# ucla-mobility/QuantV2X

Hardware: AMD Instinct MI355X
Metric: frames/sec/node (N-agent int8 BEV fusion) (higher is better)
Workload: dtype i8

## Files before the change

### include/qv2x.h

```cpp
#ifndef QV2X_H
#define QV2X_H

#include <stdint.h>

#ifdef __cplusplus
extern "C" {
#endif
#if defined(__GNUC__) || defined(__clang__)
#pragma GCC visibility push(default)
#endif

#define QV2X_OK 0
#define QV2X_EINVAL (-1)
#define QV2X_EALIGN (-2)
#define QV2X_MAX_GROUPS 4

const char* qv2x_last_error(void);
#define QV2X_ABI_VERSION 9
int qv2x_version(void);

int qv2x_fill_i8(int8_t* buf, int64_t bytes, int value, void* stream);

int64_t qv2x_voxelize_workspace_bytes(int n_points);
int qv2x_voxelize_f32(const float* points, int n_points, const float* lidar_range, const float* voxel_size, int agent,
                      int max_points, int max_voxels, void* workspace, int64_t workspace_bytes,
                      float* voxel_features, int32_t* voxel_coords, int32_t* voxel_num_points, int32_t* n_voxels, void* stream);

int64_t qv2x_voxelize_batch_workspace_bytes(int n_sweeps, const int32_t* n_points );
int qv2x_voxelize_batch_f32(const float* const* points , const int32_t* n_points , int n_sweeps,
                            const float* lidar_range, const float* voxel_size, int first_agent, int max_points, int capacity,
                            void* workspace, int64_t workspace_bytes, float* voxel_features, int32_t* voxel_coords,
                            int32_t* voxel_num_points, int32_t* voxel_counts, void* stream);

typedef struct {
    float w[64 * 10];
    float b[64];
    float d1, z1, d2, z2;
    float vox[3], off[3];
} qv2x_pfn_params;
int qv2x_pfn_scatter_i8(const float* voxel_features, const int32_t* voxel_coords, const int32_t* voxel_num_points,
                        int M, int max_points, const qv2x_pfn_params* params ,
                        int8_t* canvas, int N, int ny, int nx, void* stream);
int qv2x_pfn_unscatter_i8(const int32_t* voxel_coords, int M, int value, int8_t* canvas, int N, int ny, int nx, void* stream);

typedef struct {
    int32_t n, h, w, cin_total, stride, cout;
    int32_t ngroups;
    int32_t group_c0[QV2X_MAX_GROUPS], group_c[QV2X_MAX_GROUPS], group_zx[QV2X_MAX_GROUPS];
    int32_t out_ctotal, out_c0;
    int32_t relu;
    float out_delta, out_zp;
} qv2x_conv_desc;
int qv2x_conv3x3_i8(const qv2x_conv_desc* desc , const int8_t* in, const int8_t* w,
                    const float* scale, const int32_t* corr, const int32_t* aw, const float* bias,
                    int8_t* out, void* stream);

int qv2x_conv3x3_i8_wide_ok(const qv2x_conv_desc* desc );
int qv2x_conv3x3_i8_pack_wide(const qv2x_conv_desc* desc , const int8_t* w, int8_t* w_wide, void* stream);
int qv2x_conv3x3_i8_wide(const qv2x_conv_desc* desc , const int8_t* in, const int8_t* w_wide,
                         const float* scale, const int32_t* corr, const int32_t* aw, const float* bias,
                         int8_t* out, void* stream);

typedef struct {
    int32_t n, h, w;
    int32_t in_h, in_w;
    int32_t depth, stride0, relu;
    float out_delta[4], out_zp[4];
} qv2x_chain_desc;
int qv2x_conv3x3_i8_chain64(const qv2x_chain_desc* desc , const int8_t* in, const int8_t* w_chain,
                            const float* scale, const int32_t* corr, const int32_t* aw, const float* bias,
                            int8_t* out, void* stream);

typedef struct {
    int32_t n, h, w, cin, cout, s;
    int32_t in_zx;
    float in_delta;
    int32_t out_ctotal, out_c0, relu;
    float out_delta, out_zp;
    int32_t out_h, out_w;
} qv2x_deconv_desc;
int qv2x_deconv_i8(const qv2x_deconv_desc* desc , const int8_t* in, const float* w, const float* bias,
                   int8_t* out, void* stream);

int qv2x_deconv_i8_batch(const qv2x_deconv_desc* descs , int n, const int8_t* const* ins ,
                         const float* const* ws, const float* const* biases, int8_t* const* outs, void* stream);

typedef struct {
    int32_t n, h, w;
    int32_t levels, kc;
    int32_t in_zx;
    float in_delta;
    int32_t segs;
} qv2x_encode_desc;
int64_t qv2x_codebook_level_floats(int kc);
int qv2x_codebook_c2_f32(const float* codebook, int kc, float* c2, void* stream);
int qv2x_codebook_encode_f32(const qv2x_encode_desc* desc , const int8_t* in,
                             const float* const* level_weights ,
                             uint8_t* codes, void* stream);
int qv2x_codebook_encode_wave_f32(const qv2x_encode_desc* desc , const int8_t* in, const float* in_f32,
                                  const float* const* level_weights , uint8_t* codes, void* stream);

int qv2x_codebook_encode_collapsed_f32(const qv2x_encode_desc* desc , const int8_t* in, const float* g_packed, const float* bias,
                                       const float* tables, uint8_t* codes, void* stream);

int qv2x_codebook_encode_candidates_i8(const qv2x_encode_desc* desc , const int8_t* in, const int8_t* g_limbs, const double* bias_packed,
                                       const int32_t* tables, const float* tau , uint8_t* codes, uint32_t* list, uint32_t* counters,
                                       void* stream);
int qv2x_codebook_encode_listed_f32(const qv2x_encode_desc* desc , const int8_t* in, const float* const* level_weights ,
                                    const uint32_t* list, const uint32_t* list_count, uint8_t* codes, void* stream);

int qv2x_codebook_encode_candidates_seg_i8(const qv2x_encode_desc* desc , const int8_t* in, const int8_t* g_limbs, const double* bias_packed,
                                           const int32_t* tables, const float* tau , uint8_t* codes, uint32_t* list, uint32_t* counters,
                                           void* stream);

typedef struct {
    int32_t agents, h, w, levels, kc;
    int32_t max_cav, ego;
    int64_t code_agent_stride, code_level_stride;
    double h_metres, w_metres, discrete_ratio;
    int32_t fusion;
} qv2x_fuse_desc;
int qv2x_fuse_att_f32(const qv2x_fuse_desc* desc , const uint8_t* codes, const float* lut, const float* lut_bias,
                      const float* feats, const double* pairwise, float* fused, void* stream);

int qv2x_fuse_att_batch_f32(const qv2x_fuse_desc* desc , int n_scenes, const int64_t* scene_offset ,
                            const int32_t* scene_agents , const uint8_t* codes, const float* lut, const float* lut_bias,
                            const float* feats, const double* pairwise, float* fused, void* stream);

int qv2x_decode_lut_f32(const uint8_t* codes, int R, int levels, int kc, const float* lut, const float* lut_bias,
                        float* out, void* stream);

int qv2x_dequant_i8_f32(const int8_t* in, int n, int h, int w, int c, int zp, float delta, float* out, void* stream);

int qv2x_heads_f32(const float* x, int R, int hw, int cout, int cout_pad, const float* w, const float* bias,
                   const float* da, const float* za, float* out, void* stream);

int qv2x_fuse_heads_batch_f32(const qv2x_fuse_desc* desc , int n_scenes, const int64_t* scene_offset ,
                              const int32_t* scene_agents , const uint8_t* codes, const float* lut, const float* lut_bias,
                              const float* feats, const double* pairwise, int cout, int cout_pad, const float* w, const float* bias,
                              const float* da, const float* za, float* out, float* fused_tap, void* stream);

int qv2x_table_heads_f32(const uint8_t* codes, int R, int hw, int levels, int kc, int c0, int c1, const float* tables,
                         const float* bias, const float* da, const float* za, float* out0, float* out1, void* stream);

int qv2x_decode_heads_f32(const uint8_t* codes, int R, int hw, int levels, int kc, const float* lut, const float* lut_bias,
                          int cout, int cout_pad, const float* w, const float* bias, const float* da, const float* za,
                          float* out, void* stream);

int qv2x_single_heads_lut_f32(const uint8_t* codes, int R, int hw, int levels, int kc, int cout, const float* tables,
                              const float* bias, const float* da, const float* za, float* out, void* stream);

int qv2x_heads_pair_f32(const float* x, int R, int hw, int cout, int cout_pad, const float* w, const float* bias,
                        const float* da, const float* za, float* out,
                        const uint8_t* codes, int R1, int levels, int kc, const float* lut, const float* lut_bias,
                        int cout1, int cout_pad1, const float* w1, const float* bias1, const float* da1,
                        const float* za1, float* out1, void* stream);

typedef struct {
    int32_t h, w, anchors_per_cell, num_bins;
    float score_threshold, nms_threshold, dir_offset;
    float range[6];
    float transform[16];
    int32_t max_boxes;
    int32_t num_classes;
    int32_t range_xy_only;
    float max_extent, z_min, z_max;
} qv2x_postprocess_desc;
int64_t qv2x_postprocess_workspace_bytes(const qv2x_postprocess_desc* desc );
int qv2x_postprocess_f32(const qv2x_postprocess_desc* desc , const float* cls, const float* reg, const float* dir,
                         const float* anchors, void* workspace, int64_t workspace_bytes, float* out_corners,
                         float* out_scores, int32_t* out_labels, int32_t* out_count, void* stream);

int64_t qv2x_postprocess_batch_workspace_bytes(const qv2x_postprocess_desc* desc , int frames);
int qv2x_postprocess_batch_f32(const qv2x_postprocess_desc* desc , int frames, const float* cls, int64_t cls_frame_stride,
                               const float* reg, int64_t reg_frame_stride, const float* dir, int64_t dir_frame_stride,
                               const float* anchors, const float* transforms , void* workspace, int64_t workspace_bytes,
                               float* out_corners, float* out_scores, int32_t* out_labels, int32_t* out_count, void* stream);

int64_t qv2x_postprocess_late_workspace_bytes(const qv2x_postprocess_desc* desc , int ncav);
int qv2x_postprocess_late_f32(const qv2x_postprocess_desc* desc , int ncav, const float* const* cls, const float* const* reg,
                              const float* const* dir, const float* const* anchors, const float* transforms , void* workspace,
                              int64_t workspace_bytes, float* out_corners, float* out_scores, int32_t* out_labels, int32_t* out_count,
                              void* stream);

typedef struct {
    int32_t n, h, w;
    int32_t cin_total, cin0, cin;
    int32_t stride;
    int32_t cout;
    int32_t out_ctotal, out_c0, relu;
} qv2x_f32conv_desc;
int qv2x_conv3x3_f32(const qv2x_f32conv_desc* desc , const float* in, const float* w, const float* bias, float* out, void* stream);
int qv2x_deconv_f32(const qv2x_f32conv_desc* desc , const float* in, const float* w, const float* bias, float* out, void* stream);
int qv2x_pfn_scatter_f32(const float* voxel_features, const int32_t* voxel_coords, const int32_t* voxel_num_points, int M, int max_points,
                         const float* w, const float* b, const float* vox, const float* off, float* canvas, int N, int ny, int nx, void* stream);
int qv2x_codebook_encode_f32in(const qv2x_encode_desc* desc , const float* in, const float* const* level_weights ,
                               uint8_t* codes, void* stream);

int qv2x_pyramid_weighted_fuse_f32(const qv2x_fuse_desc* desc , int channels, const float* feats, const float* score,
                                   const double* pairwise, float* out, void* stream);


typedef struct {
    int32_t n, h, w, cin, cout, stride;
    int32_t mode, relu;
    int32_t out_ctotal, out_c0;
    float out_delta, out_zp;
    int32_t res_zx;
    float res_delta;
} qv2x_conv1x1_desc;
int qv2x_conv1x1_i8(const qv2x_conv1x1_desc* desc , const int8_t* in, const int8_t* w_frag, const float* scale,
                    const int32_t* corr, const int32_t* aw, const float* bias, const void* res, void* out, void* stream);

typedef struct {
    int32_t n, h, w, c, cg, stride, relu;
    float out_delta, out_zp;
} qv2x_gconv_desc;
int qv2x_gconv3x3_i8(const qv2x_gconv_desc* desc , const int8_t* in, const int8_t* w_frag, const float* scale,
                     const int32_t* corr, const int32_t* aw, const float* bias, int8_t* out, void* stream);

typedef struct {
    int32_t n, h, w, planes, width, cg;
    int32_t in_zx;
    float in_delta;
    float delta1, zp1, delta2, zp2, out_delta, out_zp;
} qv2x_bottleneck_desc;
int qv2x_bottleneck_i8(const qv2x_bottleneck_desc* desc , const int8_t* x, const int8_t* const* w, const float* const* scale,
                       const int32_t* const* corr, const int32_t* const* aw, const float* const* bias, int8_t* out, void* stream);

int qv2x_conv3x3_i8_res(const qv2x_conv_desc* desc , const int8_t* in, const int8_t* w, const float* scale, const int32_t* corr,
                        const int32_t* aw, const float* bias, int res_mode, const void* res, int res_zx, float res_delta,
                        int8_t* out, void* stream);

int qv2x_deconv_f32in(const qv2x_deconv_desc* desc , const float* in, const float* w, const float* bias, int8_t* out, void* stream);

int qv2x_codebook_decode_f32(const uint8_t* codes, int64_t agent_stride, int64_t level_stride, int agents, int hw, int levels,
                             int kc, int d, const float* lut, const float* bias, float* out, void* stream);

int64_t qv2x_codebook64_level_floats(int kc);
int qv2x_codebook64_c2_f32(const float* codebook, int kc, float* c2, void* stream);
int qv2x_codebook_encode64_f32(const qv2x_encode_desc* desc , int cin_total, const int8_t* in,
                               const float* const* level_weights , uint8_t* codes, void* stream);

int qv2x_codebook_encode64_f32in(const qv2x_encode_desc* desc , int cin_total, const float* in,
                                 const float* const* level_weights , uint8_t* codes, void* stream);

int qv2x_add_relu_f32(const float* a, const float* b, float* out, int64_t count, void* stream);
int qv2x_occ_sigmoid_f32(const float* in, int n, int h, int w, int c_total, float* occ, float* score, void* stream);
int qv2x_pyramid_weighted_fuse_f32p(const qv2x_fuse_desc* desc , int channels, const float* feats, const float* score,
                                    const double* pairwise, float* out, void* stream);

typedef struct {
    int32_t n, h, w, c;
    int32_t aw, corr;
    float scale, bias, out_delta, out_zp;
} qv2x_occ_desc;
int qv2x_occ_score_i8(const qv2x_occ_desc* desc , const int8_t* in, const int8_t* w, const float* score_lut, float* score,
                      uint8_t* occ_code, void* stream);

int qv2x_pyramid_weighted_fuse_i8(const qv2x_fuse_desc* desc , int channels, const int8_t* feats, int in_zx, float in_delta,
                                  const float* score, const double* pairwise, float* out, void* stream);

typedef struct {
    int32_t subm;
    int32_t k[3], s[3], p[3];
    int32_t in_shape[3], out_shape[3];
    int32_t agents, cin, cout;
    int32_t cap_in, cap_out;
    float out_delta, out_zp;
} qv2x_spconv_desc;
int qv2x_mean_vfe_f32(const float* voxel_features, const int32_t* voxel_num_points, const int32_t* n_voxels , int cap,
                      int max_points, float* out, void* stream);
int qv2x_sp_index_scatter(const int32_t* coords, const int32_t* n_rows , int cap, int agents, int D, int H, int W,
                          int32_t* volume, int set, void* stream);
int64_t qv2x_sp_out_sites_workspace_bytes(const qv2x_spconv_desc* desc );
int qv2x_sp_out_sites(const qv2x_spconv_desc* desc , const int32_t* in_coords, const int32_t* n_in, int32_t* out_volume,
                      int32_t* out_coords, int32_t* n_out, void* workspace, int64_t workspace_bytes, void* stream);
int qv2x_sp_rulebook(const qv2x_spconv_desc* desc , const int32_t* out_coords, const int32_t* n_out, const int32_t* in_volume,
                     int32_t* nbr, void* stream);
int qv2x_sp_conv_f32in(const qv2x_spconv_desc* desc , const float* feat, const int32_t* nbr, const int32_t* n_out, const float* w,
                       const float* bn_g, const float* bn_h, int8_t* out, void* stream);
int qv2x_sp_conv_i8(const qv2x_spconv_desc* desc , const int8_t* in, const int32_t* nbr, const int32_t* n_out, const int8_t* w_frag,
                    const float* scale, const int32_t* corr, const int32_t* aw, const float* bn_g, const float* bn_h, int8_t* out, void* stream);
int qv2x_sp_to_bev_i8(const int8_t* feat, const int32_t* coords, const int32_t* n_rows , int cap, int c, int c_padded, int agents,
                      int D, int H, int W, int fill, int8_t* bev, void* stream);

#define QV2X_COMM_ID_BYTES 128
int qv2x_comm_unique_id(void* id );
int qv2x_comm_init(const void* id , int world, int rank, void** comm);
int qv2x_comm_destroy(void* comm);
int qv2x_allgather_codes(void* comm, const uint8_t* send, uint8_t* recv, int64_t bytes_per_rank, void* stream);

int qv2x_pairwise_from_poses_f64(const uint8_t* gathered, int world, int64_t agent_stride_bytes, int64_t pose_offset_bytes,
                                 int max_cav, double* pairwise, void* stream);
int qv2x_pairwise_from_poses_batch_f64(const uint8_t* gathered, int world, int64_t agent_stride_bytes, int64_t pose_offset_bytes,
                                       int frames, int64_t frame_stride_bytes, int max_cav, double* pairwise, void* stream);

#define QV2X_WIRE_F32 0
#define QV2X_WIRE_U8 1
int qv2x_fuse_att_band_f32(const qv2x_fuse_desc* desc , int n_scenes, const int64_t* scene_offset ,
                           const int32_t* scene_agents , const uint8_t* codes, const float* lut, const float* lut_bias,
                           const float* feats, const double* pairwise, int64_t cell0, int64_t n_cells, float* fused, void* stream);
int qv2x_heads_band(const float* x, int n_scenes, int64_t n_cells, int cout, int cout_pad, const float* w, const float* bias,
                    const float* da, const float* za, int wire, const float* da_host , void* out, void* stream);
int qv2x_fuse_heads_band(const qv2x_fuse_desc* desc , int n_scenes, const int64_t* scene_offset ,
                         const int32_t* scene_agents , const uint8_t* codes, const float* lut, const float* lut_bias,
                         const float* feats, const double* pairwise, int64_t cell0, int64_t n_cells, int cout, int cout_pad,
                         const float* w, const float* bias, const float* da, const float* za, int wire, const float* da_host ,
                         void* out, float* fused_tap, void* stream);
int qv2x_assemble_bands(const uint8_t* slabs, int world, int64_t slab_bytes, int frames, int cout, int h, int w, int wire,
                        const float* da, const float* za, float* out, void* stream);

typedef struct {
    int32_t frames;
    int32_t det_cap;
    int32_t gt_cap;
    int32_t n_classes;
    int32_t n_ranges;
    int32_t n_thresholds;
    float ranges[4][2];
    float thresholds[4];
} qv2x_eval_desc;
int64_t qv2x_eval_workspace_bytes(const qv2x_eval_desc* desc );
int qv2x_eval_tp_fp_f32(const qv2x_eval_desc* desc , const float* det_corners, const float* det_scores, const int32_t* det_labels,
                        const int32_t* det_count, const float* gt_corners, const int32_t* gt_labels, const int32_t* gt_count,
                        void* workspace, int64_t workspace_bytes, int32_t* out_order, float* out_scores, uint8_t* out_flags,
                        int32_t* out_match, int32_t* out_gt, void* stream);

typedef struct {
    int32_t frames;
    int32_t agents;
    int32_t obj_cap;
    int32_t gt_cap;
    int32_t row_floats;
    int32_t order;
    int32_t mode;
    int32_t range_xy_only;
    float range[6];
    float iou_threshold;
} qv2x_gt_desc;
int qv2x_gt_boxes_f32(const qv2x_gt_desc* desc , const float* boxes, const uint8_t* mask, const int32_t* ids, const float* transforms,
                      const int32_t* agent_counts, float* gt_corners, int32_t* gt_labels, int32_t* gt_ids, int32_t* gt_counts,
                      int32_t* gt_totals, void* stream);

typedef struct {
    int32_t channels;
    int32_t candidates;
    int32_t n_levels;
    int32_t reserved;
    int64_t per_channel;
} qv2x_range_search_desc;
int64_t qv2x_range_search_workspace_bytes(const qv2x_range_search_desc* desc );
int qv2x_range_search_f32(const qv2x_range_search_desc* desc , const float* x, const float* delta, const float* zp, double* loss,
                          int32_t* best, void* workspace, void* stream);

#define QV2X_LSS_LOGITS 0
#define QV2X_LSS_PROBS 1
typedef struct {
    int32_t samples;
    int32_t views;
    int32_t depth_bins;
    int32_t fh, fw;
    int32_t features;
    int32_t nx[3];
    float dx[3], bx[3];
} qv2x_lss_desc;
int64_t qv2x_lss_workspace_bytes(const qv2x_lss_desc* desc );
int qv2x_lss_plan_f32(const qv2x_lss_desc* desc , const float* frustum, const float* rots, const float* trans, const float* intrins,
                      const float* post_rots, const float* post_trans, int32_t* cells_out, void* workspace, void* stream);
int qv2x_lss_splat_f32(const qv2x_lss_desc* desc , const float* depth, const float* feats, int mode, void* workspace, float* out,
                       void* stream);

#if defined(__GNUC__) || defined(__clang__)
#pragma GCC visibility pop
#endif
#ifdef __cplusplus
}
#endif
#endif
```

### quantv2x_amd/csrc/codebook_encode.h

```cpp
#pragma once
#include "common.h"

namespace qv2x {

constexpr int ENC_D = 256;
constexpr int ENC_WAVE_PAD = 16 * 256;

struct EncArgs {
    const int8_t* in; const float* in_f32; uint8_t* codes;
    const float* lvl[4];
    int n, h, w, levels, kc, ax, M;
    int segs, ke;
    float dx;
    int m_lo, m_hi;
    int list_slots = 1, list_tail_max = 0;
    const unsigned* list = nullptr; const unsigned* list_count = nullptr;
};

__device__ __host__ __forceinline__ int64_t level_floats_wg(int kc) { return 3LL * (ENC_D * ENC_D + ENC_D) + (int64_t)ENC_D * kc + (int64_t)kc * ENC_D + kc; }
__device__ __host__ __forceinline__ int64_t level_floats(int kc) { return level_floats_wg(kc) + 3LL * ENC_D * ENC_D + (int64_t)((kc + 63) / 64 * 64) * ENC_D + ENC_WAVE_PAD; }

struct ListPlan { int n[3], first[3], total, full; };
__device__ __forceinline__ ListPlan list_plan(const EncArgs& a) {
    ListPlan p;
    int t = 0;
#pragma unroll
    for (int c = 0; c < 3; ++c) { p.n[c] = (int)a.list_count[1 + c]; p.first[c] = t; t += (p.n[c] + 31) >> 5; }
    p.total = t;
    const int full = t / a.list_slots * a.list_slots;
    p.full = t - full > a.list_tail_max ? t : full;
    return p;
}
__device__ __forceinline__ void list_tile(const ListPlan& p, int tile, int& cls, int& i0) {
    cls = tile >= p.first[2] ? 2 : (tile >= p.first[1] ? 1 : 0);
    i0 = (tile - p.first[cls]) * 32;
}

int encode_wave_launch(const EncArgs& a, hipStream_t st);
int encode_wave_list_launch(const EncArgs& a, int waves, hipStream_t st);

}
```

### quantv2x_amd/csrc/codebook_encode.hip

```cpp
#include <cstdlib>

#include <atomic>

#include "codebook_encode.h"

namespace qv2x {

#ifdef QV2X_ENC_TRACE
__device__ unsigned long long g_enc_blk[4096][4];
#endif
#ifdef QV2X_ENC_FINE
__device__ long long g_enc_fine[2048][40];
#define EFINE(k) do { if (threadIdx.x == 0 && blockIdx.x < 2048) g_enc_fine[blockIdx.x][12 * l + (k)] = __builtin_amdgcn_s_memtime(); } while (0)
#else
#define EFINE(k) do { } while (0)
#endif

constexpr int LDF = 258;
__device__ __forceinline__ int kpos(int c) { return (c & ~3) | ((c & 1) << 1) | ((c >> 1) & 1); }
constexpr int D = 256;
#ifndef QV2X_ENC_LDS_PAD
#define QV2X_ENC_LDS_PAD 0
#endif

__device__ __forceinline__ void lds_barrier() {
    asm volatile("s_waitcnt lgkmcnt(0)" ::: "memory");
    __builtin_amdgcn_s_barrier();
}


struct GemmHead { float2 s0[4]; float b; };
__device__ __forceinline__ GemmHead gemm_head(const float2* __restrict__ wp, const float* __restrict__ bias, int wave, int lane) {
    const int par = lane >> 5, col = wave * 32 + (lane & 31);
    GemmHead h;
    h.b = bias[col];
    const float2* wl = wp + (size_t)col * 2 + par;
#pragma unroll
    for (int t = 0; t < 4; ++t) h.s0[t] = wl[(size_t)t * D * 2];
    return h;
}

template <int ERT>
__device__ __forceinline__ void gemm_rows_x32(const float* __restrict__ src, const float2* __restrict__ wp, const GemmHead& head,
                                              int wave, int lane, v16f (&acc)[ERT]) {
    const int par = lane >> 5, col = wave * 32 + (lane & 31);
    const float b = head.b;
#pragma unroll
    for (int i = 0; i < ERT; ++i)
#pragma unroll
        for (int r = 0; r < 16; ++r) acc[i][r] = b;
    const float2* wl = wp + (size_t)col * 2 + par;
    const float* al = src + (lane & 31) * LDF + 2 * par;
    auto loadB = [&](float2 (&dst)[4], int q0) {
#pragma unroll
        for (int t = 0; t < 4; ++t) dst[t] = wl[(size_t)(q0 + t) * D * 2];
    };
    auto compute4 = [&](const float2 (&bset)[4], int q0) {
        float2 av[4][ERT];
#pragma unroll
        for (int t = 0; t < 4; ++t)
#pragma unroll
            for (int i = 0; i < ERT; ++i) av[t][i] = *(const float2*)(al + i * 32 * LDF + (q0 + t) * 4);
#pragma unroll
        for (int t = 0; t < 4; ++t) {
#pragma unroll
            for (int i = 0; i < ERT; ++i) acc[i] = __builtin_amdgcn_mfma_f32_32x32x2f32(av[t][i].x, bset[t].x, acc[i], 0, 0, 0);
#pragma unroll
            for (int i = 0; i < ERT; ++i) acc[i] = __builtin_amdgcn_mfma_f32_32x32x2f32(av[t][i].y, bset[t].y, acc[i], 0, 0, 0);
        }
    };
    float2 s0[4], s1[4];
#pragma unroll
    for (int t = 0; t < 4; ++t) s0[t] = head.s0[t];
    for (int q0 = 0; q0 < 64; q0 += 8) {
        loadB(s1, q0 + 4);
        __builtin_amdgcn_sched_barrier(0);
        compute4(s0, q0);
        __builtin_amdgcn_sched_barrier(0);
        loadB(s0, q0 + 8);
        __builtin_amdgcn_sched_barrier(0);
        compute4(s1, q0 + 4);
        __builtin_amdgcn_sched_barrier(0);
    }
}

__device__ __forceinline__ unsigned long long dist_key(float d, int code) {
    unsigned b = __builtin_bit_cast(unsigned, d);
    b ^= (unsigned)((int)b >> 31) | 0x80000000u;
    return ((unsigned long long)b << 32) | (unsigned)code;
}

template <int ERT>
__device__ __forceinline__ void store_tile(float* __restrict__ dst, int wave, int lane, const v16f (&acc)[ERT]) {
#pragma unroll
    for (int i = 0; i < ERT; ++i)
#pragma unroll
        for (int r = 0; r < 16; ++r)
            dst[(i * 32 + mfma32_row(r, lane)) * LDF + kpos(wave * 32 + (lane & 31))] = acc[i][r];
}

constexpr int ENC_MAX_TILES = 16;
template <int ER> constexpr int enc_smem_floats() { return 2 * ER * LDF + 4 * ER + 4 * ER + 2 * ENC_MAX_TILES * ER + 4 * ER + QV2X_ENC_LDS_PAD; }

template <int ER, bool EXT, bool LIST = false>
__device__ __forceinline__ void encode_rows(const EncArgs& a, const int m0, float* __restrict__ smem, const unsigned* __restrict__ lst = nullptr,
                                            const int n_listed = 0, const int start = 0) {
    constexpr int ERT = ER / 32;
    const int segs = EXT ? a.segs : 1;
    float* bufA = smem;
    float* bufB = smem + ER * LDF;
    float* x2 = smem + 2 * ER * LDF;
    float* pval = x2 + 4 * ER;
    unsigned long long* pkey = (unsigned long long*)(pval + 4 * ER);
    int* code_s = (int*)(pkey + ENC_MAX_TILES * ER);

    const int tid = threadIdx.x, lane = tid & 63, wave = tid >> 6;
#ifdef QV2X_ENC_TRACE
    const unsigned long long t_start = __builtin_readcyclecounter();
    unsigned hwid, xcc;
    asm volatile("s_getreg_b32 %0, hwreg(HW_REG_HW_ID)" : "=s"(hwid));
    asm volatile("s_getreg_b32 %0, hwreg(HW_REG_XCC_ID)" : "=s"(xcc));
#endif
    {
        constexpr int TPR = 512 / ER;
        constexpr int CPT = D / TPR;
        const int row = tid / TPR, part = tid % TPR;
        int m = m0 + row;
        if (LIST) m = (int)lst[m < n_listed ? m : n_listed - 1];
        m = m < a.M ? m : a.M - 1;
        const int img = m / (a.h * a.w), rem = m - img * (a.h * a.w);
        const int y = rem / a.w, x = rem - y * a.w;
        const size_t pixel = (size_t)(img * (a.h + 2) + y + 1) * (a.w + 2) + x + 1;
        const int8_t* src = a.in + pixel * D + part * CPT;
        if (a.in_f32) {
            const float* sf = a.in_f32 + pixel * D + part * CPT;
#pragma unroll
            for (int c = 0; c < CPT / 4; ++c) {
                const v4f v = *(const v4f*)(sf + c * 4);
#pragma unroll
                for (int e = 0; e < 4; ++e) bufA[row * LDF + kpos(part * CPT + c * 4 + e)] = v[e];
            }
        } else
#pragma unroll
        for (int c = 0; c < CPT / 16; ++c) {
            const v4i raw = *(const v4i*)(src + c * 16);
#pragma unroll
            for (int e = 0; e < 16; ++e) {
                const int xs = (raw[e >> 2] << (24 - (e & 3) * 8)) >> 24;
                bufA[row * LDF + kpos(part * CPT + c * 16 + e)] = (float)(xs + a.ax) * a.dx;
            }
        }
    }
    GemmHead head = gemm_head((const float2*)a.lvl[0], a.lvl[0] + D * D, wave, lane);
    lds_barrier();

    v16f acc[ERT];
    for (int l = 0; l < a.levels; ++l) {
        const float* W = a.lvl[l];
        const float* stage_w = W;
        const float* stage_b = stage_w + D * D;
        const float* qhead_w = stage_b + D;
        const float* qhead_b = qhead_w + D * D;
        const float* lhead_w = qhead_b + D;
        const float* lhead_b = lhead_w + D * D;
        const float* cbp = lhead_b + D;
        const float* cb = cbp + (size_t)D * a.ke;
        const float* c2 = cb + (size_t)a.ke * D;

        EFINE(0);
        gemm_rows_x32(bufA, (const float2*)stage_w, head, wave, lane, acc);
        EFINE(1);
        const bool proven = LIST && l < start;
        if (proven) {
            head = gemm_head((const float2*)lhead_w, lhead_b, wave, lane);
            store_tile(bufB, wave, lane, acc);
            if (tid < ER * segs) {
                const int sg = tid / ER, r = tid - sg * ER;
                code_s[tid] = sg * a.kc + (int)a.codes[((size_t)l * segs + sg) * a.M + lst[m0 + r < n_listed ? m0 + r : n_listed - 1]];
            }
            lds_barrier();
        } else {
        head = gemm_head((const float2*)qhead_w, qhead_b, wave, lane);
        store_tile(bufB, wave, lane, acc);
        lds_barrier();
        EFINE(2);
        gemm_rows_x32(bufB, (const float2*)qhead_w, head, wave, lane, acc);
        EFINE(3);
        if (l + 1 < a.levels) head = gemm_head((const float2*)lhead_w, lhead_b, wave, lane);
        store_tile(bufA, wave, lane, acc);
        lds_barrier();
        EFINE(4);

        if (tid < ER * 4) {
            const int row = tid % ER, part = tid / ER;
            const float2* qr = (const float2*)(bufA + row * LDF + part * 64);
            float s = 0.0f;
#pragma unroll 4
            for (int j = 0; j < 16; ++j) {
                const float2 e = qr[2 * j], o = qr[2 * j + 1];
                s = fmaf(e.x, e.x, s); s = fmaf(o.x, o.x, s); s = fmaf(e.y, e.y, s); s = fmaf(o.y, o.y, s);
            }
            pval[part * ER + row] = s;
        }
        constexpr int TPR = 8 / ERT;
        const int ct0 = wave % TPR, rt = wave / TPR;
        const int ntile = (a.ke + 31) >> 5;
        float2 dhead[4];
        float c2v = 0.0f;
        if (ct0 < ntile) {
            const int code = ct0 * 32 + (lane & 31);
            const float2* cl = (const float2*)cbp + (size_t)code * 2 + (lane >> 5);
#pragma unroll
            for (int t = 0; t < 4; ++t) dhead[t] = cl[(size_t)t * a.ke * 2];
            c2v = c2[code];
        }
        lds_barrier();
        EFINE(5);
        if (tid < ER) {
            const float p0 = pval[tid], p1 = pval[ER + tid], p2 = pval[2 * ER + tid], p3 = pval[3 * ER + tid];
            if (segs == 1) x2[tid] = (p0 + p1) + (p2 + p3);
            else if (segs == 2) { x2[tid] = p0 + p1; x2[ER + tid] = p2 + p3; }
            else { x2[tid] = p0; x2[ER + tid] = p1; x2[2 * ER + tid] = p2; x2[3 * ER + tid] = p3; }
        }
        lds_barrier();
        EFINE(6);

#pragma unroll 1
        for (int ct = ct0; ct < ntile; ct += EXT ? TPR : ENC_MAX_TILES) {
            const int par = lane >> 5, code = ct * 32 + (lane & 31);
            v16f dacc;
#pragma unroll
            for (int r = 0; r < 16; ++r) dacc[r] = 0.0f;
            const float2* cl = (const float2*)cbp + (size_t)code * 2 + par;
            const float* al = bufA + (rt * 32 + (lane & 31)) * LDF + 2 * par;
            auto loadC = [&](float2 (&dst)[4], int q0) {
#pragma unroll
                for (int t = 0; t < 4; ++t) dst[t] = cl[(size_t)(q0 + t) * a.ke * 2];
            };
            auto dist4 = [&](const float2 (&bset)[4], int q0) {
                float2 av[4];
#pragma unroll
                for (int t = 0; t < 4; ++t) av[t] = *(const float2*)(al + (q0 + t) * 4);
#pragma unroll
                for (int t = 0; t < 4; ++t) {
                    dacc = __builtin_amdgcn_mfma_f32_32x32x2f32(av[t].x, bset[t].x, dacc, 0, 0, 0);
                    dacc = __builtin_amdgcn_mfma_f32_32x32x2f32(av[t].y, bset[t].y, dacc, 0, 0, 0);
                }
            };
            float2 s0[4], s1[4];
            if (ct == ct0) {
#pragma unroll
                for (int t = 0; t < 4; ++t) s0[t] = dhead[t];
            } else {
                loadC(s0, 0);
                c2v = c2[code];
            }
            for (int q0 = 0; q0 < 64; q0 += 8) {
                loadC(s1, q0 + 4);
                __builtin_amdgcn_sched_barrier(0);
                dist4(s0, q0);
                __builtin_amdgcn_sched_barrier(0);
                loadC(s0, q0 + 8);
                __builtin_amdgcn_sched_barrier(0);
                dist4(s1, q0 + 4);
                __builtin_amdgcn_sched_barrier(0);
            }
            EFINE(7);
            unsigned resk = 0xffffffffu;
            int resc = 0;
            const int l31 = lane & 31, hi = lane >> 5;
            const float* x2r = x2 + (segs == 1 ? 0 : (ct * 32) / a.kc) * ER;
#pragma unroll
            for (int r = 0; r < 16; ++r) {
                const int row = rt * 32 + mfma32_row(r, lane);
                const float d = (x2r[row] + c2v) - 2.0f * dacc[r];
                unsigned b = __builtin_bit_cast(unsigned, d);
                b ^= (unsigned)((int)b >> 31) | 0x80000000u;
                unsigned m = b, o;
                o = (unsigned)__builtin_amdgcn_update_dpp((int)m, (int)m, 0xB1, 0xf, 0xf, false); m = o < m ? o : m;
                o = (unsigned)__builtin_amdgcn_update_dpp((int)m, (int)m, 0x4E, 0xf, 0xf, false); m = o < m ? o : m;
                o = (unsigned)__builtin_amdgcn_update_dpp((int)m, (int)m, 0x141, 0xf, 0xf, false); m = o < m ? o : m;
                o = (unsigned)__builtin_amdgcn_update_dpp((int)m, (int)m, 0x140, 0xf, 0xf, false); m = o < m ? o : m;
                const auto sw = __builtin_amdgcn_permlane16_swap(m, m, false, false);
                m = sw[0] < sw[1] ? sw[0] : sw[1];
                const unsigned long long eq = __builtin_amdgcn_ballot_w64(b == m);
                const int c_lo = __builtin_ctz((unsigned)eq), c_hi = __builtin_ctz((unsigned)(eq >> 32));
                const int c = hi ? c_hi : c_lo;
                const bool mine = l31 == r;
                resk = mine ? m : resk;
                resc = mine ? c : resc;
            }
            if (l31 < 16) pkey[ct * ER + rt * 32 + mfma32_row(l31, lane)] = ((unsigned long long)resk << 32) | (unsigned)(ct * 32 + resc);
        }
        lds_barrier();
        EFINE(8);
        if (tid < ER) {
            const int tps = segs == 1 ? ntile : a.kc >> 5;
            for (int sg = 0; sg < segs; ++sg) {
                unsigned long long bk = pkey[(sg * tps) * ER + tid];
                for (int wv = 1; wv < tps; ++wv) {
                    const unsigned long long ok = pkey[(sg * tps + wv) * ER + tid];
                    bk = ok < bk ? ok : bk;
                }
                const int bi = (int)(unsigned)bk;
                code_s[sg * ER + tid] = bi;
                if (LIST) {
                    if (m0 + tid < n_listed) a.codes[((size_t)l * segs + sg) * a.M + lst[m0 + tid]] = (uint8_t)(bi - sg * a.kc);
                } else if (m0 + tid < a.m_hi) a.codes[((size_t)l * segs + sg) * a.M + m0 + tid] = (uint8_t)(bi - sg * a.kc);
            }
        }
        lds_barrier();
        EFINE(9);
        }

        if (l + 1 < a.levels) {
            const int col = wave * 32 + (lane & 31);
            const int* cs = code_s + ((wave * segs) >> 3) * ER;
            float cv[ERT][16];
#pragma unroll
            for (int i = 0; i < ERT; ++i)
#pragma unroll
                for (int r = 0; r < 16; ++r) cv[i][r] = cb[(size_t)cs[i * 32 + mfma32_row(r, lane)] * D + col];
            gemm_rows_x32(bufB, (const float2*)lhead_w, head, wave, lane, acc);
            EFINE(10);
            head = gemm_head((const float2*)a.lvl[l + 1], a.lvl[l + 1] + D * D, wave, lane);
#pragma unroll
            for (int i = 0; i < ERT; ++i)
#pragma unroll
                for (int r = 0; r < 16; ++r) bufA[(i * 32 + mfma32_row(r, lane)) * LDF + kpos(col)] = acc[i][r] - cv[i][r];
            lds_barrier();
            EFINE(11);
        }
    }
#ifdef QV2X_ENC_TRACE
    if (tid == 0 && blockIdx.x < 4096) {
        g_enc_blk[blockIdx.x][0] = t_start; g_enc_blk[blockIdx.x][1] = __builtin_readcyclecounter();
        g_enc_blk[blockIdx.x][2] = hwid; g_enc_blk[blockIdx.x][3] = xcc;
    }
#endif
}

template <int ER, bool EXT = false>
__global__ __launch_bounds__(512, ER == 32 ? 4 : 2) void codebook_encode_kernel(const EncArgs a) {
    __shared__ __attribute__((aligned(16))) float smem[enc_smem_floats<ER>()];
    encode_rows<ER, EXT>(a, a.m_lo + blockIdx.x * ER, smem);
}

template <bool EXT>
__global__ __launch_bounds__(512, 2) void codebook_encode_list_tail_kernel(const EncArgs a) {
    __shared__ __attribute__((aligned(16))) float smem[enc_smem_floats<32>()];
    const ListPlan plan = list_plan(a);
    for (int t = plan.full + (int)blockIdx.x; t < plan.total; t += (int)gridDim.x) {
        int cls, i0;
        list_tile(plan, t, cls, i0);
        encode_rows<32, EXT, true>(a, i0, smem, a.list + (size_t)cls * a.M, plan.n[cls], cls);
        __syncthreads();
    }
}

template <bool EXT>
__global__ __launch_bounds__(512, 2) void codebook_encode_mixed_kernel(const EncArgs a, const int n64) {
    __shared__ __attribute__((aligned(16))) float smem[enc_smem_floats<64>()];
    if ((int)blockIdx.x < n64) encode_rows<64, EXT>(a, a.m_lo + blockIdx.x * 64, smem);
    else encode_rows<32, EXT>(a, a.m_lo + n64 * 64 + ((int)blockIdx.x - n64) * 32, smem);
}

__global__ void codebook_c2_kernel(const float* __restrict__ cb, int kc, float* __restrict__ c2) {
    const int k = blockIdx.x * blockDim.x + threadIdx.x;
    if (k >= kc) return;
    float s[4];
    for (int q = 0; q < 4; ++q) {
        float acc = 0.0f;
        for (int i = 0; i < 64; ++i) { const float v = cb[(size_t)k * D + q * 64 + i]; acc = fmaf(v, v, acc); }
        s[q] = acc;
    }
    c2[k] = (s[0] + s[1]) + (s[2] + s[3]);
}

}

extern "C" int qv2x_codebook_c2_f32(const float* codebook, int kc, float* c2, void* stream) {
    using namespace qv2x;
    if (!codebook || !c2 || kc <= 0) return fail(QV2X_EINVAL, "qv2x_codebook_c2_f32: bad arguments");
    codebook_c2_kernel<<<(kc + 63) / 64, 64, 0, (hipStream_t)stream>>>(codebook, kc, c2);
    return hip_check(hipGetLastError(), "qv2x_codebook_c2_f32 launch");
}

extern "C" int64_t qv2x_codebook_level_floats(int kc) { return qv2x::level_floats(kc); }

static int encode_launch(const qv2x_encode_desc* d, const int8_t* in, const float* in_f32, const float* const* level_weights, uint8_t* codes, void* stream,
                         int form = 0);

extern "C" int qv2x_codebook_encode_wave_f32(const qv2x_encode_desc* d, const int8_t* in, const float* in_f32, const float* const* level_weights,
                                             uint8_t* codes, void* stream) {
    if (!in && !in_f32) return qv2x::fail(QV2X_EINVAL, "qv2x_codebook_encode_wave_f32: null pointer");
    return encode_launch(d, in_f32 ? (const int8_t*)in_f32 : in, in_f32, level_weights, codes, stream, 1);
}

extern "C" int qv2x_codebook_encode_f32(const qv2x_encode_desc* d, const int8_t* in, const float* const* level_weights,
                                        uint8_t* codes, void* stream) {
    return encode_launch(d, in, nullptr, level_weights, codes, stream);
}

extern "C" int qv2x_codebook_encode_f32in(const qv2x_encode_desc* d, const float* in, const float* const* level_weights,
                                          uint8_t* codes, void* stream) {
    if (!in) return qv2x::fail(QV2X_EINVAL, "qv2x_codebook_encode_f32in: null pointer");
    return encode_launch(d, (const int8_t*)in, in, level_weights, codes, stream);
}

extern "C" int qv2x_codebook_encode_listed_f32(const qv2x_encode_desc* d, const int8_t* in, const float* const* level_weights,
                                               const uint32_t* list, const uint32_t* list_count, uint8_t* codes, void* stream) {
    using namespace qv2x;
    if (!d || !in || !level_weights || !codes || !list || !list_count) return fail(QV2X_EINVAL, "qv2x_codebook_encode_listed_f32: null pointer");
    if (d->n <= 0 || d->h <= 0 || d->w <= 0 || d->levels < 1 || d->levels > 4) return fail(QV2X_EINVAL, "qv2x_codebook_encode_listed_f32: bad shape");
    const int segs = d->segs ? d->segs : 1;
    if (segs != 1 && segs != 2) return fail(QV2X_EINVAL, "qv2x_codebook_encode_listed_f32: seg_num 1 or 2 (got %d)", d->segs);
    if (d->kc < 32 || d->kc > 256 || d->kc % 32 || (segs > 1 && d->kc % 64) || segs * d->kc > 32 * ENC_MAX_TILES)
        return fail(QV2X_EINVAL, "qv2x_codebook_encode_listed_f32: dict_size must be a multiple of 32 up to 256 (of 64 with two segments): got %d x %d", segs, d->kc);
    if ((uintptr_t)in & 15) return fail(QV2X_EALIGN, "qv2x_codebook_encode_listed_f32: in must be 16-byte aligned");
    EncArgs a;
    a.in = in; a.in_f32 = nullptr; a.codes = codes; a.n = d->n; a.h = d->h; a.w = d->w; a.levels = d->levels; a.kc = d->kc;
    a.segs = segs; a.ke = segs * d->kc;
    const bool ext = segs > 1 || a.ke > 128;
    a.ax = 128 - d->in_zx; a.dx = d->in_delta; a.M = d->n * d->h * d->w; a.m_lo = 0; a.m_hi = a.M;
    a.list = list; a.list_count = list_count;
    for (int l = 0; l < 4; ++l) {
        a.lvl[l] = l < d->levels ? level_weights[l] : nullptr;
        if (l < d->levels && (!a.lvl[l] || ((uintptr_t)a.lvl[l] & 15))) return fail(QV2X_EALIGN, "qv2x_codebook_encode_listed_f32: level %d weights null or unaligned", l);
    }
    int cus = 256, dev = 0, v = 0;
    if (hipGetDevice(&dev) == hipSuccess && hipDeviceGetAttribute(&v, hipDeviceAttributeMultiprocessorCount, dev) == hipSuccess && v > 0) cus = v;
    const int tiles = (a.M + 31) / 32;
    int tail_knob = 0;
#ifdef QV2X_DEV_KNOBS
    static const int tail_env = getenv("QV2X_LIST_TAIL") ? atoi(getenv("QV2X_LIST_TAIL")) : 0;
    tail_knob = tail_env;
#endif
    a.list_slots = 4 * cus; a.list_tail_max = tail_knob > 0 ? tail_knob : 2 * cus;
    const int grid_tail = 2 * cus;
    if (tiles + 3 >= 2 * a.list_slots) {
        if (int rc = encode_wave_list_launch(a, a.list_slots, (hipStream_t)stream)) return rc;
    } else {
        a.list_slots = 1 << 30; a.list_tail_max = 1 << 30;
    }
    if (ext) codebook_encode_list_tail_kernel<true><<<tiles < grid_tail ? tiles : grid_tail, 512, 0, (hipStream_t)stream>>>(a);
    else codebook_encode_list_tail_kernel<false><<<tiles < grid_tail ? tiles : grid_tail, 512, 0, (hipStream_t)stream>>>(a);
    return hip_check(hipGetLastError(), "qv2x_codebook_encode_listed_f32 launch");
}

static int encode_launch(const qv2x_encode_desc* d, const int8_t* in, const float* in_f32, const float* const* level_weights, uint8_t* codes, void* stream,
                         int form) {
    using namespace qv2x;
    if (!d || !in || !level_weights || !codes) return fail(QV2X_EINVAL, "qv2x_codebook_encode_f32: null pointer");
    if (d->n <= 0 || d->h <= 0 || d->w <= 0 || d->levels < 1 || d->levels > 4) return fail(QV2X_EINVAL, "qv2x_codebook_encode_f32: bad shape");
    const int segs = d->segs ? d->segs : 1;
    if (segs != 1 && segs != 2 && segs != 4) return fail(QV2X_EINVAL, "qv2x_codebook_encode_f32: seg_num must be 1, 2 or 4 (got %d)", d->segs);
    if (d->kc < 32 || d->kc > 256 || d->kc % 32 || (segs > 1 && d->kc % 64) || segs * d->kc > 32 * ENC_MAX_TILES)
        return fail(QV2X_EINVAL, "qv2x_codebook_encode_f32: dict_size must be a multiple of 32 up to 256 (of 64 with seg_num > 1; seg_num * dict_size <= %d): "
                                 "got dict_size %d, seg_num %d", 32 * ENC_MAX_TILES, d->kc, segs);
    if ((uintptr_t)in & 15) return fail(QV2X_EALIGN, "qv2x_codebook_encode_f32: in must be 16-byte aligned");
    EncArgs a;
    a.in = in; a.in_f32 = in_f32; a.codes = codes; a.n = d->n; a.h = d->h; a.w = d->w; a.levels = d->levels; a.kc = d->kc;
    a.segs = segs; a.ke = segs * d->kc;
    const bool ext = segs > 1 || a.ke > 128;
    a.ax = 128 - d->in_zx; a.dx = d->in_delta; a.M = d->n * d->h * d->w; a.m_lo = 0; a.m_hi = a.M;
    for (int l = 0; l < 4; ++l) {
        a.lvl[l] = l < d->levels ? level_weights[l] : nullptr;
        if (l < d->levels && (!a.lvl[l] || ((uintptr_t)a.lvl[l] & 15))) return fail(QV2X_EALIGN, "qv2x_codebook_encode_f32: level %d weights null or unaligned", l);
    }
    int er_env = 0;
#ifdef QV2X_DEV_KNOBS
    static const int er_knob = [] { const char* e = getenv("QV2X_ENC_ROWS"); return e ? atoi(e) : 0; }();
    if (er_knob != 0 && er_knob != 32 && er_knob != 64 && er_knob != 96) return fail(QV2X_EINVAL, "QV2X_ENC_ROWS=%d: 32, 64 or 96", er_knob);
    er_env = er_knob;
#endif
    static std::atomic<int> cus_of[64];
    int cus = 256, dev = 0, v = 0;
    if (hipGetDevice(&dev) == hipSuccess && dev >= 0 && dev < 64) {
        cus = cus_of[dev].load(std::memory_order_relaxed);
        if (cus == 0) {
            cus = (hipDeviceGetAttribute(&v, hipDeviceAttributeMultiprocessorCount, dev) == hipSuccess && v > 0) ? v : 256;
            cus_of[dev].store(cus, std::memory_order_relaxed);
        }
    }
    hipStream_t st = (hipStream_t)stream;
    if (form == 1) return encode_wave_launch(a, st);
    const int slots = 4 * cus, waves = (a.M + 31) / 32;
    const int rounds = waves / slots, rest = waves - rounds * slots;
    int tail_max = 2 * cus;
#ifdef QV2X_DEV_KNOBS
    static const int tail_knob = [] { const char* e = getenv("QV2X_ENC_TAIL"); return e ? atoi(e) : -1; }();
    if (tail_knob >= 0) tail_max = tail_knob;
#endif
    if (er_env == 0 && rounds >= 1) {
        if (rest == 0 || rest > tail_max) return encode_wave_launch(a, st);
        EncArgs main = a, tail = a;
        main.m_hi = rounds * slots * 32;
        tail.m_lo = main.m_hi;
        if (int rc = encode_wave_launch(main, st)) return rc;
        if (ext) codebook_encode_kernel<32, true><<<rest, 512, 0, st>>>(tail);
        else codebook_encode_kernel<32><<<rest, 512, 0, st>>>(tail);
        return hip_check(hipGetLastError(), "qv2x_codebook_encode_f32 launch");
    }
    const int n64 = (a.M / 64) / cus * cus;
    const int er = er_env ? er_env : (n64 > 0 ? 96 : 32);
    if (er == 64) {
        if (ext) codebook_encode_kernel<64, true><<<(a.M + 63) / 64, 512, 0, st>>>(a);
        else codebook_encode_kernel<64><<<(a.M + 63) / 64, 512, 0, st>>>(a);
    } else if (er == 96 && n64 > 0) {
        if (ext) codebook_encode_mixed_kernel<true><<<n64 + (a.M - n64 * 64 + 31) / 32, 512, 0, st>>>(a, n64);
        else codebook_encode_mixed_kernel<false><<<n64 + (a.M - n64 * 64 + 31) / 32, 512, 0, st>>>(a, n64);
    } else if (ext) {
        codebook_encode_kernel<32, true><<<(a.M + 31) / 32, 512, 0, st>>>(a);
    } else {
        codebook_encode_kernel<32><<<(a.M + 31) / 32, 512, 0, st>>>(a);
    }
    return hip_check(hipGetLastError(), "qv2x_codebook_encode_f32 launch");
}

#ifdef QV2X_ENC_FINE
extern "C" __attribute__((visibility("default"))) int qv2x_debug_encode_fine(long long* host, int n) {
    return hipMemcpyFromSymbol(host, HIP_SYMBOL(qv2x::g_enc_fine), (size_t)n * 40 * sizeof(long long)) == hipSuccess ? 0 : -1;
}
#endif
#ifdef QV2X_ENC_TRACE
extern "C" __attribute__((visibility("default"))) int qv2x_debug_encode_blocks(unsigned long long* host, int n) {
    return (int)hipMemcpyFromSymbol(host, HIP_SYMBOL(qv2x::g_enc_blk), (size_t)n * 4 * sizeof(unsigned long long));
}
#endif
```

### quantv2x_amd/csrc/codebook_encode_cand.hip

```cpp
#include "common.h"

namespace qv2x {
namespace {

struct CandArgs {
    const int8_t* in; const int8_t* gpack; const double* bias; const int* tables;
    uint8_t* codes; unsigned* list; unsigned* counters;
    float tau[3][3];
    int n, h, w, hw, M, levels, kc, ke, zx, gbytes, tbytes;
    float delta;
};

constexpr int NPF = 8;
constexpr int LIMBS = 3;
template <int V> struct IC { static constexpr int value = V; };

__device__ __forceinline__ double shfl_xor_f64(double v, int m) {
    const long long b = __builtin_bit_cast(long long, v);
    const int lo = __shfl_xor((int)b, m), hi = __shfl_xor((int)(b >> 32), m);
    return __builtin_bit_cast(double, ((long long)hi << 32) | (unsigned)lo);
}

template <int CT, int SEGS, int PACK>
__global__ __launch_bounds__(256) __attribute__((amdgpu_waves_per_eu(1, 1))) void encode_candidates_kernel(const CandArgs a) {
    const int lane = threadIdx.x & 63, wave = __builtin_amdgcn_readfirstlane(threadIdx.x >> 6), j = lane & 31, hf = lane >> 5;
    const int m0 = ((int)blockIdx.x * 4 + wave) * (32 * CT);

    v4i xb[CT][8];
    int m[CT];
    float n0[CT], n1[CT];
#pragma unroll
    for (int ct = 0; ct < CT; ++ct) {
        m[ct] = m0 + 32 * ct + j;
        const int mc = m[ct] < a.M ? m[ct] : a.M - 1;
        const int img = mc / a.hw, rem = mc - img * a.hw, y = rem / a.w, x = rem - y * a.w;
        const int8_t* px = a.in + ((size_t)(img * (a.h + 2) + y + 1) * (a.w + 2) + x + 1) * 256 + 16 * hf;
#pragma unroll
        for (int s = 0; s < 8; ++s) xb[ct][s] = *(const v4i*)(px + 32 * s);
        unsigned s1 = 0, s2 = 0, sad = 0;
        const unsigned zx4 = (unsigned)a.zx * 0x01010101u;
#pragma unroll
        for (int s = 0; s < 8; ++s)
#pragma unroll
            for (int d = 0; d < 4; ++d) {
                const unsigned u = (unsigned)xb[ct][s][d] ^ 0x80808080u;
                s1 = __builtin_amdgcn_udot4(u, 0x01010101u, s1, false);
                s2 = __builtin_amdgcn_udot4(u, u, s2, false);
                sad = __builtin_amdgcn_sad_u8(u, zx4, sad);
            }
        s1 += __shfl_xor(s1, 32); s2 += __shfl_xor(s2, 32); sad += __shfl_xor(sad, 32);
        const int n2 = (int)s2 - 2 * a.zx * (int)s1 + 256 * a.zx * a.zx;
        n0[ct] = a.delta * sqrtf((float)n2);
        n1[ct] = (float)sad;
    }

    const __amdgpu_buffer_rsrc_t grs = __builtin_amdgcn_make_buffer_rsrc((void*)a.gpack, 0, a.gbytes, 0x00020000);
    int wo = 0;
    const int loff = lane * 16;
    auto gload = [&](int f) __attribute__((always_inline)) { return (v4i)__builtin_amdgcn_raw_buffer_load_b128(grs, loff, wo + f * 1024, 0); };
    v4i ring[NPF];
#pragma unroll
    for (int i = 0; i < NPF; ++i) ring[i] = gload(i);

    const __amdgpu_buffer_rsrc_t brs = __builtin_amdgcn_make_buffer_rsrc((void*)a.bias, 0, a.levels * a.ke * 8, 0x00020000);
    const __amdgpu_buffer_rsrc_t trs = __builtin_amdgcn_make_buffer_rsrc((void*)a.tables, 0, a.tbytes, 0x00020000);
    int o[2][SEGS][CT] = {};
    int first[CT];
#pragma unroll
    for (int ct = 0; ct < CT; ++ct) first[ct] = 3;
    const int ntile = a.kc >> 5;
    const int tsz = a.ke * a.ke;
    auto level = [&](auto lc) __attribute__((always_inline)) {
        constexpr int l = decltype(lc)::value;
        bool weak_l[CT];
#pragma unroll
        for (int ct = 0; ct < CT; ++ct) weak_l[ct] = false;
        auto segment = [&](auto sc) __attribute__((always_inline)) {
        constexpr int sg = decltype(sc)::value;
        double best[CT], second[CT];
#pragma unroll
        for (int ct = 0; ct < CT; ++ct) best[ct] = second[ct] = 1.0e300;
        v4i qb[2][2], qt[2][l > 0 ? l * SEGS : 1][CT];
        auto issue = [&](int T, int g, int slot) __attribute__((always_inline)) {
            const int col = sg * a.kc + 32 * T + 8 * g;
            const int kofs = l * a.ke + col;
            qb[slot][0] = (v4i)__builtin_amdgcn_raw_buffer_load_b128(brs, 32 * hf, kofs * 8, 0);
            qb[slot][1] = (v4i)__builtin_amdgcn_raw_buffer_load_b128(brs, 32 * hf + 16, kofs * 8, 0);
#pragma unroll
            for (int ct = 0; ct < CT; ++ct) {
#pragma unroll
                for (int jj = 0; jj < l; ++jj)
#pragma unroll
                    for (int sp = 0; sp < SEGS; ++sp)
                        qt[slot][jj * SEGS + sp][ct] = (v4i)__builtin_amdgcn_raw_buffer_load_b128(trs, o[jj][sp][ct], ((l * (l - 1) / 2 + jj) * tsz + col) * 4, 0);
            }
        };
#pragma unroll 1
        for (int T = 0; T < ntile; ++T) {
            v16i acc[LIMBS][CT];
#pragma unroll
            for (int lb = 0; lb < LIMBS; ++lb)
#pragma unroll
                for (int ct = 0; ct < CT; ++ct)
#pragma unroll
                    for (int r = 0; r < 16; ++r) acc[lb][ct][r] = 0;
#pragma unroll
            for (int f = 0; f < LIMBS * 8; ++f) {
                const v4i A = ring[f % NPF];
#pragma unroll
                for (int ct = 0; ct < CT; ++ct) acc[f >> 3][ct] = __builtin_amdgcn_mfma_i32_32x32x32_i8(A, xb[ct][f & 7], acc[f >> 3][ct], 0, 0, 0);
                ring[f % NPF] = gload(f + NPF);
                if (f == LIMBS * 8 - 6) issue(T, 0, 0);
                __builtin_amdgcn_sched_barrier(0);
            }
            wo += LIMBS * 8 * 1024;
#pragma unroll
            for (int g = 0; g < 4; ++g) {
                if (g < 3) issue(T, g + 1, (g + 1) & 1);
                __builtin_amdgcn_sched_barrier(0);
                const int sl = g & 1;
                double b[4];
                b[0] = __builtin_bit_cast(double, ((unsigned long long)(unsigned)qb[sl][0][1] << 32) | (unsigned)qb[sl][0][0]);
                b[1] = __builtin_bit_cast(double, ((unsigned long long)(unsigned)qb[sl][0][3] << 32) | (unsigned)qb[sl][0][2]);
                b[2] = __builtin_bit_cast(double, ((unsigned long long)(unsigned)qb[sl][1][1] << 32) | (unsigned)qb[sl][1][0]);
                b[3] = __builtin_bit_cast(double, ((unsigned long long)(unsigned)qb[sl][1][3] << 32) | (unsigned)qb[sl][1][2]);
#pragma unroll
                for (int ct = 0; ct < CT; ++ct) {
#pragma unroll
                    for (int e = 0; e < 4; ++e) {
                        const int r = 4 * g + e;
                        int lo = (acc[1][ct][r] << 8) + acc[0][ct][r];
#pragma unroll
                        for (int q = 0; q < l * SEGS; ++q) lo += qt[sl][q][ct][e];
                        double c = __builtin_fma((double)lo, (double)PACK, b[e]);
                        c = __builtin_fma((double)acc[2][ct][r], 65536.0 * PACK, c);
                        second[ct] = fmin(second[ct], fmax(best[ct], c));
                        best[ct] = fmin(best[ct], c);
                    }
                }
                __builtin_amdgcn_sched_barrier(0);
            }
        }
#pragma unroll
        for (int ct = 0; ct < CT; ++ct) {
            const double ob = shfl_xor_f64(best[ct], 32), os = shfl_xor_f64(second[ct], 32);
            const double nb = fmin(best[ct], ob), ns = fmin(fmax(best[ct], ob), fmin(second[ct], os));
            const int c = (int)((long long)nb & (PACK - 1));
            if (l < 2) o[l < 2 ? l : 0][sg][ct] = ((sg * a.kc + c) * a.ke + 4 * hf) * 4;
            const float t = ((a.tau[l][0] + a.tau[l][1] * n0[ct]) + (a.tau[l][2] * n0[ct]) * n0[ct]) + n1[ct];
            weak_l[ct] |= !(ns - nb > (double)PACK * (double)ceilf(t) + (double)(PACK - 1));
            if (hf == 0 && m[ct] < a.M) a.codes[(size_t)(l * SEGS + sg) * a.M + m[ct]] = (uint8_t)c;
        }
        };
        segment(IC<0>{});
        if constexpr (SEGS > 1) segment(IC<1>{});
#pragma unroll
        for (int ct = 0; ct < CT; ++ct)
            if (weak_l[ct] && first[ct] == 3) first[ct] = l;
    };
    level(IC<0>{});
    if (a.levels > 1) level(IC<1>{});
    if (a.levels > 2) level(IC<2>{});
    unsigned long long mask[3][CT];
    unsigned cnt[3] = {0, 0, 0};
#pragma unroll
    for (int c = 0; c < 3; ++c)
#pragma unroll
        for (int ct = 0; ct < CT; ++ct) {
            mask[c][ct] = __builtin_amdgcn_ballot_w64(first[ct] == c && hf == 0 && m[ct] < a.M);
            cnt[c] += (unsigned)__builtin_popcountll(mask[c][ct]);
        }
    __shared__ unsigned wcnt[4][3], wbase[3];
    if (lane == 0) { wcnt[wave][0] = cnt[0]; wcnt[wave][1] = cnt[1]; wcnt[wave][2] = cnt[2]; }
    __syncthreads();
    if (threadIdx.x < 3) {
        const unsigned tot = wcnt[0][threadIdx.x] + wcnt[1][threadIdx.x] + wcnt[2][threadIdx.x] + wcnt[3][threadIdx.x];
        wbase[threadIdx.x] = tot ? atomicAdd(a.counters + 1 + threadIdx.x, tot) : 0u;
        if (tot) atomicAdd(a.counters, tot);
    }
    __syncthreads();
    unsigned base[3];
#pragma unroll
    for (int c = 0; c < 3; ++c) {
        base[c] = wbase[c];
        for (int w2 = 0; w2 < wave; ++w2) base[c] += wcnt[w2][c];
    }
#pragma unroll
    for (int c = 0; c < 3; ++c) {
        unsigned at = __builtin_amdgcn_readfirstlane(base[c]);
#pragma unroll
        for (int ct = 0; ct < CT; ++ct) {
            if (first[ct] == c && hf == 0 && m[ct] < a.M)
                a.list[(size_t)c * a.M + at + (unsigned)__builtin_popcountll(mask[c][ct] & ((1ull << lane) - 1ull))] = (unsigned)m[ct];
            at += (unsigned)__builtin_popcountll(mask[c][ct]);
        }
    }
}

__global__ void zero_counters_kernel(unsigned* c) { if (threadIdx.x < 4) c[threadIdx.x] = 0; }

template <int CT, int SEGS, int PACK>
void launch(const CandArgs& a, hipStream_t st) {
    encode_candidates_kernel<CT, SEGS, PACK><<<(a.M + 128 * CT - 1) / (128 * CT), 256, 0, st>>>(a);
}

template <int PACK, int MAX_SEGS>
int candidates(const char* me, const qv2x_encode_desc* d, const int8_t* in, const int8_t* g_limbs, const double* bias_packed, const int32_t* tables,
               const float* tau, uint8_t* codes, uint32_t* list, uint32_t* counters, void* stream) {
    if (!d || !in || !g_limbs || !bias_packed || !tau || !codes || !list || !counters) return fail(QV2X_EINVAL, "%s: null pointer", me);
    if (d->n <= 0 || d->h <= 0 || d->w <= 0 || d->levels < 1 || d->levels > 3) return fail(QV2X_EINVAL, "%s: 1..3 levels", me);
    const int segs = d->segs ? d->segs : 1;
    if (segs < 1 || segs > MAX_SEGS) return fail(QV2X_EINVAL, "%s: seg_num 1 .. %d (got %d; the exact entry takes seg_num 1 | 2 | 4)", me, MAX_SEGS, d->segs);
    if (d->kc < 32 || d->kc > PACK || d->kc % 32 || (segs > 1 && d->kc % 64))
        return fail(QV2X_EINVAL, "%s: dict_size a multiple of 32 up to %d (of 64 with two segments; got %d x %d)", me, PACK, segs, d->kc);
    if (d->levels > 1 && !tables) return fail(QV2X_EINVAL, "%s: the residual levels need their tables", me);
    if (d->in_zx < 0 || d->in_zx > 255) return fail(QV2X_EINVAL, "%s: in_zx outside 0..255", me);
    if (((uintptr_t)in & 15) || ((uintptr_t)g_limbs & 15) || ((uintptr_t)tables & 15) || ((uintptr_t)bias_packed & 7))
        return fail(QV2X_EALIGN, "%s: 16-byte aligned maps, limbs and tables", me);
    CandArgs a;
    a.in = in; a.gpack = g_limbs; a.bias = bias_packed; a.tables = tables; a.codes = codes; a.list = list; a.counters = counters;
    for (int l = 0; l < 3; ++l)
        for (int i = 0; i < 3; ++i) a.tau[l][i] = l < d->levels ? tau[l * 3 + i] : 0.0f;
    a.n = d->n; a.h = d->h; a.w = d->w; a.hw = d->h * d->w; a.M = d->n * a.hw; a.levels = d->levels; a.kc = d->kc; a.ke = segs * d->kc; a.zx = d->in_zx;
    a.gbytes = d->levels * (a.ke / 32) * LIMBS * 8 * 1024;
    a.tbytes = (d->levels > 1 ? d->levels * (d->levels - 1) / 2 : 1) * a.ke * a.ke * 4;
    a.delta = d->in_delta;
    hipStream_t st = (hipStream_t)stream;
    zero_counters_kernel<<<1, 64, 0, st>>>(counters);
    int dev = 0, cus = 256, v = 0;
    if (hipGetDevice(&dev) == hipSuccess && hipDeviceGetAttribute(&v, hipDeviceAttributeMultiprocessorCount, dev) == hipSuccess && v > 0) cus = v;
    const bool large = a.M >= 4 * cus * 32 * (segs == 2 ? 3 : 4) * 2;
    if (segs == 1) large ? launch<4, 1, PACK>(a, st) : launch<2, 1, PACK>(a, st);
    else if constexpr (MAX_SEGS > 1) large ? launch<3, 2, PACK>(a, st) : launch<2, 2, PACK>(a, st);
    return hip_check(hipGetLastError(), me);
}

}
}

extern "C" int qv2x_codebook_encode_candidates_i8(const qv2x_encode_desc* d, const int8_t* in, const int8_t* g_limbs, const double* bias_packed,
                                                  const int32_t* tables, const float* tau, uint8_t* codes, uint32_t* list, uint32_t* counters,
                                                  void* stream) {
    return qv2x::candidates<128, 1>("qv2x_codebook_encode_candidates_i8", d, in, g_limbs, bias_packed, tables, tau, codes, list, counters, stream);
}

extern "C" int qv2x_codebook_encode_candidates_seg_i8(const qv2x_encode_desc* d, const int8_t* in, const int8_t* g_limbs, const double* bias_packed,
                                                      const int32_t* tables, const float* tau, uint8_t* codes, uint32_t* list, uint32_t* counters,
                                                      void* stream) {
    return qv2x::candidates<256, 2>("qv2x_codebook_encode_candidates_seg_i8", d, in, g_limbs, bias_packed, tables, tau, codes, list, counters, stream);
}
```

### quantv2x_amd/csrc/codebook_encode_wave.hip

```cpp
#include "codebook_encode.h"

namespace qv2x {

namespace {

constexpr int D = ENC_D;
constexpr int RS = 260;
constexpr int NPF = 4;

__device__ __forceinline__ v16f mfma(float a, float b, v16f c) { return __builtin_amdgcn_mfma_f32_32x32x2f32(a, b, c, 0, 0, 0); }


__device__ __forceinline__ void tile_to_lds(float* __restrict__ row, int h, int T, const v16f& acc) {
#pragma unroll
    for (int rq = 0; rq < 4; ++rq) {
        float* g = row + (4 * T + rq) * 8 + 2 * h;
        *(float2*)g = make_float2(acc[4 * rq], acc[4 * rq + 2]);
        *(float2*)(g + 4) = make_float2(acc[4 * rq + 1], acc[4 * rq + 3]);
    }
}

__device__ __forceinline__ void lds_to_operand(const float* __restrict__ row, int h, float (&m)[128]) {
#pragma unroll
    for (int g = 0; g < 32; ++g) {
        const v4f v = *(const v4f*)(row + g * 8 + 4 * h);
        m[4 * g] = v.x; m[4 * g + 1] = v.y; m[4 * g + 2] = v.z; m[4 * g + 3] = v.w;
    }
}

__device__ __forceinline__ void tile_vec(const float* __restrict__ p, int h, int T, v4f (&o)[4]) {
#pragma unroll
    for (int rq = 0; rq < 4; ++rq) o[rq] = *(const v4f*)(p + 32 * T + 8 * rq + 4 * h);
}

#ifdef QV2X_ENCW_FINE
__device__ long long g_encw_fine[4096][32];
#define WFINE(k) do { if (threadIdx.x == 0 && blockIdx.x < 4096) g_encw_fine[blockIdx.x][8 * l + (k)] = __builtin_readcyclecounter(); } while (0)
#define WFINE2(k) do { if (fine2 && threadIdx.x == 0 && blockIdx.x < 4096) g_encw_fine[blockIdx.x][24 + (k)] = __builtin_readcyclecounter(); } while (0)
#define WFINE2_ARM(v) fine2 = (v)
#else
#define WFINE(k) do { } while (0)
#define WFINE2(k) do { } while (0)
#define WFINE2_ARM(v) do { } while (0)
#endif

}

template <int V> struct IC { static constexpr int value = V; };

template <bool F32IN, int SEGS, bool LIST = false>
__global__ __attribute__((amdgpu_flat_work_group_size(64, 64), amdgpu_waves_per_eu(1, 1))) void codebook_encode_wave_kernel(const EncArgs a) {
    __shared__ __attribute__((aligned(16))) float smem[32 * RS];
    const int lane = threadIdx.x, j = lane & 31, h = lane >> 5;
    float* const row = smem + j * RS;
    ListPlan plan{};
    if (LIST) plan = list_plan(a);
#pragma unroll 1
    for (int round = 0; LIST ? round * (int)gridDim.x < plan.full : round == 0; ++round) {
    const int tile = LIST ? round * (int)gridDim.x + ((round & 1) ? (int)gridDim.x - 1 - (int)blockIdx.x : (int)blockIdx.x) : (int)blockIdx.x;
    if (LIST && tile >= plan.full) continue;
    int mrow;
    bool owned;
    int start = 0;
    if (LIST) {
        int cls, i0;
        list_tile(plan, tile, cls, i0);
        owned = i0 + j < plan.n[cls];
        mrow = (int)a.list[(size_t)cls * a.M + (owned ? i0 + j : plan.n[cls] - 1)];
        start = cls;
    } else {
        mrow = a.m_lo + tile * 32 + j;
        owned = mrow < a.m_hi;
    }

    float xq[128], z[128];
    {
        int m = mrow;
        m = m < a.M ? m : a.M - 1;
        const int img = m / (a.h * a.w), rem = m - img * (a.h * a.w);
        const int y = rem / a.w, x = rem - y * a.w;
        const size_t pixel = (size_t)(img * (a.h + 2) + y + 1) * (a.w + 2) + x + 1;
        if (F32IN) {
            const v4f* sf = (const v4f*)(a.in_f32 + pixel * D);
#pragma unroll
            for (int q = 0; q < 64; ++q) {
                const v4f v = sf[q];
                xq[2 * q] = h ? v.y : v.x;
                xq[2 * q + 1] = h ? v.w : v.z;
            }
        } else {
            const v4i* src = (const v4i*)(a.in + pixel * D);
            const float fax = (float)(a.ax - 128);
#pragma unroll
            for (int c = 0; c < 16; ++c) {
                const v4i raw = src[c];
#pragma unroll
                for (int d = 0; d < 4; ++d) {
                    const unsigned u = ((unsigned)raw[d] ^ 0x80808080u) >> (8 * h);
                    xq[8 * c + 2 * d] = ((float)(u & 0xffu) + fax) * a.dx;
                    xq[8 * c + 2 * d + 1] = ((float)((u >> 16) & 0xffu) + fax) * a.dx;
                }
            }
        }
    }

    for (int l = 0; l < a.levels; ++l) {
        const float* W = a.lvl[l];
        const float* stage_b = W + D * D;
        const float* qhead_b = stage_b + D + D * D;
        const float* lhead_b = qhead_b + D + D * D;
        const float* cb = lhead_b + D + (size_t)D * a.ke;
        const float* c2 = cb + (size_t)a.ke * D;
        const __amdgpu_buffer_rsrc_t wrs = __builtin_amdgcn_make_buffer_rsrc((void*)(W + level_floats_wg(a.ke)), 0, 0x7fffffff, 0x00020000);
        int wo = 0;
        const int loff = lane * 16;
        auto wload = [&](int grp) __attribute__((always_inline)) {
            return __builtin_bit_cast(v4f, __builtin_amdgcn_raw_buffer_load_b128(wrs, loff, wo + grp * 1024, 0));
        };
        const bool last = l + 1 == a.levels;
        const int npair = (a.ke + 63) >> 6;

        v4f bn[2][4];
        auto next_vec = [&](const float* p, int P) __attribute__((always_inline)) {
            tile_vec(p, h, 2 * P, bn[0]);
            tile_vec(p, h, 2 * P + 1, bn[1]);
        };
        auto next_c2 = [&](int P) __attribute__((always_inline)) {
            tile_vec(c2, h, 2 * P, bn[0]);
            if (64 * P + 32 < a.ke) tile_vec(c2, h, 2 * P + 1, bn[1]);
            else
#pragma unroll
                for (int i = 0; i < 4; ++i) bn[1][i] = v4f{INFINITY, INFINITY, INFINITY, INFINITY};
        };
        auto next_c2s = [&](int s0, int s1, int P) __attribute__((always_inline)) {
            tile_vec(c2 + s0 * a.kc, h, P, bn[0]);
            tile_vec(c2 + s1 * a.kc, h, P, bn[1]);
        };
        next_vec(stage_b, 0);
        __builtin_amdgcn_sched_barrier(0);
        v4f ring[2 * NPF];
#pragma unroll
        for (int i = 0; i < 2 * NPF; ++i) ring[i] = wload(i);
        __builtin_amdgcn_sched_barrier(0);

        v16f acc[2];
#ifdef QV2X_ENCW_FINE
        bool fine2 = false;
#endif
        auto tile2g = [&](const float (&m)[128], const bool biased, auto&& hook, auto ng_c, auto off0_c, auto off1_c) __attribute__((always_inline)) {
            constexpr int NG = decltype(ng_c)::value, OFF0 = decltype(off0_c)::value, OFF1 = decltype(off1_c)::value;
            WFINE2(0);
#pragma unroll
            for (int t = 0; t < 2; ++t)
#pragma unroll
                for (int r = 0; r < 16; ++r) acc[t][r] = biased ? bn[t][r >> 2][r & 3] : 0.0f;
            WFINE2(1);
#pragma unroll
            for (int g = 0; g < NG; ++g) {
                const v4f A0 = ring[(2 * g) % (2 * NPF)], A1 = ring[(2 * g + 1) % (2 * NPF)];
                acc[0] = mfma(A0.x, m[OFF0 + 4 * g], acc[0]);
                acc[1] = mfma(A1.x, m[OFF1 + 4 * g], acc[1]);
                __builtin_amdgcn_sched_barrier(0);
                acc[0] = mfma(A0.y, m[OFF0 + 4 * g + 1], acc[0]);
                acc[1] = mfma(A1.y, m[OFF1 + 4 * g + 1], acc[1]);
                __builtin_amdgcn_sched_barrier(0);
                acc[0] = mfma(A0.z, m[OFF0 + 4 * g + 2], acc[0]);
                acc[1] = mfma(A1.z, m[OFF1 + 4 * g + 2], acc[1]);
                __builtin_amdgcn_sched_barrier(0);
                acc[0] = mfma(A0.w, m[OFF0 + 4 * g + 3], acc[0]);
                acc[1] = mfma(A1.w, m[OFF1 + 4 * g + 3], acc[1]);
                if (g == NG - NPF - 1) hook();
                if (NG == 32 && g == 7) WFINE2(2);
                if (NG == 32 && g == 15) WFINE2(3);
                if (NG == 32 && g == 23) WFINE2(4);
#ifndef QV2X_ENCW_ABL_NOLOAD
                ring[(2 * g) % (2 * NPF)] = wload(2 * (g + NPF));
                ring[(2 * g + 1) % (2 * NPF)] = wload(2 * (g + NPF) + 1);
#endif
                __builtin_amdgcn_sched_barrier(0);
            }
#ifndef QV2X_ENCW_ABL_SAMEW
            wo += NG * 2048;
#endif
            WFINE2(5);
        };
        auto tile2 = [&](const float (&m)[128], const bool biased, auto&& hook) __attribute__((always_inline)) {
            tile2g(m, biased, hook, IC<32>{}, IC<0>{}, IC<0>{});
        };

        WFINE(0);
#pragma unroll 1
        for (int P = 0; P < 4; ++P) {
            WFINE2_ARM(l == 1 && P == 1);
            tile2(xq, true, [&]() __attribute__((always_inline)) { next_vec(P < 3 ? stage_b : qhead_b, P < 3 ? P + 1 : 0); });
            tile_to_lds(row, h, 2 * P, acc[0]);
            tile_to_lds(row, h, 2 * P + 1, acc[1]);
            WFINE2(6);
            WFINE2_ARM(false);
        }
        WFINE(1);
        lds_to_operand(row, h, z);
        WFINE(2);
        unsigned bcs = 0;
        if (LIST && l < start) {
            wo = SEGS == 1 ? (8 + npair) * 65536 : 8 * 65536 + (SEGS / 2) * (a.kc >> 5) * (32 / SEGS) * 2048;
            next_vec(lhead_b, 0);
#pragma unroll
            for (int i = 0; i < 2 * NPF; ++i) ring[i] = wload(i);
#pragma unroll
            for (int sg = 0; sg < SEGS; ++sg) bcs |= (unsigned)a.codes[((size_t)l * SEGS + sg) * a.M + mrow] << (8 * sg);
        } else {
#pragma unroll 1
        for (int P = 0; P < 4; ++P) {
            tile2(z, true, [&]() __attribute__((always_inline)) { if (P < 3) next_vec(qhead_b, P + 1); else if (SEGS == 1) next_c2(0); else next_c2s(0, 1, 0); });
            tile_to_lds(row, h, 2 * P, acc[0]);
            tile_to_lds(row, h, 2 * P + 1, acc[1]);
        }
        WFINE(3);
        lds_to_operand(row, h, xq);
        float x2s[4];
        {
            const float* qh = row + 128 * h;
            float p[2];
#pragma unroll
            for (int c = 0; c < 2; ++c) {
                float s = 0.0f;
#pragma unroll
                for (int g = 0; g < 8; ++g) {
                    const v4f e = *(const v4f*)(qh + (8 * c + g) * 8), o = *(const v4f*)(qh + (8 * c + g) * 8 + 4);
                    s = fmaf(e.x, e.x, s); s = fmaf(o.x, o.x, s); s = fmaf(e.y, e.y, s); s = fmaf(o.y, o.y, s);
                    s = fmaf(e.z, e.z, s); s = fmaf(o.z, o.z, s); s = fmaf(e.w, e.w, s); s = fmaf(o.w, o.w, s);
                }
                p[c] = s;
            }
            const float mine = p[0] + p[1];
            const float other = __shfl_xor(mine, 32);
            if (a.segs == 1) {
                x2s[0] = x2s[1] = x2s[2] = x2s[3] = mine + other;
            } else if (a.segs == 2) {
                x2s[0] = h ? other : mine; x2s[1] = h ? mine : other; x2s[2] = x2s[3] = 0.0f;
            } else {
                const float o0 = __shfl_xor(p[0], 32), o1 = __shfl_xor(p[1], 32);
                x2s[0] = h ? o0 : p[0]; x2s[1] = h ? o1 : p[1]; x2s[2] = h ? p[0] : o0; x2s[3] = h ? p[1] : o1;
            }
        }
        WFINE(4);
        if constexpr (SEGS == 1) {
        float best = INFINITY;
        int bc = 0;
        const int ppseg = npair / a.segs;
#pragma unroll 1
        for (int P = 0; P < npair; ++P) {
            const int seg = a.segs == 1 ? 0 : P / ppseg, cbase = seg * a.kc;
            const float x2 = seg == 0 ? x2s[0] : (seg == 1 ? x2s[1] : (seg == 2 ? x2s[2] : x2s[3]));
            v4f c2t[2][4];
#pragma unroll
            for (int t = 0; t < 2; ++t)
#pragma unroll
                for (int i = 0; i < 4; ++i) c2t[t][i] = bn[t][i];
            tile2(xq, false, [&]() __attribute__((always_inline)) { if (P + 1 < npair) next_c2(P + 1); else if (!last) next_vec(lhead_b, 0); });
#pragma unroll
            for (int t = 0; t < 2; ++t)
#pragma unroll
                for (int r = 0; r < 16; ++r) {
                    const float s = x2 + c2t[t][r >> 2][r & 3];
                    const float d = s - 2.0f * acc[t][r];
                    const int code = 64 * P + 32 * t + 8 * (r >> 2) + 4 * h + (r & 3) - cbase;
                    const bool lt = d < best;
                    best = lt ? d : best;
                    bc = lt ? code : bc;
                }
            if (a.segs == 1 ? P + 1 == npair : (P + 1) % ppseg == 0) {
                const float od = __shfl_xor(best, 32);
                const int oc = __shfl_xor(bc, 32);
                if (od < best || (od == best && oc < bc)) bc = oc;
                if (h == 0 && owned) a.codes[((size_t)l * a.segs + seg) * a.M + mrow] = (uint8_t)bc;
                bcs |= (unsigned)bc << (8 * seg);
                best = INFINITY; bc = 0;
            }
        }
        } else {
            const int ntile = a.kc >> 5;
            auto seg_pairs = [&](auto sa_c, auto sb_c, const bool more_after) __attribute__((always_inline)) {
                constexpr int SA = decltype(sa_c)::value, SB = decltype(sb_c)::value, NG = 32 / SEGS;
                float best[2] = {INFINITY, INFINITY};
                int bc[2] = {0, 0};
#pragma unroll 1
                for (int P = 0; P < ntile; ++P) {
                    v4f c2t[2][4];
#pragma unroll
                    for (int t = 0; t < 2; ++t)
#pragma unroll
                        for (int i = 0; i < 4; ++i) c2t[t][i] = bn[t][i];
                    tile2g(xq, false, [&]() __attribute__((always_inline)) {
                        if (P + 1 < ntile) next_c2s(SA, SB, P + 1);
                        else if (more_after) next_c2s(SA + 2, SB + 2, 0);
                        else if (!last) next_vec(lhead_b, 0);
                    }, IC<NG>{}, IC<4 * NG * SA>{}, IC<4 * NG * SB>{});
#pragma unroll
                    for (int t = 0; t < 2; ++t) {
                        const float x2 = x2s[t ? SB : SA];
#pragma unroll
                        for (int r = 0; r < 16; ++r) {
                            const float sv = x2 + c2t[t][r >> 2][r & 3];
                            const float d = sv - 2.0f * acc[t][r];
                            const int code = 32 * P + 8 * (r >> 2) + 4 * h + (r & 3);
                            const bool lt = d < best[t];
                            best[t] = lt ? d : best[t];
                            bc[t] = lt ? code : bc[t];
                        }
                    }
                }
#pragma unroll
                for (int t = 0; t < 2; ++t) {
                    const int seg = t ? SB : SA;
                    const float od = __shfl_xor(best[t], 32);
                    const int oc = __shfl_xor(bc[t], 32);
                    if (od < best[t] || (od == best[t] && oc < bc[t])) bc[t] = oc;
                    if (h == 0 && owned) a.codes[((size_t)l * SEGS + seg) * a.M + mrow] = (uint8_t)bc[t];
                    bcs |= (unsigned)bc[t] << (8 * seg);
                }
            };
            if constexpr (SEGS == 2) seg_pairs(IC<0>{}, IC<1>{}, false);
            else { seg_pairs(IC<0>{}, IC<1>{}, true); seg_pairs(IC<2>{}, IC<3>{}, false); }
        }
        }
        WFINE(5);
        if (last) break;
#pragma unroll 1
        for (int P = 0; P < 4; ++P) {
            const int seg = (P * a.segs) >> 2;
            const float* cw = cb + (size_t)(seg * a.kc + (int)((bcs >> (8 * seg)) & 0xffu)) * D;
            v4f cv[2][4];
            tile_vec(cw, h, 2 * P, cv[0]);
            tile_vec(cw, h, 2 * P + 1, cv[1]);
            __builtin_amdgcn_sched_barrier(0);
            tile2(z, true, [&]() __attribute__((always_inline)) { if (P < 3) next_vec(lhead_b, P + 1); });
#pragma unroll
            for (int t = 0; t < 2; ++t) {
#pragma unroll
                for (int r = 0; r < 16; ++r) acc[t][r] = acc[t][r] - cv[t][r >> 2][r & 3];
                tile_to_lds(row, h, 2 * P + t, acc[t]);
            }
        }
        WFINE(6);
        lds_to_operand(row, h, xq);
        WFINE(7);
    }
    }
}

int encode_wave_launch(const EncArgs& a, hipStream_t st) {
    const unsigned grid = (unsigned)((a.m_hi - a.m_lo + 31) / 32);
    if (a.segs == 2) {
        if (a.in_f32) codebook_encode_wave_kernel<true, 2><<<grid, 64, 0, st>>>(a);
        else codebook_encode_wave_kernel<false, 2><<<grid, 64, 0, st>>>(a);
    } else if (a.segs == 4) {
        if (a.in_f32) codebook_encode_wave_kernel<true, 4><<<grid, 64, 0, st>>>(a);
        else codebook_encode_wave_kernel<false, 4><<<grid, 64, 0, st>>>(a);
    } else if (a.in_f32) codebook_encode_wave_kernel<true, 1><<<grid, 64, 0, st>>>(a);
    else codebook_encode_wave_kernel<false, 1><<<grid, 64, 0, st>>>(a);
    return hip_check(hipGetLastError(), "qv2x_codebook_encode_f32 (wave form) launch");
}


int encode_wave_list_launch(const EncArgs& a, int waves, hipStream_t st) {
    if ((a.segs != 1 && a.segs != 2) || a.in_f32) return fail(QV2X_EINVAL, "qv2x_codebook_encode_listed_f32: seg_num 1 | 2, i8 rows");
    if (a.segs == 2) codebook_encode_wave_kernel<false, 2, true><<<(unsigned)waves, 64, 0, st>>>(a);
    else codebook_encode_wave_kernel<false, 1, true><<<(unsigned)waves, 64, 0, st>>>(a);
    return hip_check(hipGetLastError(), "qv2x_codebook_encode_listed_f32 launch");
}

}

#ifdef QV2X_ENCW_FINE
extern "C" __attribute__((visibility("default"))) int qv2x_debug_encw_fine(long long* host, int n) {
    return hipMemcpyFromSymbol(host, HIP_SYMBOL(qv2x::g_encw_fine), (size_t)n * 32 * sizeof(long long)) == hipSuccess ? 0 : -1;
}
#endif
```

### quantv2x_amd/encode_two_stage.py

```python
from typing import Dict

import numpy as np

U = 2.0 ** -24
LIMBS = 3
G_MAX_INT = 2 ** 23 - 2 ** 15 - 2 ** 7 - 1


def _sn(m):
    return float(np.linalg.norm(m, 2)) if m.size else 0.0


def _kappa(w, block=8):
    k = w.shape[1]
    return float(sum(min(block, k - i0) * _sn(w[:, :min(k, i0 + block)]) for i0 in range(0, k, block)))


class _Aff:

    def __init__(self, p=0.0, r=0.0):
        self.p, self.r = float(p), float(r)

    def __add__(self, o):
        return _Aff(self.p + o.p, self.r + o.r)

    def scale(self, c):
        return _Aff(self.p * c, self.r * c)


def encode_error_bound(state: Dict[str, np.ndarray], levels: int, delta: float, segs: int = 1):
    g = lambda l, n: state[f"codebook/{l}/{n}"].astype(np.float64)
    u1 = U / (1.0 - U)
    ub = u1 / (1.0 - 256.0 * u1)
    eye = np.eye(256)
    A, shift, back = eye.copy(), np.zeros(256), []
    srcs = [(eye.copy(), _Aff(U, 0.0), "x0 = fl(n * delta)")]
    ea, eb, ec, report = [], [], [], []

    def offset(shift, back):
        return float(np.linalg.norm(shift) + sum(sum(float(n.max()) for n in np.split(np.linalg.norm(g(j, "codebook") @ B.T, axis=1), segs))
                                                 for j, B in enumerate(back)))

    def norm_bound(A, shift, back, srcs):
        d = _Aff()
        for M, e, _ in srcs:
            d = d + e.scale(_sn(M))
        return _Aff(_sn(A), offset(shift, back)) + d

    def layer(W, b, vin: _Aff):
        return _Aff(ub * _kappa(W) * vin.p, ub * (256.0 * float(np.linalg.norm(b)) + _kappa(W) * vin.r) + 1e-30)

    for l in range(levels):
        S, bs, Q, bq, Cb = g(l, "stage_w"), g(l, "stage_b"), g(l, "qhead_w"), g(l, "qhead_b"), g(l, "codebook")
        vx = norm_bound(A, shift, back, srcs)
        srcs = [(S @ M, e, n) for M, e, n in srcs] + [(eye.copy(), layer(S, bs, vx), f"stage{l}")]
        A, shift, back = S @ A, S @ shift + bs, [S @ B for B in back]
        vz = norm_bound(A, shift, back, srcs)
        sq = [(Q @ M, e, n) for M, e, n in srcs] + [(eye.copy(), layer(Q, bq, vz), f"qhead{l}")]
        vq = norm_bound(Q @ A, Q @ shift + bq, [Q @ B for B in back], sq)
        cn = np.linalg.norm(Cb, axis=1)
        cmax, c2max = float(cn.max()), float((cn ** 2).max())
        e = _Aff()
        for M, eps, name in sq:
            wpair = 0.0
            for K in np.split(Cb @ M, segs):
                gram = K @ K.T
                dg = np.diag(gram)
                wpair = max(wpair, float(np.sqrt(max(0.0, (dg[:, None] + dg[None, :] - 2.0 * gram).max()))))
            e = e + eps.scale(2.0 * wpair)
            report.append((l, name, wpair, eps.p, eps.r))
        e = e + vq.scale(2.0 * 2.0 * 256.0 * ub * cmax)
        e = e + vq.scale(2.0 * 2.0 * U * cmax * (1.0 + 256.0 * ub))
        fin = 2.0 * U * (2.0 + U)
        x2 = fin * (1.0 + 2.0 ** -17)
        ea.append(e.r + (fin * (1.0 + 1e-5) + 2.0 * 67.0 * U) * c2max + x2 * vq.r * vq.r)
        eb.append(e.p + x2 * 2.0 * vq.p * vq.r)
        ec.append(x2 * vq.p * vq.p)
        if l < levels - 1:
            Lh, bl = g(l, "lhead_w"), g(l, "lhead_b")
            srcs = [(Lh @ M, e_, n) for M, e_, n in srcs] + [(eye.copy(), layer(Lh, bl, vz), f"lhead{l}")]
            A, shift, back = Lh @ A, Lh @ shift + bl, [Lh @ B for B in back] + [eye.copy()]
            vn = norm_bound(A, shift, back, srcs)
            srcs = srcs + [(eye.copy(), vn.scale(U / (1.0 - U)), f"sub{l}")]
    host = 1.0 + 1e-6
    return np.array(ea) * host, np.array(eb) * host, np.array(ec) * host, report


def pack_factor(segs: int, kc: int) -> int:
    return 128 if segs == 1 and kc <= 128 else 256


CANDIDATE_ENTRY = {128: "qv2x_codebook_encode_candidates_i8", 256: "qv2x_codebook_encode_candidates_seg_i8"}


def candidate_tables(state: Dict[str, np.ndarray], levels: int, in_delta: float, in_zx: int, segs: int = 1) -> Dict[str, np.ndarray]:
    from .engine import collapse_encoder_f64
    G, gb, tabs = collapse_encoder_f64(state, levels)
    ke = G.shape[0] // levels
    kc = ke // segs
    if any(state[f"codebook/{l}/codebook"].shape[0] != ke for l in range(levels)):
        raise ValueError("two-stage encode: every level needs the same dict_size")
    if segs == 1:
        if kc % 32 or kc > 256 or levels > 3:
            raise ValueError("two-stage encode: dict_size 32 | 64 | 96 | 128 | ... | 256, up to three levels")
    elif segs != 2 or kc * segs != ke or kc % 64 or kc > 256 or levels > 3:
        raise ValueError("two-stage encode: seg_num 1 | 2, dict_size a multiple of 64 up to 256 with two segments, up to three levels")
    n_t = segs * max(levels - 1, 0)
    tlim = 2.0 ** 29 / max(2, n_t)
    blim = 2.0 ** 44 if pack_factor(segs, kc) == 128 else 2.0 ** 43
    gs = float(in_delta) * G
    tmax = max([float(np.abs(t).max()) for t in tabs.values()] + [0.0])
    h = max(float(np.abs(gs).max()) / G_MAX_INT, tmax / (tlim - 2.0), float(np.abs(gb).max()) / (blim - 2.0 ** 32))
    gi = np.rint(gs / h).astype(np.int64)
    limbs, rest = [], gi.copy()
    for _ in range(LIMBS):
        d = ((rest + 128) % 256) - 128
        limbs.append(d.astype(np.int8))
        rest = (rest - d) // 256
    if rest.any():
        raise ValueError("two-stage encode: G on the grid does not fit the candidate stage's int8 limbs")
    bias = np.rint(gb / h).astype(np.int64) + (128 - int(in_zx)) * gi.sum(1)
    tables = np.stack([np.rint(tabs[(l, j)] / h) for l in range(levels) for j in range(l)]) if levels > 1 else np.zeros((1, ke, ke))
    if np.abs(tables).max() >= tlim or np.abs(bias).max() >= blim:
        raise ValueError("two-stage encode: table / bias entries leave the fixed-point range of the candidate stage")
    lane = np.arange(64)
    score = (np.arange(levels * ke // 32)[:, None, None, None] * 32 + (lane & 31)[None, None, :, None])
    chan = (32 * np.arange(8)[None, :, None, None] + 16 * (lane >> 5)[None, None, :, None] + np.arange(16)[None, None, None, :])
    packed = np.stack([lb[score, chan] for lb in limbs], axis=1)
    packed = packed.reshape(levels, ke // 32, LIMBS, 8, 64, 16)
    ea, eb, ec, report = encode_error_bound(state, levels, in_delta, segs)
    fp = 1.0 + 1e-4
    tau = np.zeros((levels, 3))
    for l in range(levels):
        own = 1.0 + segs * l + 2.0
        tau[l] = [(ea[l] / h + own) * fp, eb[l] / h * fp, ec[l] / h * fp]
    return {"gpack": np.ascontiguousarray(packed, dtype=np.int8), "bias": np.ascontiguousarray(bias, dtype=np.int64),
            "tables": np.ascontiguousarray(tables, dtype=np.int32), "tau": np.ascontiguousarray(tau, dtype=np.float32), "h": h,
            "g_int": gi, "bound": (ea, eb, ec), "report": report, "segs": segs, "kc": kc, "pack": pack_factor(segs, kc)}


def candidate_emulate(codes_u8: np.ndarray, tabs: Dict[str, np.ndarray], in_delta: float, in_zx: int):
    gi, bias, tables, tau, h = tabs["g_int"], tabs["bias"], tabs["tables"], tabs["tau"], tabs["h"]
    levels = tau.shape[0]
    segs = int(tabs.get("segs", 1))
    ke = gi.shape[0] // levels
    kc = ke // segs
    P = float(tabs.get("pack", 128))
    b = codes_u8.astype(np.float64) - 128.0
    s = b @ gi.astype(np.float64).T + bias.astype(np.float64)[None]
    n = codes_u8.astype(np.int64) - int(in_zx)
    n1, n2 = np.abs(n).sum(1), (n * n).sum(1)
    n0 = (np.float32(in_delta) * np.sqrt(n2.astype(np.float32))).astype(np.float32)
    out = np.zeros((levels * segs, codes_u8.shape[0]), np.uint8)
    flags = np.zeros((levels * segs, codes_u8.shape[0]), bool)
    gaps = np.zeros((levels * segs, codes_u8.shape[0]))
    for l in range(levels):
        sc = s[:, l * ke:(l + 1) * ke].copy()
        for j in range(l):
            for sp in range(segs):
                sc += tables[l * (l - 1) // 2 + j][sp * kc + out[j * segs + sp].astype(np.int64)].astype(np.float64)
        t = (((tau[l, 0] + tau[l, 1] * n0) + (tau[l, 2] * n0) * n0) + n1.astype(np.float32)).astype(np.float32)
        assert t.dtype == np.float32 and n0.dtype == np.float32
        t = t.astype(np.float64)
        for sg in range(segs):
            v = sc[:, sg * kc:(sg + 1) * kc]
            order = np.argsort(v, axis=1, kind="stable")
            best, second = np.take_along_axis(v, order[:, :1], 1)[:, 0], np.take_along_axis(v, order[:, 1:2], 1)[:, 0]
            p = l * segs + sg
            out[p] = order[:, 0]
            k2 = order[:, 1]
            flags[p] = (P * second + k2) - (P * best + out[p]) <= P * np.ceil(t) + (P - 1.0)
            gaps[p] = (second - best) * h
    return out, flags.any(0), flags, gaps
```

### quantv2x_amd/engine.py

```python
from __future__ import annotations

import ctypes as C
from typing import Dict, List, NamedTuple, Optional

import numpy as np
import torch
import torch.nn as nn

from . import lib as L
from .ptq_state import export_ptq_state, load_ptq_state

_HEADS = ("cls_head", "reg_head", "dir_head")


def _dev(a: np.ndarray, dev) -> torch.Tensor:
    return torch.from_numpy(np.ascontiguousarray(a)).to(dev).contiguous()


def _pack_k4(w: np.ndarray) -> np.ndarray:
    j, k = w.shape
    assert k % 4 == 0
    return np.ascontiguousarray(w.T.reshape(k // 4, 4, j).transpose(0, 2, 1), dtype=np.float32)


def decode_tables(state: Dict[str, np.ndarray], levels: int, width: int = 256):
    g = lambda l, n: state[f"codebook/{l}/{n}"].astype(np.float64)
    tables, const, chain = [], np.zeros(width), np.eye(width)
    for l in range(levels):
        front = chain @ g(l, "restore_w")
        tables.append((front @ g(l, "dqhead_w") @ g(l, "codebook").T).T)
        const = const + front @ g(l, "dqhead_b") + chain @ g(l, "restore_b")
        if l < levels - 1:
            const = const + front @ g(l, "side_b")
            chain = front @ g(l, "side_w")
    return np.ascontiguousarray(np.stack(tables), dtype=np.float32), np.ascontiguousarray(const, dtype=np.float32)


def collapse_encoder_f64(state: Dict[str, np.ndarray], levels: int):
    g = lambda l, n: state[f"codebook/{l}/{n}"].astype(np.float64)
    kc = int(state["codebook/0/codebook"].shape[0])
    front, shift = np.eye(256), np.zeros(256)
    back = []
    G, gb, tables = [], [], {}
    for l in range(levels):
        Ws, bs, Wq, bq, Cb = g(l, "stage_w"), g(l, "stage_b"), g(l, "qhead_w"), g(l, "qhead_b"), g(l, "codebook")
        Gp = -2.0 * Cb @ Wq @ Ws
        gp = (Cb * Cb).sum(1) - 2.0 * Cb @ (Wq @ bs + bq)
        G.append(Gp @ front)
        gb.append(Gp @ shift + gp)
        for j, Bj in enumerate(back):
            tables[(l, j)] = -(Gp @ Bj @ g(j, "codebook").T).T
        if l < levels - 1:
            A = g(l, "lhead_w") @ Ws
            d = g(l, "lhead_w") @ bs + g(l, "lhead_b")
            front, shift = A @ front, A @ shift + d
            back = [A @ Bj for Bj in back] + [np.eye(256)]
    return np.concatenate(G), np.concatenate(gb), tables


def collapse_encoder(state: Dict[str, np.ndarray], levels: int, in_delta: float, in_zx: int):
    Gall, gall, tables = collapse_encoder_f64(state, levels)
    kc = Gall.shape[0] // levels
    bias = gall + in_delta * (0.0 - in_zx) * Gall.sum(1)
    Gs = in_delta * Gall
    nct = levels * kc // 32
    lane = np.arange(64)
    col = (np.arange(nct)[:, None, None] * 32 + (lane & 31)[None, None, :])
    k = (2 * np.arange(128)[None, :, None] + (lane >> 5)[None, None, :])
    packed = Gs[col, k]
    tab = np.stack([tables[(l, j)] for l in range(levels) for j in range(l)]) if levels > 1 else np.zeros((1, kc, kc))
    return (np.ascontiguousarray(packed, dtype=np.float32), np.ascontiguousarray(bias, dtype=np.float32), np.ascontiguousarray(tab, dtype=np.float32))


def _pack_k4p(w: np.ndarray) -> np.ndarray:
    return np.ascontiguousarray(_pack_k4(w)[:, :, [0, 2, 1, 3]])


def _pack_wave(w: np.ndarray) -> np.ndarray:
    j, k = w.shape
    assert k == 256
    if j % 64:
        w = np.concatenate([w, np.zeros((64 - j % 64, k), w.dtype)])
    return np.ascontiguousarray(w.reshape(-1, 2, 32, 32, 4, 2).transpose(0, 3, 1, 5, 2, 4), dtype=np.float32)


ENC_WAVE_PAD = 16 * 256


def _pack_wave_seg(cb: np.ndarray, segs: int) -> np.ndarray:
    ke, k = cb.shape
    kc, d = ke // segs, 256 // segs
    assert k == 256 and segs in (2, 4) and kc % 32 == 0
    blocks = np.stack([cb[sg * kc:(sg + 1) * kc, sg * d:(sg + 1) * d] for sg in range(segs)])
    b = blocks.reshape(segs // 2, 2, kc // 32, 32, d // 8, 4, 2)
    return np.ascontiguousarray(b.transpose(0, 2, 4, 1, 6, 3, 5), dtype=np.float32)


def wave_section(stage_w, qhead_w, lhead_w, cb, segs: int = 1) -> np.ndarray:
    cbs = _pack_wave(cb) if segs == 1 else _pack_wave_seg(cb, segs)
    sec = np.concatenate([_pack_wave(stage_w).reshape(-1), _pack_wave(qhead_w).reshape(-1), cbs.reshape(-1), _pack_wave(lhead_w).reshape(-1)])
    full = 3 * 65536 + (cb.shape[0] + 63) // 64 * 64 * 256
    return np.concatenate([sec, np.zeros(full - sec.size + ENC_WAVE_PAD, np.float32)])


class _ConvLayer:

    def __init__(self, state, name, in_groups, stride, dev, pad_cin=0, pad_cout=0):
        code = state[name + "/w_code"]
        dw = state[name + "/w_delta"].astype(np.float32)
        zw = state[name + "/w_zp"].astype(np.int64)
        bias_np = state[name + "/bias"].astype(np.float32)
        if pad_cin > code.shape[1]:
            fill = np.broadcast_to(np.clip(zw, 0, 255).astype(np.uint8)[:, None, None, None], (code.shape[0], pad_cin - code.shape[1], 3, 3))
            code = np.concatenate([code, fill], axis=1)
        if pad_cout > code.shape[0]:
            extra = pad_cout - code.shape[0]
            code = np.concatenate([code, np.full((extra,) + code.shape[1:], 128, np.uint8)])
            dw, zw = np.concatenate([dw, np.ones(extra, np.float32)]), np.concatenate([zw, np.full(extra, 128, np.int64)])
            bias_np = np.concatenate([bias_np, np.zeros(extra, np.float32)])
        cout = code.shape[0]
        ws = code.astype(np.int64) - 128
        aw = 128 - zw
        parts, corr, scale = [], [], []
        for (c0, c, dx, zx) in in_groups:
            blk = ws[:, c0:c0 + c].transpose(0, 2, 3, 1).reshape(cout, -1)
            parts.append(blk)
            ax = 128 - int(zx)
            corr.append(ax * blk.sum(axis=1) + blk.shape[1] * ax * aw)
            scale.append(np.float32(dx) * dw)
        self.name, self.stride, self.cout = name, stride, cout
        self.groups = [(int(c0), int(c), int(zx)) for (c0, c, _, zx) in in_groups]
        self.w = _dev(np.concatenate(parts, axis=1).astype(np.int8), dev)
        self.w_wide = None
        self.scale = _dev(np.stack(scale).astype(np.float32), dev)
        self.corr = _dev(np.stack(corr).astype(np.int32), dev)
        self.aw = _dev(aw.astype(np.int32), dev)
        self.bias = _dev(bias_np, dev)
        self.out_q = (float(np.float32(state[name + "/a_delta"])), int(state[name + "/a_zp"]))
        assert np.abs(np.stack(corr)).max() < 2 ** 31


class _ChainLayers:
    MAX_DEPTH = 4

    @staticmethod
    def eligible(convs) -> bool:
        return (1 <= len(convs) <= _ChainLayers.MAX_DEPTH and all(c.cout == 64 and len(c.groups) == 1 and c.groups[0][1] == 64 for c in convs)
                and all(c.stride == 1 for c in convs[1:]))

    def __init__(self, convs, dev):
        self.convs = convs
        self.name = convs[-1].name
        packed = []
        for c in convs:
            w = c.w.cpu().numpy().reshape(2, 32, 9, 2, 2, 16)
            packed.append(w.transpose(0, 2, 3, 4, 1, 5))
        self.w = _dev(np.stack(packed).astype(np.int8), dev)
        cat = lambda ts: torch.cat([t.reshape(-1) for t in ts]).contiguous()
        self.scale, self.corr = cat([c.scale for c in convs]), cat([c.corr for c in convs])
        self.aw, self.bias = cat([c.aw for c in convs]), cat([c.bias for c in convs])
        self.stride0 = convs[0].stride
        self.out_q = convs[-1].out_q


class _DeconvLayer:
    def __init__(self, state, name, in_q, dev):
        code = state[name + "/w_code"].astype(np.float32)
        dw = state[name + "/w_delta"].astype(np.float32).reshape(-1, 1, 1, 1)
        zw = state[name + "/w_zp"].astype(np.float32).reshape(-1, 1, 1, 1)
        wdeq = ((code - zw) * dw).astype(np.float32)
        cin, cout, s, _ = wdeq.shape
        cols = wdeq.transpose(0, 2, 3, 1).reshape(cin, s * s * cout)
        self.w = _dev(_pack_k4p(cols.T), dev)
        self.bias = _dev(state[name + "/bias"].astype(np.float32), dev)
        self.name, self.cin, self.cout, self.s, self.in_q = name, cin, cout, s, in_q
        self.out_q = (float(np.float32(state[name + "/a_delta"])), int(state[name + "/a_zp"]))


class _Heads:

    def __init__(self, state, suffix, dev):
        ws, bs, das, zas = [], [], [], []
        for h in _HEADS:
            n = h + suffix
            code = state[n + "/w_code"].astype(np.float32).reshape(state[n + "/w_code"].shape[0], -1)
            w = ((code - state[n + "/w_zp"].astype(np.float32)[:, None]) * state[n + "/w_delta"].astype(np.float32)[:, None])
            ws.append(w.astype(np.float32))
            bs.append(state[n + "/bias"].astype(np.float32))
            off = bool(state[n + "/a_off"])
            das.append(np.full(w.shape[0], -1.0 if off else float(np.float32(state[n + "/a_delta"])), np.float32))
            zas.append(np.full(w.shape[0], 0.0 if off else float(state[n + "/a_zp"]), np.float32))
        self._stack(ws, bs, das, zas, dev)

    @classmethod
    def folded_fp32(cls, state, suffix, dev):
        hd = cls.__new__(cls)
        ws = [state[h + suffix + "/w"] for h in _HEADS]
        hd._stack(ws, [state[h + suffix + "/bias"] for h in _HEADS], [np.full(w.shape[0], -1.0, np.float32) for w in ws],
                  [np.zeros(w.shape[0], np.float32) for w in ws], dev)
        return hd

    def _stack(self, ws, bs, das, zas, dev):
        self.splits = [w.shape[0] for w in ws]
        self.cout = sum(self.splits)
        self.cout_pad = (self.cout + 31) // 32 * 32
        if self.cout_pad > 96:
            raise NotImplementedError("heads: at most 96 stacked output channels")
        pad = self.cout_pad - self.cout
        w = np.concatenate(ws + [np.zeros((pad, 256), np.float32)])
        self.w = _dev(_pack_k4p(w), dev)
        self.bias = _dev(np.concatenate(bs + [np.zeros(pad, np.float32)]), dev)
        self.da = _dev(np.concatenate(das + [np.full(pad, -1.0, np.float32)]), dev)
        self.za = _dev(np.concatenate(zas + [np.zeros(pad, np.float32)]), dev)
        self._w_np, self._b_np = np.concatenate(ws).astype(np.float64), np.concatenate(bs).astype(np.float64)
        self.da_np = np.ascontiguousarray(np.concatenate(das))
        self.lut_tables = None

    def collapse_over_decode(self, lut: np.ndarray, lut_bias: np.ndarray, dev):
        t = np.einsum("lkd,cd->lkc", lut.astype(np.float64), self._w_np)
        b = lut_bias.astype(np.float64) @ self._w_np.T + self._b_np
        self.lut_tables = (_dev(t.astype(np.float32), dev), _dev(b.astype(np.float32), dev))


def scene_layout(data_dict: dict, n_total: int):
    pairwise = data_dict["pairwise_t_matrix"]
    if pairwise.dtype != torch.float64 or not pairwise.is_contiguous():
        pairwise = pairwise.to(torch.float64).contiguous()
    if pairwise.shape[0] == 1:
        return pairwise, [n_total]
    rl = data_dict["record_len"]
    if isinstance(rl, torch.Tensor) and rl.is_cuda and torch.cuda.is_current_stream_capturing():
        raise ValueError("record_len on the GPU cannot be read during HIP-graph capture: pass a CPU tensor")
    return pairwise, [int(v) for v in (rl.tolist() if isinstance(rl, torch.Tensor) else rl)]


def split_heads(preds: torch.Tensor, splits, suffix: str = "") -> dict:
    c, r, _ = splits
    out = {"cls_preds" + suffix: preds[:, :c], "reg_preds" + suffix: preds[:, c:c + r], "dir_preds" + suffix: preds[:, c + r:]}
    if not suffix:
        out["preds_tensor"] = preds
    return out


def capture_call(call):
    side = torch.cuda.Stream()
    side.wait_stream(torch.cuda.current_stream())
    with torch.cuda.stream(side):
        for _ in range(2):
            call()
    torch.cuda.current_stream().wait_stream(side)
    graph = torch.cuda.CUDAGraph()
    with torch.cuda.graph(graph):
        out = call()

    def replay():
        graph.replay()
        return out
    replay.graph = graph
    return replay


def capture_forward(module: nn.Module, data_dict: dict):
    rl = data_dict.get("record_len")
    if data_dict["pairwise_t_matrix"].shape[0] > 1 and isinstance(rl, torch.Tensor) and rl.is_cuda:
        data_dict = dict(data_dict, record_len=rl.cpu())
    return capture_call(lambda: module.forward(data_dict))


def assemble_heter_codes(owner: str, engines: dict, slot_cache: dict, agents: list, data_dict: dict, encode, taps: Optional[dict]) -> torch.Tensor:
    unknown = sorted(set(agents) - set(engines))
    if unknown:
        raise NotImplementedError(f"{owner}: no engine for modality {unknown}")
    slots = slot_cache.get(tuple(agents))
    if slots is None:
        if torch.cuda.is_current_stream_capturing():
            raise L.Qv2xError(f"{owner}: agent layout {agents} is new and the stream is capturing -- its slot indices are an H2D copy; "
                              "run one eager forward of this layout first (capture does)")
        slots = {m: torch.as_tensor([i for i, a in enumerate(agents) if a == m], dtype=torch.int64, device=e.dev) for m, e in engines.items()}
        slot_cache[tuple(agents)] = slots
    e = next(iter(engines.values()))
    n_total, hw, lv = len(agents), e.fh * e.fw, e.levels
    enc = torch.empty((lv, n_total * hw), dtype=torch.uint8, device=e.dev)
    for m, eng in engines.items():
        k = int(slots[m].numel())
        if not k:
            continue
        mt = {} if taps is not None else None
        codes = encode(eng, data_dict["inputs_" + m], k, mt).view(lv, k, hw)
        enc.view(lv, n_total, hw).index_copy_(1, slots[m], codes)
        if taps is not None:
            taps["modality/" + m] = mt
    return enc


def pillar_inputs(inputs: dict, pfn: bool = True):
    vf = inputs["voxel_features"].contiguous()
    co = inputs["voxel_coords"].to(torch.int32).contiguous()
    npnt = inputs["voxel_num_points"].to(torch.int32).contiguous()
    if pfn and (vf.dtype != torch.float32 or vf.dim() != 3 or tuple(vf.shape[1:]) != (32, 4)):
        raise ValueError("voxel_features must be float32 [M, 32, 4]")
    return vf, co, npnt


def pfn_params(state: Dict[str, np.ndarray]):
    s, n = state, "encoder_m1.pillar_vfe.pfn_layers.0.linear"
    wq = ((s[n + "/w_code"].astype(np.float32) - s[n + "/w_zp"].astype(np.float32)[:, None])
          * s[n + "/w_delta"].astype(np.float32)[:, None]).astype(np.float32)
    if wq.shape != (64, 10):
        raise NotImplementedError("deployed PFN expects Linear(10 -> 64)")
    p = L.PfnParams()
    p.w[:] = wq.reshape(-1).tolist()
    p.b[:] = s[n + "/bias"].astype(np.float32).tolist()
    p.d1, p.z1 = float(np.float32(s[n + "/a_delta"])), float(s[n + "/a_zp"])
    p.d2, p.z2 = float(np.float32(s["pfn/a2_delta"])), float(s["pfn/a2_zp"])
    p.vox[:] = [float(np.float32(v)) for v in s["meta/voxel"]]
    p.off[:] = [float(np.float32(v)) for v in s["meta/offset"]]
    return p, (p.d2, int(p.z2))


def level_blob_host(state: Dict[str, np.ndarray], l: int, ke: int, D: int, segs: int):
    W = 64 if D == 64 else 256
    last = f"codebook/{l}/lhead_w" not in state

    def padded(n, *shape):
        out = np.zeros(shape, np.float32)
        if not (last and n.startswith("lhead")):
            a = state[f"codebook/{l}/{n}"]
            out[tuple(slice(0, k) for k in a.shape)] = a
        return out
    stage, qhead, lhead, cb = padded("stage_w", W, W), padded("qhead_w", W, W), padded("lhead_w", W, W), padded("codebook", ke, W)
    parts = [_pack_k4p(stage), padded("stage_b", W), _pack_k4p(qhead), padded("qhead_b", W), _pack_k4p(lhead), padded("lhead_b", W),
             _pack_k4p(cb), cb, np.zeros(ke, np.float32)]
    flat = np.concatenate([p.reshape(-1) for p in parts])
    c2_off = flat.size - ke
    if W == 256:
        flat = np.concatenate([flat, wave_section(stage, qhead, lhead, cb, segs)])
    return flat, c2_off - ke * W, c2_off


def level_blob(lib, state: Dict[str, np.ndarray], l: int, ke: int, D: int, segs: int, dev) -> torch.Tensor:
    flat, cb_off, c2_off = level_blob_host(state, l, ke, D, segs)
    floats, c2fn, name = ((lib.qv2x_codebook64_level_floats, lib.qv2x_codebook64_c2_f32, "qv2x_codebook64_c2_f32") if D == 64
                          else (lib.qv2x_codebook_level_floats, lib.qv2x_codebook_c2_f32, "qv2x_codebook_c2_f32"))
    assert flat.size == floats(ke)
    blob = _dev(flat, dev)
    L.check(c2fn(C.c_void_p(blob.data_ptr() + 4 * cb_off), ke, C.c_void_p(blob.data_ptr() + 4 * c2_off), L.current_stream()), name)
    return blob


class CodebookConstants(NamedTuple):
    enc_levels: int
    segs: int
    levels: int
    ke: int
    kc: int
    D: int
    lut_host: np.ndarray
    lut_bias_host: np.ndarray
    lut: torch.Tensor
    lut_bias: torch.Tensor
    level_blobs: List[torch.Tensor]
    level_ptrs: object


def codebook_constants(lib, state: Dict[str, np.ndarray], dev, refuse) -> CodebookConstants:
    s = state
    enc_levels, segs = int(s["meta/codebook_levels"]), int(s.get("meta/codebook_segs", 1))
    ke, D = (int(v) for v in s["codebook/0/codebook"].shape)
    kc, levels = ke // segs, enc_levels * segs
    refuse(ke, kc, D, segs)
    lut, lut_bias = decode_tables(s, enc_levels, D)
    lut = lut.reshape(levels, kc, D)
    blobs = [level_blob(lib, s, l, ke, D, segs, dev) for l in range(enc_levels)]
    return CodebookConstants(enc_levels, segs, levels, ke, kc, D, lut, lut_bias, _dev(lut, dev), _dev(lut_bias, dev), blobs,
                             (C.c_void_p * enc_levels)(*[b.data_ptr() for b in blobs]))


def _pairwise_from_poses(self, gathered: torch.Tensor, world: int, agent_stride: int, pose_offset: int, max_cav: int, out: torch.Tensor):
    L.check(self.lib.qv2x_pairwise_from_poses_f64(L.ptr(gathered), world, agent_stride, pose_offset, max_cav, L.ptr(out),
                                                  L.current_stream()), "qv2x_pairwise_from_poses_f64")


class DeployedPostStage(nn.Module):
    fuse_heads_min_tiles = 4 * 1280
    fuse_heads_max_agents = 4
    single_agent_tables = True
    band_one_launch = None
    _band_rows = None

    def __init__(self, state: Dict[str, np.ndarray], device, emit_single_preds: Optional[bool]):
        super().__init__()
        self.lib = L.load()
        if not torch.cuda.is_available():
            raise L.Qv2xError(f"{type(self).__name__} needs an MI355X (torch.cuda.is_available() is False)")
        self.state, self.dev = state, torch.device(device)
        s, dev = state, self.dev
        if str(s.get("meta/fusion_method", "att")) not in ("att", "max"):
            raise NotImplementedError(f"deployed path: fusion_method {s['meta/fusion_method']!r} ('att' = AttFusion and 'max' = MaxFusion are built here)")
        self.fusion = 1 if str(s.get("meta/fusion_method", "att")) == "max" else 0
        self.nx, self.ny, _ = (int(v) for v in s["meta/grid"])
        self.hm, self.wm = (float(v) for v in s["meta/HW_metres"])
        self.ratio = float(s["meta/discrete_ratio"])
        self.layer_nums = [int(v) for v in s["meta/layer_nums"]]
        self.strides = [int(v) for v in s["meta/layer_strides"]]
        self.ups = [int(v) for v in s["meta/upsample_strides"]]
        self.has_codebook = bool(s["meta/has_codebook"])
        self.emit_single = bool(s["meta/supervise_single"]) if emit_single_preds is None else bool(emit_single_preds)
        self._lut_host = (None, None)
        if self.has_codebook:
            c = codebook_constants(self.lib, s, dev, self._refuse_codebook)
            self.enc_levels, self.segs, self.levels, self.ke, self.kc = c.enc_levels, c.segs, c.levels, c.ke, c.kc
            self.lut, self.lut_bias, self.level_blobs, self.level_ptrs = c.lut, c.lut_bias, c.level_blobs, c.level_ptrs
            self._lut_host = (c.lut_host, c.lut_bias_host)

    @staticmethod
    def _refuse_codebook(ke, kc, D, segs):
        if ke > 512 or kc > 256:
            raise NotImplementedError(f"deployed codebook path: seg_num * dict_size <= 512, dict_size <= 256 (got {segs} x {kc}): "
                                      "the encode kernels' tile budget (qv2x_codebook_encode_f32)")
        if D != 256:
            raise NotImplementedError(f"deployed codebook path: a codebook as wide as the 256-channel shared feature (got {D})")

    def _set_heads(self, heads: _Heads, heads_single: Optional[_Heads], tables: bool):
        self.heads, self.heads_single = heads, heads_single
        self.table_heads, self.single_by_tables, self.single_by_global_tables = None, False, False
        if not (tables and self.has_codebook):
            return
        (lut, lut_bias), dev = self._lut_host, self.dev
        self.single_by_tables = (self.heads_single is not None and self.levels <= 4
                                 and self.levels * self.kc * self.heads_single.cout * 4 <= 60 * 1024)
        self.single_by_global_tables = (not self.single_by_tables and self.heads_single is not None and self.levels <= 16
                                        and self.heads_single.cout % 4 == 0 and self.heads_single.cout <= 128)
        if self.single_by_tables or self.single_by_global_tables:
            self.heads_single.collapse_over_decode(lut, lut_bias, dev)
        sets = [self.heads] + ([self.heads_single] if self.heads_single is not None else [])
        ct = sum(h.cout for h in sets)
        ct4 = (ct + 3) // 4 * 4
        st = ct4 if (ct4 // 4) % 2 else ct4 + 4
        in_lds = self.levels <= 4 and (self.levels * self.kc * st + 4 * ct4) * 4 <= 160 * 1024
        if in_lds or (self.levels <= 16 and ct % 4 == 0 and ct <= 128):
            t = np.concatenate([np.einsum("lkd,cd->lkc", lut.astype(np.float64), h._w_np) for h in sets], axis=2)
            b = np.concatenate([lut_bias.astype(np.float64) @ h._w_np.T + h._b_np for h in sets])
            cat = lambda name: torch.cat([getattr(h, name)[:h.cout] for h in sets]).contiguous()
            self.table_heads = (_dev(t.astype(np.float32), dev), _dev(b.astype(np.float32), dev), cat("da"), cat("za"),
                                self.heads.cout, self.heads_single.cout if self.heads_single is not None else 0)

    def _run_heads(self, hd: _Heads, rows, nb, hw):
        out = torch.empty((nb, hd.cout, self.fh, self.fw), dtype=torch.float32, device=self.dev)
        L.check(self.lib.qv2x_heads_f32(L.ptr(rows), nb * hw, hw, hd.cout, hd.cout_pad, L.ptr(hd.w), L.ptr(hd.bias),
                                        L.ptr(hd.da), L.ptr(hd.za), L.ptr(out), L.current_stream()), "qv2x_heads_f32")
        return out

    def wire_shape(self):
        self._workspace(1)
        return self.levels, self.fh * self.fw

    pairwise_from_poses = _pairwise_from_poses

    def pairwise_frames_from_poses(self, gathered: torch.Tensor, world: int, agent_stride: int, pose_offset: int, frames: int, frame_stride: int,
                                   max_cav: int, out: torch.Tensor):
        L.check(self.lib.qv2x_pairwise_from_poses_batch_f64(L.ptr(gathered), world, agent_stride, pose_offset, frames, frame_stride, max_cav,
                                                            L.ptr(out), L.current_stream()), "qv2x_pairwise_from_poses_batch_f64")

    def fuse_frames_and_heads(self, gathered: torch.Tensor, agent_stride: int, level_stride: int, frame_stride: int, pairwise: torch.Tensor,
                              n_agents: int, ego: int, own_codes: Optional[torch.Tensor], frames: int) -> dict:
        lens = [n_agents] * frames
        form = self._post_form(lens, None, own_codes is not None and frame_stride == self.fh * self.fw)
        return self._post(form, L.ptr(gathered), agent_stride, level_stride, None, pairwise, [f * frame_stride for f in range(frames)], lens, ego,
                          own_codes, frames)

    def band_shape(self):
        self._workspace(1)
        return self.heads.cout, self.fh, self.fw

    def head_wire_supported(self, wire: str) -> bool:
        if wire not in L.WIRES:
            raise ValueError(f"wire: one of {sorted(L.WIRES)}, got {wire!r}")
        return wire == "f32" or bool((self.heads.da_np > 0).all())

    def fuse_frames_and_heads_band(self, gathered: torch.Tensor, agent_stride: int, level_stride: int, frame_stride: int, pairwise: torch.Tensor,
                                   n_agents: int, ego: int, frames: int, y0: int, y1: int, out_slab: torch.Tensor, wire: str = "f32"):
        if not self.head_wire_supported(wire):
            raise L.Qv2xError("band wire 'u8': a head without an output quantizer has no codes to send")
        hd, n_cells, esz = self.heads, (y1 - y0) * self.fw, (1 if wire == "u8" else 4)
        if not 0 <= y0 <= y1 <= self.fh:
            raise ValueError(f"band rows [{y0}, {y1}) outside the map's {self.fh} rows")
        if out_slab.dtype != torch.uint8 or out_slab.numel() < frames * hd.cout * n_cells * esz:
            raise ValueError("out_slab: u8, at least frames * cout * band cells * element size bytes")
        if n_cells == 0:
            return
        one_launch = self.band_one_launch
        if one_launch is None:
            one_launch = frames * n_cells // 32 >= self.fuse_heads_min_tiles and n_agents <= self._one_launch_agents()
        rows = None
        if not one_launch:
            key = (frames, n_cells)
            if self._band_rows is None or self._band_rows[0] != key:
                self._band_rows = (key, torch.empty((frames, n_cells, 256), dtype=torch.float32, device=self.dev))
            rows = self._band_rows[1]
        base, st = out_slab.data_ptr(), L.current_stream()
        for s0, n, d, offs, cnts, lut, lb in self._scene_chunks(agent_stride, level_stride, pairwise, [f * frame_stride for f in range(frames)],
                                                                [n_agents] * frames, ego):
            out = C.c_void_p(base + s0 * hd.cout * n_cells * esz)
            if one_launch:
                L.check(self.lib.qv2x_fuse_heads_band(C.byref(d), n, offs, cnts, L.ptr(gathered), lut, lb, None, L.ptr(pairwise[s0]),
                                                      y0 * self.fw, n_cells, hd.cout, hd.cout_pad, L.ptr(hd.w), L.ptr(hd.bias), L.ptr(hd.da),
                                                      L.ptr(hd.za), L.WIRES[wire], L.ptr(hd.da_np), out, None, st), "qv2x_fuse_heads_band")
            else:
                L.check(self.lib.qv2x_fuse_att_band_f32(C.byref(d), n, offs, cnts, L.ptr(gathered), lut, lb, None, L.ptr(pairwise[s0]),
                                                        y0 * self.fw, n_cells, L.ptr(rows[s0]), st), "qv2x_fuse_att_band_f32")
                L.check(self.lib.qv2x_heads_band(L.ptr(rows[s0]), n, n_cells, hd.cout, hd.cout_pad, L.ptr(hd.w), L.ptr(hd.bias),
                                                 L.ptr(hd.da), L.ptr(hd.za), L.WIRES[wire], L.ptr(hd.da_np), out, st), "qv2x_heads_band")

    def assemble_bands(self, gathered_slabs: torch.Tensor, world: int, frames: int, wire: str, out: torch.Tensor):
        hd = self.heads
        L.check(self.lib.qv2x_assemble_bands(L.ptr(gathered_slabs), world, gathered_slabs.shape[1], frames, hd.cout, self.fh, self.fw, L.WIRES[wire],
                                             L.ptr(hd.da), L.ptr(hd.za), L.ptr(out), L.current_stream()), "qv2x_assemble_bands")

    def band_output(self, preds: torch.Tensor, own_codes: Optional[torch.Tensor], frames: int) -> dict:
        out = split_heads(preds, self.heads.splits)
        if own_codes is not None:
            out.update(self.single_preds(own_codes, frames))
        return out

    def decode_rows(self, codes, n_rows_total):
        out = torch.empty((n_rows_total, 256), dtype=torch.float32, device=self.dev)
        L.check(self.lib.qv2x_decode_lut_f32(L.ptr(codes), n_rows_total, self.levels, self.kc, L.ptr(self.lut),
                                             L.ptr(self.lut_bias), L.ptr(out), L.current_stream()), "qv2x_decode_lut_f32")
        return out

    def _fuse_desc(self, agent_stride, level_stride, pairwise_b, n, ego):
        d = L.FuseDesc()
        d.agents, d.h, d.w = n, self.fh, self.fw
        d.levels, d.kc = (self.levels, self.kc) if self.has_codebook else (1, 1)
        d.max_cav, d.ego = pairwise_b.shape[0], ego
        d.code_agent_stride, d.code_level_stride = agent_stride, level_stride
        d.h_metres, d.w_metres, d.discrete_ratio = self.hm, self.wm, self.ratio
        d.fusion = self.fusion
        return d

    def fuse(self, codes_ptr, agent_stride, level_stride, feats, pairwise_b, n, out, ego=0):
        d = self._fuse_desc(agent_stride, level_stride, pairwise_b, n, ego)
        lut, lb = self._lut_ptrs()
        L.check(self.lib.qv2x_fuse_att_f32(C.byref(d), codes_ptr, lut, lb, L.ptr(feats) if feats is not None else None,
                                           L.ptr(pairwise_b), L.ptr(out), L.current_stream()), "qv2x_fuse_att_f32")

    def _lut_ptrs(self):
        return (L.ptr(self.lut), L.ptr(self.lut_bias)) if self.has_codebook else (None, None)

    def _scene_chunks(self, agent_stride, level_stride, pairwise, offsets, counts, ego):
        lut, lb = self._lut_ptrs()
        for s0 in range(0, len(counts), 64):
            s1 = min(len(counts), s0 + 64)
            d = self._fuse_desc(agent_stride, level_stride, pairwise[s0], max(counts[s0:s1]), ego)
            yield s0, s1 - s0, d, (C.c_int64 * (s1 - s0))(*offsets[s0:s1]), (C.c_int32 * (s1 - s0))(*counts[s0:s1]), lut, lb

    def fuse_scenes(self, codes_ptr, agent_stride, level_stride, feats, pairwise, offsets, counts, out, ego=0):
        for s0, n, d, offs, cnts, lut, lb in self._scene_chunks(agent_stride, level_stride, pairwise, offsets, counts, ego):
            L.check(self.lib.qv2x_fuse_att_batch_f32(C.byref(d), n, offs, cnts, codes_ptr, lut, lb,
                                                     L.ptr(feats) if feats is not None else None, L.ptr(pairwise[s0]), L.ptr(out[s0]),
                                                     L.current_stream()), "qv2x_fuse_att_batch_f32")

    def _self_transforms_are_identity(self, pairwise: torch.Tensor) -> bool:
        if pairwise.is_cuda:
            if torch.cuda.is_current_stream_capturing():
                return True
            ref = getattr(self, "_ident_ref", None)
            if ref is not None and ref[0]() is pairwise and ref[1] == pairwise._version:
                return ref[2]
            t00 = pairwise[:, 0, 0].cpu()
        else:
            t00 = pairwise[:, 0, 0]
        ok = bool((t00 == torch.eye(4, dtype=t00.dtype)).all())
        if pairwise.is_cuda:
            import weakref
            self._ident_ref = (weakref.ref(pairwise), pairwise._version, ok)
        return ok

    def _one_launch_agents(self) -> int:
        batched = self.has_codebook and self.levels == 3
        return self.fuse_heads_max_agents if batched else min(self.fuse_heads_max_agents, 1)

    def _table_heads_out(self, codes, n: int) -> dict:
        tab, tb, da, za, c0, c1 = self.table_heads
        hw = self.fh * self.fw
        preds = torch.empty((n, c0, self.fh, self.fw), dtype=torch.float32, device=self.dev)
        sp = torch.empty((n, c1, self.fh, self.fw), dtype=torch.float32, device=self.dev) if c1 else None
        L.check(self.lib.qv2x_table_heads_f32(L.ptr(codes), n * hw, hw, self.levels, self.kc, c0, c1, L.ptr(tab), L.ptr(tb), L.ptr(da), L.ptr(za),
                                              L.ptr(preds), L.ptr(sp) if sp is not None else None, L.current_stream()), "qv2x_table_heads_f32")
        out = split_heads(preds, self.heads.splits)
        if sp is not None:
            out.update(split_heads(sp, self.heads_single.splits, "_single"))
        return out

    def fuse_heads_scenes(self, codes_ptr, agent_stride, level_stride, feats, pairwise, offsets, counts, ego=0, fused_tap=None):
        hd, hw = self.heads, self.fh * self.fw
        out = torch.empty((len(counts), hd.cout, self.fh, self.fw), dtype=torch.float32, device=self.dev)
        for s0, n, d, offs, cnts, lut, lb in self._scene_chunks(agent_stride, level_stride, pairwise, offsets, counts, ego):
            L.check(self.lib.qv2x_fuse_heads_batch_f32(C.byref(d), n, offs, cnts, codes_ptr, lut, lb,
                                                       L.ptr(feats) if feats is not None else None, L.ptr(pairwise[s0]),
                                                       hd.cout, hd.cout_pad, L.ptr(hd.w), L.ptr(hd.bias), L.ptr(hd.da), L.ptr(hd.za), L.ptr(out[s0]),
                                                       L.ptr(fused_tap[s0]) if fused_tap is not None else None, L.current_stream()),
                    "qv2x_fuse_heads_batch_f32")
        return out

    def _post_form(self, lens: List[int], taps: Optional[dict], identity) -> str:
        if (taps is None and self.table_heads is not None and self.single_agent_tables and all(n == 1 for n in lens)
                and (identity() if callable(identity) else identity)):
            return "tables"
        if taps is None and len(lens) * self.fh * self.fw // 32 >= self.fuse_heads_min_tiles and max(lens) <= self._one_launch_agents():
            return "one_launch"
        return "fused"

    def _post(self, form: str, codes_ptr, agent_stride, level_stride, feats, pairwise, offsets, lens: List[int], ego: int,
              own: Optional[torch.Tensor], n_own: int, taps: Optional[dict] = None) -> dict:
        if form == "tables":
            return self._table_heads_out(own, len(lens))
        hw, nb = self.fh * self.fw, len(lens)
        single = self.heads_single is not None and own is not None
        sp = None
        if form == "one_launch":
            preds = self.fuse_heads_scenes(codes_ptr, agent_stride, level_stride, feats, pairwise, offsets, lens, ego)
            if single:
                sp = self._decode_heads_single(own, n_own)
        else:
            fused = torch.empty((nb, hw, 256), dtype=torch.float32, device=self.dev)
            self.fuse_scenes(codes_ptr, agent_stride, level_stride, feats, pairwise, offsets, lens, fused, ego)
            if single:
                preds, sp = self._heads_pair(fused, nb, own, n_own)
            else:
                preds = self._run_heads(self.heads, fused, nb, hw)
            if taps is not None:
                taps["fused"] = fused
        if self.heads_single is not None and sp is None and feats is not None:
            sp = self._run_heads(self.heads_single, feats, sum(lens), hw)
        out = split_heads(preds, self.heads.splits)
        if sp is not None:
            out.update(split_heads(sp, self.heads_single.splits, "_single"))
        return out

    def fuse_and_heads(self, codes, agent_stride, level_stride, pairwise_b, n_agents, ego=0) -> dict:
        return self.fuse_heads_and_single(codes, agent_stride, level_stride, pairwise_b, n_agents, ego, None, 0)

    def _decode_heads_single(self, codes, n_agents: int):
        hw = self.fh * self.fw
        hd = self.heads_single
        sp = torch.empty((n_agents, hd.cout, self.fh, self.fw), dtype=torch.float32, device=self.dev)
        if self.single_by_tables:
            tab, tb = hd.lut_tables
            L.check(self.lib.qv2x_single_heads_lut_f32(L.ptr(codes), n_agents * hw, hw, self.levels, self.kc, hd.cout, L.ptr(tab), L.ptr(tb),
                                                       L.ptr(hd.da), L.ptr(hd.za), L.ptr(sp), L.current_stream()), "qv2x_single_heads_lut_f32")
            return sp
        if self.single_by_global_tables:
            tab, tb = hd.lut_tables
            L.check(self.lib.qv2x_table_heads_f32(L.ptr(codes), n_agents * hw, hw, self.levels, self.kc, hd.cout, 0, L.ptr(tab), L.ptr(tb),
                                                  L.ptr(hd.da), L.ptr(hd.za), L.ptr(sp), None, L.current_stream()), "qv2x_table_heads_f32")
            return sp
        L.check(self.lib.qv2x_decode_heads_f32(L.ptr(codes), n_agents * hw, hw, self.levels, self.kc, L.ptr(self.lut), L.ptr(self.lut_bias),
                                               hd.cout, hd.cout_pad, L.ptr(hd.w), L.ptr(hd.bias), L.ptr(hd.da), L.ptr(hd.za),
                                               L.ptr(sp), L.current_stream()), "qv2x_decode_heads_f32")
        return sp

    def _heads_pair(self, fused, nb, codes, n_agents):
        hw = self.fh * self.fw
        hd, hs = self.heads, self.heads_single
        if self.single_by_tables or self.single_by_global_tables:
            return self._run_heads(hd, fused, nb, hw), self._decode_heads_single(codes, n_agents)
        preds = torch.empty((nb, hd.cout, self.fh, self.fw), dtype=torch.float32, device=self.dev)
        sp = torch.empty((n_agents, hs.cout, self.fh, self.fw), dtype=torch.float32, device=self.dev)
        L.check(self.lib.qv2x_heads_pair_f32(L.ptr(fused), nb * hw, hw, hd.cout, hd.cout_pad, L.ptr(hd.w), L.ptr(hd.bias), L.ptr(hd.da),
                                             L.ptr(hd.za), L.ptr(preds), L.ptr(codes), n_agents * hw, self.levels, self.kc,
                                             L.ptr(self.lut), L.ptr(self.lut_bias), hs.cout, hs.cout_pad, L.ptr(hs.w), L.ptr(hs.bias),
                                             L.ptr(hs.da), L.ptr(hs.za), L.ptr(sp), L.current_stream()), "qv2x_heads_pair_f32")
        return preds, sp

    def fuse_heads_and_single(self, codes, agent_stride, level_stride, pairwise_b, n_agents, ego, own_codes, n_own: int = 1) -> dict:
        pairwise = pairwise_b.to(torch.float64).contiguous()[None]
        return self._post("fused", L.ptr(codes), agent_stride, level_stride, None, pairwise, [0], [n_agents], ego, own_codes, n_own)

    def single_preds(self, codes, n_agents: int) -> dict:
        if self.heads_single is None:
            return {}
        return split_heads(self._decode_heads_single(codes, n_agents), self.heads_single.splits, "_single")

    @torch.no_grad()
    def forward(self, data_dict: dict, taps: Optional[dict] = None) -> dict:
        agents = data_dict["agent_modality_list"]
        n_total = len(agents)
        if any(a != "m1" for a in agents):
            raise NotImplementedError("deployed path: every agent is the LiDAR modality 'm1' (a heterogeneous model deploys as DeployedHeterModel)")
        enc = self.encode_agents(data_dict["inputs_m1"], n_total, taps)
        return self.finish(enc, n_total, data_dict, taps)

    @torch.no_grad()
    def finish(self, enc, n_total: int, data_dict: dict, taps: Optional[dict] = None) -> dict:
        pairwise, lens = scene_layout(data_dict, n_total)
        hw = self.fh * self.fw
        feats = None if self.has_codebook else self._shared_features(enc, n_total)
        form = self._post_form(lens, taps, lambda: self._self_transforms_are_identity(data_dict["pairwise_t_matrix"]))
        if form != "tables" and not pairwise.is_cuda:
            if torch.cuda.is_current_stream_capturing():
                raise ValueError("pairwise_t_matrix on the host cannot be uploaded during HIP-graph capture: pass a device tensor")
            pairwise = pairwise.to(self.dev)
        starts = [sum(lens[:bi]) for bi in range(len(lens))]
        if self.has_codebook:
            out = self._post(form, L.ptr(enc), hw, n_total * hw, None, pairwise, [st * hw for st in starts], lens, 0, enc, n_total, taps)
        else:
            out = self._post(form, None, 0, 0, feats, pairwise, [st * hw * 256 for st in starts], lens, 0, None, n_total, taps)
        if taps is not None:
            taps["codes"] = enc if self.has_codebook else None
            taps["features"] = feats
        return out

    def capture(self, data_dict: dict):
        return capture_forward(self, data_dict)


class DeployedModel(DeployedPostStage):

    def __init__(self, state: Dict[str, np.ndarray], device="cuda", emit_single_preds: Optional[bool] = None):
        super().__init__(state, device, emit_single_preds)
        s, dev = state, self.dev

        self.encoder_kind = str(s["meta/encoder"]) if "meta/encoder" in s else "point_pillar"
        if self.encoder_kind == "second":
            last = int(s["second/n_layers"]) - 1
            q = (float(np.float32(s[f"second/{last}/a_delta"])), int(s[f"second/{last}/a_zp"]))
            self.canvas_c, self.canvas_q, self.pfn = int(s["meta/canvas_channels"]), q, None
            self.second: Dict[int, object] = {}
            self.second_max_voxels, self.second_max_points = 70000, 5
        else:
            self.pfn, q = pfn_params(s)
            self.canvas_c, self.canvas_q = 64, q

        self.blocks: List[List[_ConvLayer]] = []
        self.chains: List[Optional[_ChainLayers]] = []
        self.deblocks: List[_DeconvLayer] = []
        cat_groups, c0 = [], 0
        cin = self.canvas_c
        for lvl in range(len(self.layer_nums)):
            convs = []
            for i in range(self.layer_nums[lvl] + 1):
                layer = _ConvLayer(s, f"backbone_m1.blocks.{lvl}.{i + 1}", [(0, cin, q[0], q[1])],
                                   self.strides[lvl] if i == 0 else 1, dev)
                convs.append(layer)
                q, cin = layer.out_q, layer.cout
            self.blocks.append(convs)
            self.chains.append(_ChainLayers(convs, dev) if _ChainLayers.eligible(convs) else None)
            de = _DeconvLayer(s, f"backbone_m1.deblocks.{lvl}.0", q, dev)
            self.deblocks.append(de)
            cat_groups.append((c0, de.cout, de.out_q[0], de.out_q[1]))
            c0 += de.cout
        self.cat_channels = c0
        self.shrink0 = _ConvLayer(s, "shrinker_m1.layers.0.double_conv.0", cat_groups, 1, dev)
        self.shrink1 = _ConvLayer(s, "shrinker_m1.layers.0.double_conv.1",
                                  [(0, self.shrink0.cout, *self.shrink0.out_q)], 1, dev)
        if self.shrink1.cout != 256:
            raise NotImplementedError("deployed path expects a 256-channel shared feature")
        self.compress = bool(s.get("meta/compress", False))
        self.final = self.shrink1
        if self.compress:
            if self.has_codebook:
                raise NotImplementedError("deployed path: compressor and codebook together")
            narrow = int(s["compressor.encoder.0/w_code"].shape[0])
            pad = (narrow + 63) // 64 * 64
            self.comp = [_ConvLayer(s, "compressor.encoder.0", [(0, 256, *self.shrink1.out_q)], 1, dev, pad_cout=pad)]
            self.comp.append(_ConvLayer(s, "compressor.decoder.0", [(0, pad, *self.comp[0].out_q)], 1, dev, pad_cin=pad))
            self.comp.append(_ConvLayer(s, "compressor.decoder.1", [(0, 256, *self.comp[1].out_q)], 1, dev))
            self.comp_channels = narrow
            self.final = self.comp[-1]
        self._set_heads(_Heads(s, "", dev), _Heads(s, "_single", dev) if (self.emit_single and "cls_head_single/w_code" in s) else None,
                        tables=True)
        self._bufs: Dict[int, dict] = {}
        self.use_wide_conv, self.batch_deconvs, self.use_chains = True, True, True
        self.chain_max_agents = 1
        self._collapsed, self._two_stage, self.two_stage_refused = None, None, None
        self.encode_form = "auto"
        self.encode_mode = "two_stage" if self.two_stage_supported() else "exact"

    def _padded(self, n, h, w, c, q):
        t = torch.empty((n, h + 2, w + 2, c), dtype=torch.int8, device=self.dev)
        t.fill_(int(q[1]) - 128)
        return t

    def _workspace(self, n: int) -> dict:
        if n in self._bufs:
            return self._bufs[n]
        b = {}
        h, w = self.ny, self.nx
        if self.encoder_kind == "second":
            from .engine_second import DeployedSecondEncoder
            self.second[n] = DeployedSecondEncoder(self.state, self.dev, agents=n, max_voxels=self.second_max_voxels, max_points=self.second_max_points)
            b["canvas"] = self.second[n].bev
        else:
            b["canvas"] = self._padded(n, h, w, 64, self.canvas_q)
        b["lvl"] = []
        for lvl, convs in enumerate(self.blocks):
            h, w = (h + 2 - 3) // self.strides[lvl] + 1, (w + 2 - 3) // self.strides[lvl] + 1
            zps = {c.out_q[1] for c in convs}
            if len(zps) != 1:
                raise NotImplementedError("conv outputs of one backbone level must share a zero point (post-ReLU: 0)")
            pair = [self._padded(n, h, w, convs[0].cout, convs[0].out_q) for _ in range(2)]
            b["lvl"].append((pair, h, w))
        (_, h0, w0) = b["lvl"][0]
        self.fh, self.fw = h0 * self.ups[0], w0 * self.ups[0]
        for lvl, (_, hl, wl) in enumerate(b["lvl"]):
            if (hl * self.ups[lvl], wl * self.ups[lvl]) != (self.fh, self.fw):
                raise ValueError(f"deblock {lvl} upsamples {hl}x{wl} by {self.ups[lvl]} to {hl * self.ups[lvl]}x{wl * self.ups[lvl]}, "
                                 f"level 0 gives {self.fh}x{self.fw}: the grid does not line up across backbone levels")
        cat = torch.empty((n, self.fh + 2, self.fw + 2, self.cat_channels), dtype=torch.int8, device=self.dev)
        c0 = 0
        for de in self.deblocks:
            cat[..., c0:c0 + de.cout] = int(de.out_q[1]) - 128
            c0 += de.cout
        b["cat"] = cat
        b["s0"] = self._padded(n, self.fh, self.fw, self.shrink0.cout, self.shrink0.out_q)
        b["s1"] = self._padded(n, self.fh, self.fw, self.shrink1.cout, self.shrink1.out_q)
        if self.compress:
            b["comp"] = [self._padded(n, self.fh, self.fw, c.cout, c.out_q) for c in self.comp]
        hw = self.fh * self.fw
        if self.has_codebook:
            b["codes"] = torch.empty((self.levels, n, hw), dtype=torch.uint8, device=self.dev)
        if self.two_stage_supported():
            if self._two_stage is None and self.encode_mode == "two_stage":
                self._build_two_stage()
            b["enc_list"] = torch.zeros(3 * n * hw, dtype=torch.int32, device=self.dev)
            b["enc_counters"] = torch.zeros(4, dtype=torch.int32, device=self.dev)
        if not self.has_codebook or self.heads_single is not None:
            b["feats"] = torch.empty((n, hw, 256), dtype=torch.float32, device=self.dev)
        self._bufs[n] = b
        return b

    def _conv(self, layer: _ConvLayer, x, n, h, w, out, out_ctotal=None, out_c0=0):
        d = L.ConvDesc()
        d.n, d.h, d.w, d.cin_total, d.stride, d.cout = n, h, w, x.shape[-1], layer.stride, layer.cout
        d.ngroups = len(layer.groups)
        for i, (c0, c, zx) in enumerate(layer.groups):
            d.group_c0[i], d.group_c[i], d.group_zx[i] = c0, c, zx
        d.out_ctotal = out.shape[-1] if out_ctotal is None else out_ctotal
        d.out_c0, d.relu = out_c0, 1
        d.out_delta, d.out_zp = layer.out_q[0], float(layer.out_q[1])
        if self.use_wide_conv and self.lib.qv2x_conv3x3_i8_wide_ok(C.byref(d)):
            if layer.w_wide is None:
                layer.w_wide = torch.empty_like(layer.w)
                L.check(self.lib.qv2x_conv3x3_i8_pack_wide(C.byref(d), L.ptr(layer.w), L.ptr(layer.w_wide), L.current_stream()), layer.name)
            L.check(self.lib.qv2x_conv3x3_i8_wide(C.byref(d), L.ptr(x), L.ptr(layer.w_wide), L.ptr(layer.scale), L.ptr(layer.corr),
                                                  L.ptr(layer.aw), L.ptr(layer.bias), L.ptr(out), L.current_stream()), layer.name)
            return
        L.check(self.lib.qv2x_conv3x3_i8(C.byref(d), L.ptr(x), L.ptr(layer.w), L.ptr(layer.scale), L.ptr(layer.corr),
                                         L.ptr(layer.aw), L.ptr(layer.bias), L.ptr(out), L.current_stream()), layer.name)

    def _chain(self, ch: _ChainLayers, x, n, h, w, out):
        d = L.ChainDesc()
        d.n, d.in_h, d.in_w = n, h, w
        d.h, d.w = out.shape[1] - 2, out.shape[2] - 2
        d.depth, d.stride0, d.relu = len(ch.convs), ch.stride0, 1
        for i, c in enumerate(ch.convs):
            d.out_delta[i], d.out_zp[i] = c.out_q[0], float(c.out_q[1])
        L.check(self.lib.qv2x_conv3x3_i8_chain64(C.byref(d), L.ptr(x), L.ptr(ch.w), L.ptr(ch.scale), L.ptr(ch.corr), L.ptr(ch.aw),
                                                 L.ptr(ch.bias), L.ptr(out), L.current_stream()), ch.name)

    def _deconv_desc(self, de: _DeconvLayer, n, h, w, out, out_c0):
        d = L.DeconvDesc()
        d.n, d.h, d.w, d.cin, d.cout, d.s = n, h, w, de.cin, de.cout, de.s
        d.in_zx, d.in_delta = int(de.in_q[1]), float(de.in_q[0])
        d.out_ctotal, d.out_c0, d.relu = out.shape[-1], out_c0, 1
        d.out_delta, d.out_zp = de.out_q[0], float(de.out_q[1])
        d.out_h, d.out_w = out.shape[1] - 2, out.shape[2] - 2
        return d

    def _deconv(self, de: _DeconvLayer, x, n, h, w, out, out_c0):
        d = self._deconv_desc(de, n, h, w, out, out_c0)
        L.check(self.lib.qv2x_deconv_i8(C.byref(d), L.ptr(x), L.ptr(de.w), L.ptr(de.bias), L.ptr(out), L.current_stream()), de.name)

    def _deconv_batch(self, items, n):
        k = len(items)
        descs = (L.DeconvDesc * k)(*[self._deconv_desc(de, n, h, w, out, c0) for (de, x, h, w, out, c0) in items])
        arr = lambda ts: (C.c_void_p * k)(*[t.data_ptr() for t in ts])
        L.check(self.lib.qv2x_deconv_i8_batch(descs, k, arr([it[1] for it in items]), arr([it[0].w for it in items]),
                                              arr([it[0].bias for it in items]), arr([it[4] for it in items]), L.current_stream()),
                "qv2x_deconv_i8_batch")

    def conv_plan(self, n_agents: int):
        b = self._workspace(n_agents)
        use_chains = self.use_chains and n_agents <= self.chain_max_agents
        key = ("plan", use_chains)
        if key in b:
            return b[key]
        plan = []
        x, h, w, c0 = b["canvas"], self.ny, self.nx, 0
        for lvl, convs in enumerate(self.blocks):
            pair, ho, wo = b["lvl"][lvl]
            macs = [n_agents * ho * wo * layer.cout * layer.w.shape[1] for layer in convs]
            if use_chains and self.chains[lvl] is not None:
                out = pair[(len(convs) - 1) % 2]
                plan.append(("chain", self.chains[lvl], x, h, w, out, 0, sum(macs)))
                x, h, w = out, ho, wo
            else:
                for i, layer in enumerate(convs):
                    out = pair[i % 2]
                    plan.append(("conv", layer, x, h, w, out, 0, macs[i]))
                    x, h, w = out, ho, wo
            de = self.deblocks[lvl]
            plan.append(("deconv", de, x, h, w, b["cat"], c0, n_agents * h * w * de.cin * de.cout * de.s * de.s))
            c0 += de.cout
        hw = n_agents * self.fh * self.fw
        plan.append(("conv", self.shrink0, b["cat"], self.fh, self.fw, b["s0"], 0, hw * self.shrink0.cout * self.shrink0.w.shape[1]))
        plan.append(("conv", self.shrink1, b["s0"], self.fh, self.fw, b["s1"], 0, hw * self.shrink1.cout * self.shrink1.w.shape[1]))
        if self.compress:
            x = b["s1"]
            for c, out in zip(self.comp, b["comp"]):
                plan.append(("conv", c, x, self.fh, self.fw, out, 0, hw * c.cout * c.w.shape[1]))
                x = out
        b[key] = plan
        return plan

    def run_plan(self, n_agents: int, only=None, taps: Optional[dict] = None):
        pending = []

        def flush():
            if len(pending) == 1:
                de, x, h, w, out, c0 = pending[0]
                self._deconv(de, x, n_agents, h, w, out, c0)
            elif pending:
                self._deconv_batch(pending, n_agents)
            pending.clear()

        for (kind, layer, x, h, w, out, c0, _) in self.conv_plan(n_agents):
            if only is not None and not only(kind, layer):
                continue
            if kind == "chain":
                self._chain(layer, x, n_agents, h, w, out)
                if taps is not None:
                    taps[layer.name] = out.clone()
            elif kind == "conv":
                if layer is self.shrink0:
                    flush()
                self._conv(layer, x, n_agents, h, w, out)
                if taps is not None:
                    taps[layer.name] = out.clone()
            else:
                pending.append((layer, x, h, w, out, c0))
                if not self.batch_deconvs:
                    flush()
        flush()

    def pillars_to_canvas(self, inputs: dict, n_agents: int, resident: bool = False):
        b = self._workspace(n_agents)
        st = L.current_stream()
        vf, co, npnt = pillar_inputs(inputs, pfn=self.encoder_kind != "second")
        if self.encoder_kind == "second":
            return self.second[n_agents]({"voxel_features": vf, "voxel_coords": co, "voxel_num_points": npnt})
        canvas = b["canvas"]
        capturing = torch.cuda.is_current_stream_capturing()
        if not resident and b.get("fill_less_graphs", False):
            raise L.Qv2xError("pillars_to_canvas(resident=False) on a workspace whose captured graphs rely on the clean resident canvas: "
                              "use resident=True + clear_pillars, or another DeployedModel")
        if not (resident and b.get("canvas_clean", False)):
            L.check(self.lib.qv2x_fill_i8(L.ptr(canvas), canvas.numel(), int(self.pfn.z2) - 128, st), "qv2x_fill_i8")
        elif capturing:
            b["fill_less_graphs"] = True
        b["canvas_clean"] = False
        L.check(self.lib.qv2x_pfn_scatter_i8(L.ptr(vf), L.ptr(co), L.ptr(npnt), vf.shape[0], 32, C.byref(self.pfn),
                                             L.ptr(canvas), n_agents, self.ny, self.nx, st), "qv2x_pfn_scatter_i8")
        return canvas

    def _restore_canvas(self, n_agents: int):
        b = self._workspace(n_agents)
        if self.encoder_kind != "second" and not torch.cuda.is_current_stream_capturing():
            L.check(self.lib.qv2x_fill_i8(L.ptr(b["canvas"]), b["canvas"].numel(), int(self.pfn.z2) - 128, L.current_stream()), "qv2x_fill_i8")
            b["canvas_clean"] = True

    def clear_pillars(self, inputs: dict, n_agents: int):
        if self.encoder_kind == "second":
            return
        b = self._workspace(n_agents)
        co = inputs["voxel_coords"].to(torch.int32).contiguous()
        L.check(self.lib.qv2x_pfn_unscatter_i8(L.ptr(co), co.shape[0], int(self.pfn.z2) - 128, L.ptr(b["canvas"]), n_agents, self.ny, self.nx,
                                               L.current_stream()), "qv2x_pfn_unscatter_i8")
        b["canvas_clean"] = True

    def encode_codes(self, n_agents: int, out: Optional[torch.Tensor] = None):
        b = self._workspace(n_agents)
        codes = b["codes"] if out is None else out
        if codes.dtype != torch.uint8 or not codes.is_contiguous() or codes.numel() != self.levels * n_agents * self.fh * self.fw:
            raise ValueError("encode_codes: out must be a contiguous uint8 tensor [levels, n_agents, H*W]")
        d = L.EncodeDesc()
        d.n, d.h, d.w, d.levels, d.kc, d.segs = n_agents, self.fh, self.fw, self.enc_levels, self.kc, self.segs
        d.in_zx, d.in_delta = int(self.shrink1.out_q[1]), float(self.shrink1.out_q[0])
        two_stage = self.encode_mode == "two_stage" and self.encode_form == "auto"
        if two_stage and self._two_stage is None:
            self._refuse_during_capture("encode_mode 'two_stage'")
            self._build_two_stage()
            two_stage = self.encode_mode == "two_stage"
        if self.encode_mode == "collapsed":
            if self.segs != 1 or self.kc > 128:
                raise NotImplementedError("encode_mode 'collapsed': seg_num 1 and dict_size <= 128 (the exact encode takes the rest)")
            if self._collapsed is None:
                self._refuse_during_capture("encode_mode 'collapsed'")
                self._collapsed = tuple(_dev(t, self.dev) for t in collapse_encoder(self.state, self.enc_levels, d.in_delta, d.in_zx))
            gp, bias, tab = self._collapsed
            L.check(self.lib.qv2x_codebook_encode_collapsed_f32(C.byref(d), L.ptr(b["s1"]), L.ptr(gp), L.ptr(bias), L.ptr(tab), L.ptr(codes),
                                                                L.current_stream()), "qv2x_codebook_encode_collapsed_f32")
            return codes
        if two_stage:
            return self._encode_two_stage(d, b, codes)
        if self.encode_mode not in ("exact", "two_stage"):
            raise ValueError(f"encode_mode {self.encode_mode!r}: 'exact' (every cell through the reference's op order), 'two_stage' (the same "
                             "indices: exact integer candidates, the chain only where the bound cannot decide) or 'collapsed' (opt-in, approximate)")
        if self.encode_form == "wave":
            L.check(self.lib.qv2x_codebook_encode_wave_f32(C.byref(d), L.ptr(b["s1"]), None, self.level_ptrs, L.ptr(codes),
                                                           L.current_stream()), "qv2x_codebook_encode_wave_f32")
            return codes
        L.check(self.lib.qv2x_codebook_encode_f32(C.byref(d), L.ptr(b["s1"]), self.level_ptrs, L.ptr(codes),
                                                  L.current_stream()), "qv2x_codebook_encode_f32")
        return codes

    def two_stage_supported(self) -> bool:
        if not self.has_codebook or self.enc_levels > 3 or self.kc > 256:
            return False
        return bool(self.kc % 32 == 0 if self.segs == 1 else self.segs == 2 and self.kc % 64 == 0)

    def _refuse_during_capture(self, what: str):
        if torch.cuda.is_current_stream_capturing():
            raise L.Qv2xError(f"{what}: its operands are built on the host and uploaded -- not inside a HIP-graph capture; encode once "
                              "in this mode before capturing")

    def _build_two_stage(self):
        if not self.two_stage_supported():
            raise NotImplementedError("encode_mode 'two_stage': seg_num 1 | 2, dict_size <= 256, up to three levels (encode_mode 'exact' takes the rest)")
        from .encode_two_stage import candidate_tables
        try:
            t = candidate_tables(self.state, self.enc_levels, float(self.shrink1.out_q[0]), int(self.shrink1.out_q[1]), self.segs)
            k = np.arange(t["bias"].shape[0], dtype=np.int64) % self.kc
            pf = int(t["pack"])
            packed = (pf * t["bias"] + k).astype(np.float64)
            if not np.array_equal(packed.astype(np.int64), pf * t["bias"] + k):
                raise ValueError("two-stage encode: packed scores not exact in float64")
            self._two_stage = (_dev(t["gpack"], self.dev), _dev(packed, self.dev), _dev(t["tables"], self.dev),
                               (C.c_float * (3 * self.enc_levels))(*[float(v) for v in t["tau"].reshape(-1)]), t)
        except Exception as e:
            self.encode_mode, self.two_stage_refused = "exact", str(e) or type(e).__name__

    def candidate_entry(self) -> str:
        from .encode_two_stage import CANDIDATE_ENTRY, pack_factor
        return CANDIDATE_ENTRY[pack_factor(self.segs, self.kc)]

    def _encode_two_stage(self, d, b, codes):
        gp, bias, tab, tau, _ = self._two_stage
        name = self.candidate_entry()
        L.check(getattr(self.lib, name)(C.byref(d), L.ptr(b["s1"]), L.ptr(gp), L.ptr(bias), L.ptr(tab), tau, L.ptr(codes),
                                        L.ptr(b["enc_list"]), L.ptr(b["enc_counters"]), L.current_stream()), name)
        L.check(self.lib.qv2x_codebook_encode_listed_f32(C.byref(d), L.ptr(b["s1"]), self.level_ptrs, L.ptr(b["enc_list"]), L.ptr(b["enc_counters"]),
                                                         L.ptr(codes), L.current_stream()), "qv2x_codebook_encode_listed_f32")
        return codes

    def encode_refine_stats(self, n_agents: int) -> dict:
        if not (self.encode_mode == "two_stage" and self.encode_form == "auto") or "enc_counters" not in self._bufs.get(n_agents, {}):
            raise L.Qv2xError(f"encode_refine_stats({n_agents}): no two-stage encode of {n_agents} frames here (encode_mode "
                              f"{self.encode_mode!r}, encode_form {self.encode_form!r}, workspaces {sorted(self._bufs)})")
        c = self._bufs[n_agents]["enc_counters"].cpu().numpy().astype(np.int64)
        cells = n_agents * self.fh * self.fw
        return {"cells": cells, "refined": int(c[0]), "refined_fraction": float(c[0]) / cells, "first_flagged_at_level": [int(v) for v in c[1:1 + self.enc_levels]]}

    def encode_into(self, inputs: dict, frames: int, codes_out: torch.Tensor):
        self.pillars_to_canvas(inputs, frames, resident=True)
        try:
            self.run_plan(frames)
            self.clear_pillars(inputs, frames)
        except BaseException:
            self._restore_canvas(frames)
            raise
        return self.encode_codes(frames, out=codes_out)

    def encode_agents(self, inputs: dict, n_agents: int, taps: Optional[dict] = None):
        b = self._workspace(n_agents)
        canvas = self.pillars_to_canvas(inputs, n_agents, resident=True)
        try:
            self.run_plan(n_agents, taps=taps)
            if taps is not None:
                taps["canvas"], taps["cat"] = canvas.clone(), b["cat"]
            self.clear_pillars(inputs, n_agents)
        except BaseException:
            self._restore_canvas(n_agents)
            raise
        if taps is not None:
            taps[self.shrink0.name], taps[self.shrink1.name] = b["s0"], b["s1"]
        if taps is not None and self.compress:
            for c, out in zip(self.comp, b["comp"]):
                taps[c.name] = out
        return self.encode_codes(n_agents) if self.has_codebook else (b["comp"][-1] if self.compress else b["s1"])

    def _shared_features(self, shrinker_out, n_total: int):
        q = self.final.out_q
        feats = self._workspace(n_total)["feats"]
        L.check(self.lib.qv2x_dequant_i8_f32(L.ptr(shrinker_out), n_total, self.fh, self.fw, 256, int(q[1]), float(q[0]), L.ptr(feats),
                                             L.current_stream()), "qv2x_dequant_i8_f32")
        return feats


class DeployedHeterModel(nn.Module):

    def __init__(self, states: Dict[str, Dict[str, np.ndarray]], ego_modality: Optional[str] = None, device="cuda", **kw):
        super().__init__()
        if not states:
            raise ValueError("DeployedHeterModel: no modality")
        self.engines = {m: DeployedModel(st, device=device, **kw) for m, st in states.items()}
        self.main = self.engines[ego_modality if ego_modality in self.engines else next(iter(self.engines))]
        for m, e in self.engines.items():
            e._workspace(1)
            if not e.has_codebook:
                raise NotImplementedError("deployed heterogeneous path: codebook models (the code planes are what the modalities share)")
            if (e.fh, e.fw, e.levels, e.kc) != (self.main.fh, self.main.fw, self.main.levels, self.main.kc):
                raise ValueError(f"modality {m}: feature map {e.fh} x {e.fw} / codebook {e.levels} x {e.kc} differs from the ego modality's")
        self.dev = self.main.dev
        self._slots: Dict[tuple, Dict[str, torch.Tensor]] = {}

    @torch.no_grad()
    def forward(self, data_dict: dict, taps: Optional[dict] = None) -> dict:
        agents = list(data_dict["agent_modality_list"])
        enc = assemble_heter_codes("DeployedHeterModel", self.engines, self._slots, agents, data_dict,
                                   lambda eng, inputs, k, mt: eng.encode_agents(inputs, k, mt), taps)
        return self.main.finish(enc, len(agents), data_dict, taps)

    def capture(self, data_dict: dict):
        return capture_forward(self, data_dict)


def deploy_heter(qt_model, device="cuda", **kw) -> DeployedHeterModel:
    model = qt_model.model if hasattr(qt_model, "model") else qt_model
    states = {m: export_ptq_state(qt_model, modality=m) for m in model.modality_name_list}
    return DeployedHeterModel(states, ego_modality=getattr(model, "ego_modality", None), device=device, **kw)


def deploy(qt_model=None, state: Optional[Dict[str, np.ndarray]] = None, path: Optional[str] = None,
           device="cuda", **kw) -> DeployedModel:
    if state is None:
        if path is not None:
            state = load_ptq_state(path)
        elif any(hasattr(m, "weight_quantizer") for m in qt_model.modules()):
            inner = qt_model.model if hasattr(qt_model, "model") else qt_model
            if len(getattr(inner, "modality_name_list", ["m1"])) > 1:
                if hasattr(inner, "pyramid_backbone"):
                    from .engine_pyramid import deploy_heter_pyramid
                    return deploy_heter_pyramid(qt_model, device=device)
                return deploy_heter(qt_model, device=device, **kw)
            state = export_ptq_state(qt_model)
        elif hasattr(qt_model, "pyramid_backbone"):
            from .engine_pyramid_fp32 import export_fp32_pyramid_state
            state = export_fp32_pyramid_state(qt_model)
        else:
            from .engine_fp32 import export_fp32_state
            state = export_fp32_state(qt_model)
    if str(state.get("meta/mode", "w8a8")) == "fp32":
        if str(state.get("meta/fusion_method", "att")) == "pyramid":
            from .engine_pyramid_fp32 import DeployedPyramidFp32Model
            return DeployedPyramidFp32Model(state, device=device, **kw)
        from .engine_fp32 import DeployedFp32Model
        return DeployedFp32Model(state, device=device, **kw)
    if str(state.get("meta/fusion_method", "att")) == "pyramid":
        from .engine_pyramid import DeployedPyramidModel
        return DeployedPyramidModel(state, device=device, **kw)
    return DeployedModel(state, device=device, **kw)
```

### quantv2x_amd/lib.py

```python
from __future__ import annotations

import ctypes as C
import os

_HERE = os.path.dirname(os.path.abspath(__file__))
LIB_PATH = os.path.join(_HERE, "libqv2x.so")
MAX_GROUPS = 4
ABI_VERSION = 9

SYMBOLS = [
    "qv2x_last_error", "qv2x_version", "qv2x_fill_i8", "qv2x_pfn_scatter_i8", "qv2x_pfn_unscatter_i8", "qv2x_conv3x3_i8",
    "qv2x_conv3x3_i8_wide_ok", "qv2x_conv3x3_i8_pack_wide", "qv2x_conv3x3_i8_wide", "qv2x_conv3x3_i8_chain64",
    "qv2x_deconv_i8", "qv2x_deconv_i8_batch", "qv2x_codebook_level_floats", "qv2x_codebook_c2_f32", "qv2x_codebook_encode_f32", "qv2x_codebook_encode_wave_f32", "qv2x_fuse_att_f32", "qv2x_fuse_att_batch_f32", "qv2x_fuse_heads_batch_f32",
    "qv2x_decode_lut_f32", "qv2x_single_heads_lut_f32", "qv2x_table_heads_f32", "qv2x_dequant_i8_f32", "qv2x_heads_f32", "qv2x_decode_heads_f32", "qv2x_heads_pair_f32", "qv2x_voxelize_workspace_bytes", "qv2x_voxelize_f32",
    "qv2x_postprocess_workspace_bytes", "qv2x_postprocess_f32", "qv2x_postprocess_late_workspace_bytes", "qv2x_postprocess_late_f32",
    "qv2x_conv3x3_f32", "qv2x_deconv_f32", "qv2x_pfn_scatter_f32", "qv2x_codebook_encode_f32in",
    "qv2x_pyramid_weighted_fuse_f32", "qv2x_pyramid_weighted_fuse_i8", "qv2x_conv1x1_i8", "qv2x_gconv3x3_i8", "qv2x_conv3x3_i8_res",
    "qv2x_deconv_f32in", "qv2x_codebook_decode_f32", "qv2x_occ_score_i8",
    "qv2x_codebook64_level_floats", "qv2x_codebook64_c2_f32", "qv2x_codebook_encode64_f32", "qv2x_codebook_encode64_f32in",
    "qv2x_add_relu_f32", "qv2x_occ_sigmoid_f32", "qv2x_pyramid_weighted_fuse_f32p", "qv2x_bottleneck_i8",
    "qv2x_comm_unique_id", "qv2x_comm_init", "qv2x_comm_destroy", "qv2x_allgather_codes", "qv2x_pairwise_from_poses_f64", "qv2x_pairwise_from_poses_batch_f64",
    "qv2x_codebook_encode_collapsed_f32", "qv2x_codebook_encode_candidates_i8", "qv2x_codebook_encode_candidates_seg_i8", "qv2x_codebook_encode_listed_f32", "qv2x_mean_vfe_f32", "qv2x_sp_index_scatter", "qv2x_sp_out_sites_workspace_bytes", "qv2x_sp_out_sites", "qv2x_sp_rulebook", "qv2x_sp_conv_f32in", "qv2x_sp_conv_i8", "qv2x_sp_to_bev_i8",
    "qv2x_fuse_att_band_f32", "qv2x_heads_band", "qv2x_fuse_heads_band", "qv2x_assemble_bands",
    "qv2x_voxelize_batch_workspace_bytes", "qv2x_voxelize_batch_f32", "qv2x_postprocess_batch_workspace_bytes", "qv2x_postprocess_batch_f32",
    "qv2x_eval_workspace_bytes", "qv2x_eval_tp_fp_f32", "qv2x_gt_boxes_f32",
    "qv2x_range_search_workspace_bytes", "qv2x_range_search_f32",
    "qv2x_lss_workspace_bytes", "qv2x_lss_plan_f32", "qv2x_lss_splat_f32",
]
WIRES = {"f32": 0, "u8": 1}
COMM_ID_BYTES = 128


class PfnParams(C.Structure):
    _fields_ = [("w", C.c_float * 640), ("b", C.c_float * 64),
                ("d1", C.c_float), ("z1", C.c_float), ("d2", C.c_float), ("z2", C.c_float),
                ("vox", C.c_float * 3), ("off", C.c_float * 3)]


class ConvDesc(C.Structure):
    _fields_ = [("n", C.c_int32), ("h", C.c_int32), ("w", C.c_int32), ("cin_total", C.c_int32),
                ("stride", C.c_int32), ("cout", C.c_int32), ("ngroups", C.c_int32),
                ("group_c0", C.c_int32 * MAX_GROUPS), ("group_c", C.c_int32 * MAX_GROUPS),
                ("group_zx", C.c_int32 * MAX_GROUPS),
                ("out_ctotal", C.c_int32), ("out_c0", C.c_int32), ("relu", C.c_int32),
                ("out_delta", C.c_float), ("out_zp", C.c_float)]


class ChainDesc(C.Structure):
    _fields_ = [("n", C.c_int32), ("h", C.c_int32), ("w", C.c_int32), ("in_h", C.c_int32), ("in_w", C.c_int32),
                ("depth", C.c_int32), ("stride0", C.c_int32), ("relu", C.c_int32),
                ("out_delta", C.c_float * 4), ("out_zp", C.c_float * 4)]


class DeconvDesc(C.Structure):
    _fields_ = [("n", C.c_int32), ("h", C.c_int32), ("w", C.c_int32), ("cin", C.c_int32), ("cout", C.c_int32),
                ("s", C.c_int32), ("in_zx", C.c_int32), ("in_delta", C.c_float),
                ("out_ctotal", C.c_int32), ("out_c0", C.c_int32), ("relu", C.c_int32),
                ("out_delta", C.c_float), ("out_zp", C.c_float), ("out_h", C.c_int32), ("out_w", C.c_int32)]


class F32ConvDesc(C.Structure):
    _fields_ = [("n", C.c_int32), ("h", C.c_int32), ("w", C.c_int32), ("cin_total", C.c_int32), ("cin0", C.c_int32), ("cin", C.c_int32),
                ("stride", C.c_int32), ("cout", C.c_int32), ("out_ctotal", C.c_int32), ("out_c0", C.c_int32), ("relu", C.c_int32)]


class Conv1x1Desc(C.Structure):
    _fields_ = [("n", C.c_int32), ("h", C.c_int32), ("w", C.c_int32), ("cin", C.c_int32), ("cout", C.c_int32), ("stride", C.c_int32),
                ("mode", C.c_int32), ("relu", C.c_int32), ("out_ctotal", C.c_int32), ("out_c0", C.c_int32),
                ("out_delta", C.c_float), ("out_zp", C.c_float), ("res_zx", C.c_int32), ("res_delta", C.c_float)]


class BottleneckDesc(C.Structure):
    _fields_ = [("n", C.c_int32), ("h", C.c_int32), ("w", C.c_int32), ("planes", C.c_int32), ("width", C.c_int32), ("cg", C.c_int32),
                ("in_zx", C.c_int32), ("in_delta", C.c_float), ("delta1", C.c_float), ("zp1", C.c_float), ("delta2", C.c_float), ("zp2", C.c_float),
                ("out_delta", C.c_float), ("out_zp", C.c_float)]


class GconvDesc(C.Structure):
    _fields_ = [("n", C.c_int32), ("h", C.c_int32), ("w", C.c_int32), ("c", C.c_int32), ("cg", C.c_int32), ("stride", C.c_int32),
                ("relu", C.c_int32), ("out_delta", C.c_float), ("out_zp", C.c_float)]


class SpconvDesc(C.Structure):
    _fields_ = [("subm", C.c_int32), ("k", C.c_int32 * 3), ("s", C.c_int32 * 3), ("p", C.c_int32 * 3),
                ("in_shape", C.c_int32 * 3), ("out_shape", C.c_int32 * 3), ("agents", C.c_int32), ("cin", C.c_int32), ("cout", C.c_int32),
                ("cap_in", C.c_int32), ("cap_out", C.c_int32), ("out_delta", C.c_float), ("out_zp", C.c_float)]


class OccDesc(C.Structure):
    _fields_ = [("n", C.c_int32), ("h", C.c_int32), ("w", C.c_int32), ("c", C.c_int32), ("aw", C.c_int32), ("corr", C.c_int32),
                ("scale", C.c_float), ("bias", C.c_float), ("out_delta", C.c_float), ("out_zp", C.c_float)]


class EncodeDesc(C.Structure):
    _fields_ = [("n", C.c_int32), ("h", C.c_int32), ("w", C.c_int32), ("levels", C.c_int32), ("kc", C.c_int32),
                ("in_zx", C.c_int32), ("in_delta", C.c_float), ("segs", C.c_int32)]


class FuseDesc(C.Structure):
    _fields_ = [("agents", C.c_int32), ("h", C.c_int32), ("w", C.c_int32), ("levels", C.c_int32), ("kc", C.c_int32),
                ("max_cav", C.c_int32), ("ego", C.c_int32),
                ("code_agent_stride", C.c_int64), ("code_level_stride", C.c_int64),
                ("h_metres", C.c_double), ("w_metres", C.c_double), ("discrete_ratio", C.c_double), ("fusion", C.c_int32)]


class PostprocessDesc(C.Structure):
    _fields_ = [("h", C.c_int32), ("w", C.c_int32), ("anchors_per_cell", C.c_int32), ("num_bins", C.c_int32),
                ("score_threshold", C.c_float), ("nms_threshold", C.c_float), ("dir_offset", C.c_float),
                ("range", C.c_float * 6), ("transform", C.c_float * 16), ("max_boxes", C.c_int32),
                ("num_classes", C.c_int32), ("range_xy_only", C.c_int32),
                ("max_extent", C.c_float), ("z_min", C.c_float), ("z_max", C.c_float)]


class EvalDesc(C.Structure):
    _fields_ = [("frames", C.c_int32), ("det_cap", C.c_int32), ("gt_cap", C.c_int32), ("n_classes", C.c_int32), ("n_ranges", C.c_int32),
                ("n_thresholds", C.c_int32), ("ranges", (C.c_float * 2) * 4), ("thresholds", C.c_float * 4)]


class GtDesc(C.Structure):
    _fields_ = [("frames", C.c_int32), ("agents", C.c_int32), ("obj_cap", C.c_int32), ("gt_cap", C.c_int32), ("row_floats", C.c_int32),
                ("order", C.c_int32), ("mode", C.c_int32), ("range_xy_only", C.c_int32), ("range", C.c_float * 6), ("iou_threshold", C.c_float)]


class RangeSearchDesc(C.Structure):
    _fields_ = [("channels", C.c_int32), ("candidates", C.c_int32), ("n_levels", C.c_int32), ("reserved", C.c_int32), ("per_channel", C.c_int64)]


class LssDesc(C.Structure):
    _fields_ = [("samples", C.c_int32), ("views", C.c_int32), ("depth_bins", C.c_int32), ("fh", C.c_int32), ("fw", C.c_int32),
                ("features", C.c_int32), ("nx", C.c_int32 * 3), ("dx", C.c_float * 3), ("bx", C.c_float * 3)]


class Qv2xError(RuntimeError):
    pass


_lib = None


def load() -> C.CDLL:
    global _lib
    if _lib is not None:
        return _lib
    if not os.path.exists(LIB_PATH):
        raise Qv2xError(f"{LIB_PATH} is missing: build it with `python -c 'import __graft_entry__ as g; g.build()'` "
                        "(hipcc --offload-arch=gfx950).  There is no CPU fallback for the deployed path.")
    lib = C.CDLL(LIB_PATH)
    missing = [s for s in SYMBOLS if not hasattr(lib, s)]
    if missing:
        raise Qv2xError(f"libqv2x.so does not export {missing}")
    vp = C.c_void_p
    lib.qv2x_last_error.restype = C.c_char_p
    lib.qv2x_version.restype = C.c_int
    if lib.qv2x_version() != ABI_VERSION:
        raise Qv2xError(f"libqv2x.so has ABI {lib.qv2x_version()}, this binding mirrors ABI {ABI_VERSION} (include/qv2x.h): rebuild the library")
    lib.qv2x_fill_i8.argtypes = [vp, C.c_int64, C.c_int, vp]
    lib.qv2x_pfn_scatter_i8.argtypes = [vp, vp, vp, C.c_int, C.c_int, C.POINTER(PfnParams), vp, C.c_int, C.c_int, C.c_int, vp]
    lib.qv2x_pfn_unscatter_i8.argtypes = [vp, C.c_int, C.c_int, vp, C.c_int, C.c_int, C.c_int, vp]
    lib.qv2x_conv3x3_i8.argtypes = [C.POINTER(ConvDesc), vp, vp, vp, vp, vp, vp, vp, vp]
    lib.qv2x_conv3x3_i8_wide.argtypes = [C.POINTER(ConvDesc), vp, vp, vp, vp, vp, vp, vp, vp]
    lib.qv2x_conv3x3_i8_chain64.argtypes = [C.POINTER(ChainDesc), vp, vp, vp, vp, vp, vp, vp, vp]
    lib.qv2x_conv3x3_i8_pack_wide.argtypes = [C.POINTER(ConvDesc), vp, vp, vp]
    lib.qv2x_conv3x3_i8_wide_ok.argtypes = [C.POINTER(ConvDesc)]
    lib.qv2x_deconv_i8.argtypes = [C.POINTER(DeconvDesc), vp, vp, vp, vp, vp]
    lib.qv2x_deconv_i8_batch.argtypes = [C.POINTER(DeconvDesc), C.c_int, C.POINTER(vp), C.POINTER(vp), C.POINTER(vp), C.POINTER(vp), vp]
    lib.qv2x_codebook_level_floats.argtypes = [C.c_int]
    lib.qv2x_codebook_level_floats.restype = C.c_int64
    lib.qv2x_codebook_c2_f32.argtypes = [vp, C.c_int, vp, vp]
    lib.qv2x_codebook_encode_f32.argtypes = [C.POINTER(EncodeDesc), vp, C.POINTER(vp), vp, vp]
    lib.qv2x_codebook_encode_wave_f32.argtypes = [C.POINTER(EncodeDesc), vp, vp, C.POINTER(vp), vp, vp]
    lib.qv2x_fuse_att_f32.argtypes = [C.POINTER(FuseDesc), vp, vp, vp, vp, vp, vp, vp]
    lib.qv2x_fuse_att_batch_f32.argtypes = [C.POINTER(FuseDesc), C.c_int, C.POINTER(C.c_int64), C.POINTER(C.c_int32), vp, vp, vp, vp, vp, vp, vp]
    lib.qv2x_decode_lut_f32.argtypes = [vp, C.c_int, C.c_int, C.c_int, vp, vp, vp, vp]
    lib.qv2x_fuse_heads_batch_f32.argtypes = [C.POINTER(FuseDesc), C.c_int, C.POINTER(C.c_int64), C.POINTER(C.c_int32), vp, vp, vp, vp, vp,
                                              C.c_int, C.c_int, vp, vp, vp, vp, vp, vp, vp]
    lib.qv2x_heads_f32.argtypes = [vp, C.c_int, C.c_int, C.c_int, C.c_int, vp, vp, vp, vp, vp, vp]
    lib.qv2x_decode_heads_f32.argtypes = [vp, C.c_int, C.c_int, C.c_int, C.c_int, vp, vp, C.c_int, C.c_int, vp, vp, vp, vp, vp, vp]
    lib.qv2x_table_heads_f32.argtypes = [vp, C.c_int, C.c_int, C.c_int, C.c_int, C.c_int, C.c_int, vp, vp, vp, vp, vp, vp, vp]
    lib.qv2x_single_heads_lut_f32.argtypes = [vp, C.c_int, C.c_int, C.c_int, C.c_int, C.c_int, vp, vp, vp, vp, vp, vp]
    lib.qv2x_heads_pair_f32.argtypes = [vp, C.c_int, C.c_int, C.c_int, C.c_int, vp, vp, vp, vp, vp,
                                        vp, C.c_int, C.c_int, C.c_int, vp, vp, C.c_int, C.c_int, vp, vp, vp, vp, vp, vp]
    lib.qv2x_dequant_i8_f32.argtypes = [vp, C.c_int, C.c_int, C.c_int, C.c_int, C.c_int, C.c_float, vp, vp]
    lib.qv2x_codebook_encode_collapsed_f32.argtypes = [C.POINTER(EncodeDesc), vp, vp, vp, vp, vp, vp]
    lib.qv2x_codebook_encode_candidates_i8.argtypes = [C.POINTER(EncodeDesc), vp, vp, vp, vp, C.POINTER(C.c_float), vp, vp, vp, vp]
    lib.qv2x_codebook_encode_candidates_seg_i8.argtypes = [C.POINTER(EncodeDesc), vp, vp, vp, vp, C.POINTER(C.c_float), vp, vp, vp, vp]
    lib.qv2x_codebook_encode_listed_f32.argtypes = [C.POINTER(EncodeDesc), vp, C.POINTER(vp), vp, vp, vp, vp]
    lib.qv2x_mean_vfe_f32.argtypes = [vp, vp, vp, C.c_int, C.c_int, vp, vp]
    lib.qv2x_sp_index_scatter.argtypes = [vp, vp, C.c_int, C.c_int, C.c_int, C.c_int, C.c_int, vp, C.c_int, vp]
    lib.qv2x_sp_out_sites_workspace_bytes.argtypes = [C.POINTER(SpconvDesc)]
    lib.qv2x_sp_out_sites_workspace_bytes.restype = C.c_int64
    lib.qv2x_sp_out_sites.argtypes = [C.POINTER(SpconvDesc), vp, vp, vp, vp, vp, vp, C.c_int64, vp]
    lib.qv2x_sp_rulebook.argtypes = [C.POINTER(SpconvDesc), vp, vp, vp, vp, vp]
    lib.qv2x_sp_conv_f32in.argtypes = [C.POINTER(SpconvDesc), vp, vp, vp, vp, vp, vp, vp, vp]
    lib.qv2x_sp_conv_i8.argtypes = [C.POINTER(SpconvDesc), vp, vp, vp, vp, vp, vp, vp, vp, vp, vp, vp]
    lib.qv2x_sp_to_bev_i8.argtypes = [vp, vp, vp, C.c_int, C.c_int, C.c_int, C.c_int, C.c_int, C.c_int, C.c_int, C.c_int, vp, vp]
    lib.qv2x_voxelize_workspace_bytes.argtypes = [C.c_int]
    lib.qv2x_voxelize_workspace_bytes.restype = C.c_int64
    lib.qv2x_voxelize_f32.argtypes = [vp, C.c_int, C.POINTER(C.c_float), C.POINTER(C.c_float), C.c_int, C.c_int, C.c_int,
                                      vp, C.c_int64, vp, vp, vp, vp, vp]
    lib.qv2x_voxelize_batch_workspace_bytes.argtypes = [C.c_int, C.POINTER(C.c_int32)]
    lib.qv2x_voxelize_batch_workspace_bytes.restype = C.c_int64
    lib.qv2x_voxelize_batch_f32.argtypes = [C.POINTER(vp), C.POINTER(C.c_int32), C.c_int, C.POINTER(C.c_float), C.POINTER(C.c_float),
                                            C.c_int, C.c_int, C.c_int, vp, C.c_int64, vp, vp, vp, vp, vp]
    lib.qv2x_postprocess_batch_workspace_bytes.argtypes = [C.POINTER(PostprocessDesc), C.c_int]
    lib.qv2x_postprocess_batch_workspace_bytes.restype = C.c_int64
    lib.qv2x_postprocess_batch_f32.argtypes = [C.POINTER(PostprocessDesc), C.c_int, vp, C.c_int64, vp, C.c_int64, vp, C.c_int64, vp, vp,
                                               vp, C.c_int64, vp, vp, vp, vp, vp]
    lib.qv2x_eval_workspace_bytes.argtypes = [C.POINTER(EvalDesc)]
    lib.qv2x_eval_workspace_bytes.restype = C.c_int64
    lib.qv2x_eval_tp_fp_f32.argtypes = [C.POINTER(EvalDesc), vp, vp, vp, vp, vp, vp, vp, vp, C.c_int64, vp, vp, vp, vp, vp, vp]
    lib.qv2x_gt_boxes_f32.argtypes = [C.POINTER(GtDesc), vp, vp, vp, vp, vp, vp, vp, vp, vp, vp, vp]
    lib.qv2x_range_search_workspace_bytes.argtypes = [C.POINTER(RangeSearchDesc)]
    lib.qv2x_range_search_workspace_bytes.restype = C.c_int64
    lib.qv2x_range_search_f32.argtypes = [C.POINTER(RangeSearchDesc), vp, vp, vp, vp, vp, vp, vp]
    lib.qv2x_lss_workspace_bytes.argtypes = [C.POINTER(LssDesc)]
    lib.qv2x_lss_workspace_bytes.restype = C.c_int64
    lib.qv2x_lss_plan_f32.argtypes = [C.POINTER(LssDesc), vp, vp, vp, vp, vp, vp, vp, vp, vp]
    lib.qv2x_lss_splat_f32.argtypes = [C.POINTER(LssDesc), vp, vp, C.c_int, vp, vp, vp]
    lib.qv2x_postprocess_workspace_bytes.argtypes = [C.POINTER(PostprocessDesc)]
    lib.qv2x_postprocess_workspace_bytes.restype = C.c_int64
    lib.qv2x_postprocess_f32.argtypes = [C.POINTER(PostprocessDesc), vp, vp, vp, vp, vp, C.c_int64, vp, vp, vp, vp, vp]
    lib.qv2x_postprocess_late_workspace_bytes.argtypes = [C.POINTER(PostprocessDesc), C.c_int]
    lib.qv2x_postprocess_late_workspace_bytes.restype = C.c_int64
    lib.qv2x_postprocess_late_f32.argtypes = [C.POINTER(PostprocessDesc), C.c_int, C.POINTER(vp), C.POINTER(vp), C.POINTER(vp), C.POINTER(vp),
                                              C.POINTER(C.c_float), vp, C.c_int64, vp, vp, vp, vp, vp]
    lib.qv2x_conv3x3_f32.argtypes = [C.POINTER(F32ConvDesc), vp, vp, vp, vp, vp]
    lib.qv2x_deconv_f32.argtypes = [C.POINTER(F32ConvDesc), vp, vp, vp, vp, vp]
    lib.qv2x_pfn_scatter_f32.argtypes = [vp, vp, vp, C.c_int, C.c_int, C.POINTER(C.c_float), C.POINTER(C.c_float), C.POINTER(C.c_float),
                                         C.POINTER(C.c_float), vp, C.c_int, C.c_int, C.c_int, vp]
    lib.qv2x_codebook_encode_f32in.argtypes = [C.POINTER(EncodeDesc), vp, C.POINTER(vp), vp, vp]
    lib.qv2x_pyramid_weighted_fuse_f32.argtypes = [C.POINTER(FuseDesc), C.c_int, vp, vp, vp, vp, vp]
    lib.qv2x_pyramid_weighted_fuse_i8.argtypes = [C.POINTER(FuseDesc), C.c_int, vp, C.c_int, C.c_float, vp, vp, vp, vp]
    lib.qv2x_conv1x1_i8.argtypes = [C.POINTER(Conv1x1Desc), vp, vp, vp, vp, vp, vp, vp, vp, vp]
    lib.qv2x_gconv3x3_i8.argtypes = [C.POINTER(GconvDesc), vp, vp, vp, vp, vp, vp, vp, vp]
    lib.qv2x_conv3x3_i8_res.argtypes = [C.POINTER(ConvDesc), vp, vp, vp, vp, vp, vp, C.c_int, vp, C.c_int, C.c_float, vp, vp]
    lib.qv2x_deconv_f32in.argtypes = [C.POINTER(DeconvDesc), vp, vp, vp, vp, vp]
    lib.qv2x_codebook_decode_f32.argtypes = [vp, C.c_int64, C.c_int64, C.c_int, C.c_int, C.c_int, C.c_int, C.c_int, vp, vp, vp, vp]
    lib.qv2x_occ_score_i8.argtypes = [C.POINTER(OccDesc), vp, vp, vp, vp, vp, vp]
    lib.qv2x_codebook64_level_floats.argtypes = [C.c_int]
    lib.qv2x_codebook64_level_floats.restype = C.c_int64
    lib.qv2x_codebook64_c2_f32.argtypes = [vp, C.c_int, vp, vp]
    lib.qv2x_codebook_encode64_f32.argtypes = [C.POINTER(EncodeDesc), C.c_int, vp, C.POINTER(vp), vp, vp]
    lib.qv2x_codebook_encode64_f32in.argtypes = [C.POINTER(EncodeDesc), C.c_int, vp, C.POINTER(vp), vp, vp]
    lib.qv2x_add_relu_f32.argtypes = [vp, vp, vp, C.c_int64, vp]
    lib.qv2x_occ_sigmoid_f32.argtypes = [vp, C.c_int, C.c_int, C.c_int, C.c_int, vp, vp, vp]
    lib.qv2x_pyramid_weighted_fuse_f32p.argtypes = [C.POINTER(FuseDesc), C.c_int, vp, vp, vp, vp, vp]
    lib.qv2x_bottleneck_i8.argtypes = [C.POINTER(BottleneckDesc), vp, C.POINTER(vp), C.POINTER(vp), C.POINTER(vp), C.POINTER(vp), C.POINTER(vp), vp, vp]
    lib.qv2x_comm_unique_id.argtypes = [vp]
    lib.qv2x_comm_init.argtypes = [vp, C.c_int, C.c_int, C.POINTER(vp)]
    lib.qv2x_comm_destroy.argtypes = [vp]
    lib.qv2x_allgather_codes.argtypes = [vp, vp, vp, C.c_int64, vp]
    lib.qv2x_pairwise_from_poses_f64.argtypes = [vp, C.c_int, C.c_int64, C.c_int64, C.c_int, vp, vp]
    lib.qv2x_pairwise_from_poses_batch_f64.argtypes = [vp, C.c_int, C.c_int64, C.c_int64, C.c_int, C.c_int64, C.c_int, vp, vp]
    lib.qv2x_fuse_att_band_f32.argtypes = [C.POINTER(FuseDesc), C.c_int, C.POINTER(C.c_int64), C.POINTER(C.c_int32), vp, vp, vp, vp, vp,
                                           C.c_int64, C.c_int64, vp, vp]
    lib.qv2x_heads_band.argtypes = [vp, C.c_int, C.c_int64, C.c_int, C.c_int, vp, vp, vp, vp, C.c_int, vp, vp, vp]
    lib.qv2x_fuse_heads_band.argtypes = [C.POINTER(FuseDesc), C.c_int, C.POINTER(C.c_int64), C.POINTER(C.c_int32), vp, vp, vp, vp, vp,
                                         C.c_int64, C.c_int64, C.c_int, C.c_int, vp, vp, vp, vp, C.c_int, vp, vp, vp, vp]
    lib.qv2x_assemble_bands.argtypes = [vp, C.c_int, C.c_int64, C.c_int, C.c_int, C.c_int, C.c_int, C.c_int, vp, vp, vp, vp]
    for s in SYMBOLS:
        if s not in ("qv2x_last_error", "qv2x_codebook_level_floats", "qv2x_codebook64_level_floats", "qv2x_voxelize_workspace_bytes", "qv2x_postprocess_workspace_bytes",
                     "qv2x_postprocess_late_workspace_bytes", "qv2x_sp_out_sites_workspace_bytes", "qv2x_voxelize_batch_workspace_bytes",
                     "qv2x_postprocess_batch_workspace_bytes", "qv2x_eval_workspace_bytes", "qv2x_range_search_workspace_bytes", "qv2x_lss_workspace_bytes"):
            getattr(lib, s).restype = C.c_int
    _lib = lib
    return lib


def check(rc: int, what: str = "") -> None:
    if rc != 0:
        msg = load().qv2x_last_error().decode(errors="replace")
        raise Qv2xError(f"{what or 'libqv2x'} failed with {rc}: {msg}")


def ptr(t) -> C.c_void_p:
    if t is None:
        return C.c_void_p(0)
    if hasattr(t, "data_ptr"):
        return C.c_void_p(t.data_ptr())
    return C.c_void_p(t.ctypes.data)


def current_stream() -> C.c_void_p:
    import torch
    return C.c_void_p(torch.cuda.current_stream().cuda_stream)
```

Baseline: 6804.

## Classify refine candidates by first/last flagged level span and stop refinement early

The candidate pass now records both the first and last level at which a cell is weakly resolved, and buckets cells into up to six span classes instead of three first-level classes. The listed refinement kernel re-encodes only from the first to the last flagged level. It stops early when no code changed at the stop level, and defers tiles whose codes changed to a full-depth pass in the tail kernel. This is meant to skip exact refinement of levels that don't need it, at the cost of per-row dirty checks (extra code reads and a shared flag), more counters and lists, and a deferred-work queue.

```diff
diff --git a/include/qv2x.h b/include/qv2x.h
--- a/include/qv2x.h
+++ b/include/qv2x.h
@@ -112,6 +112,15 @@
 int qv2x_codebook_encode_candidates_seg_i8(const qv2x_encode_desc* desc , const int8_t* in, const int8_t* g_limbs, const double* bias_packed,
                                            const int32_t* tables, const float* tau , uint8_t* codes, uint32_t* list, uint32_t* counters,
                                            void* stream);
+
+int qv2x_codebook_encode_candidates_span_i8(const qv2x_encode_desc* desc , const int8_t* in, const int8_t* g_limbs, const double* bias_packed,
+                                            const int32_t* tables, const float* tau , uint8_t* codes, uint32_t* list, uint32_t* counters,
+                                            void* stream);
+int qv2x_codebook_encode_candidates_seg_span_i8(const qv2x_encode_desc* desc , const int8_t* in, const int8_t* g_limbs,
+                                                const double* bias_packed, const int32_t* tables, const float* tau , uint8_t* codes,
+                                                uint32_t* list, uint32_t* counters, void* stream);
+int qv2x_codebook_encode_listed_span_f32(const qv2x_encode_desc* desc , const int8_t* in, const float* const* level_weights ,
+                                         uint32_t* list, uint32_t* counters, uint8_t* codes, void* stream);
 
 typedef struct {
     int32_t agents, h, w, levels, kc;
diff --git a/quantv2x_amd/csrc/codebook_encode.h b/quantv2x_amd/csrc/codebook_encode.h
--- a/quantv2x_amd/csrc/codebook_encode.h
+++ b/quantv2x_amd/csrc/codebook_encode.h
@@ -15,25 +15,49 @@
     int m_lo, m_hi;
     int list_slots = 1, list_tail_max = 0;
     const unsigned* list = nullptr; const unsigned* list_count = nullptr;
+    int span = 0;
+    unsigned* defer = nullptr; unsigned* defer_count = nullptr;
 };
 
 __device__ __host__ __forceinline__ int64_t level_floats_wg(int kc) { return 3LL * (ENC_D * ENC_D + ENC_D) + (int64_t)ENC_D * kc + (int64_t)kc * ENC_D + kc; }
 __device__ __host__ __forceinline__ int64_t level_floats(int kc) { return level_floats_wg(kc) + 3LL * ENC_D * ENC_D + (int64_t)((kc + 63) / 64 * 64) * ENC_D + ENC_WAVE_PAD; }
 
-struct ListPlan { int n[3], first[3], total, full; };
+struct ListPlan { int n0, n1, n2, n3, n4, n5, ncls, total, full; };
+__device__ __forceinline__ int list_count_of(const EncArgs& a, int c, int ncls) {
+    return c < ncls ? __builtin_amdgcn_readfirstlane((int)a.list_count[1 + c]) : 0;
+}
 __device__ __forceinline__ ListPlan list_plan(const EncArgs& a) {
     ListPlan p;
-    int t = 0;
-#pragma unroll
-    for (int c = 0; c < 3; ++c) { p.n[c] = (int)a.list_count[1 + c]; p.first[c] = t; t += (p.n[c] + 31) >> 5; }
-    p.total = t;
-    const int full = t / a.list_slots * a.list_slots;
-    p.full = t - full > a.list_tail_max ? t : full;
+    p.ncls = a.span ? a.levels * (a.levels + 1) / 2 : 3;
+    p.n0 = list_count_of(a, 0, p.ncls); p.n1 = list_count_of(a, 1, p.ncls); p.n2 = list_count_of(a, 2, p.ncls);
+    p.n3 = list_count_of(a, 3, p.ncls); p.n4 = list_count_of(a, 4, p.ncls); p.n5 = list_count_of(a, 5, p.ncls);
+    p.total = ((p.n0 + 31) >> 5) + ((p.n1 + 31) >> 5) + ((p.n2 + 31) >> 5) + ((p.n3 + 31) >> 5) + ((p.n4 + 31) >> 5) + ((p.n5 + 31) >> 5);
+    const int full = p.total / a.list_slots * a.list_slots;
+    p.full = p.total - full > a.list_tail_max ? p.total : full;
     return p;
 }
-__device__ __forceinline__ void list_tile(const ListPlan& p, int tile, int& cls, int& i0) {
-    cls = tile >= p.first[2] ? 2 : (tile >= p.first[1] ? 1 : 0);
-    i0 = (tile - p.first[cls]) * 32;
+struct ListTile { int cls, i0, n, start, stop; };
+__device__ __forceinline__ void list_tile_step(ListTile& t, int& lo, int& f, const int tile, const int c, const int n_prev, const int n_c) {
+    lo += (n_prev + 31) >> 5;
+    if (tile >= lo) { t.cls = c; f = lo; t.n = n_c; }
+}
+__device__ __forceinline__ ListTile list_tile(const EncArgs& a, const ListPlan& p, int tile) {
+    ListTile t{0, 0, p.n0, 0, 0};
+    int lo = 0, f = 0;
+    list_tile_step(t, lo, f, tile, 1, p.n0, p.n1);
+    list_tile_step(t, lo, f, tile, 2, p.n1, p.n2);
+    list_tile_step(t, lo, f, tile, 3, p.n2, p.n3);
+    list_tile_step(t, lo, f, tile, 4, p.n3, p.n4);
+    list_tile_step(t, lo, f, tile, 5, p.n4, p.n5);
+    t.i0 = (tile - f) * 32;
+    if (a.span) {
+        const int r = p.ncls - t.cls;
+        t.stop = r > 3 ? 2 : (r > 1 ? 1 : 0);
+        t.start = (t.stop + 1) * (t.stop + 2) / 2 - r;
+    } else {
+        t.start = t.cls; t.stop = a.levels - 1;
+    }
+    return t;
 }
 
 int encode_wave_launch(const EncArgs& a, hipStream_t st);
diff --git a/quantv2x_amd/csrc/codebook_encode.hip b/quantv2x_amd/csrc/codebook_encode.hip
--- a/quantv2x_amd/csrc/codebook_encode.hip
+++ b/quantv2x_amd/csrc/codebook_encode.hip
@@ -100,11 +100,11 @@
 }
 
 constexpr int ENC_MAX_TILES = 16;
-template <int ER> constexpr int enc_smem_floats() { return 2 * ER * LDF + 4 * ER + 4 * ER + 2 * ENC_MAX_TILES * ER + 4 * ER + QV2X_ENC_LDS_PAD; }
+template <int ER> constexpr int enc_smem_floats() { return 2 * ER * LDF + 4 * ER + 4 * ER + 2 * ENC_MAX_TILES * ER + 4 * ER + 4 + QV2X_ENC_LDS_PAD; }
 
 template <int ER, bool EXT, bool LIST = false>
 __device__ __forceinline__ void encode_rows(const EncArgs& a, const int m0, float* __restrict__ smem, const unsigned* __restrict__ lst = nullptr,
-                                            const int n_listed = 0, const int start = 0) {
+                                            const int n_listed = 0, const int start = 0, const int stop = 0) {
     constexpr int ERT = ER / 32;
     const int segs = EXT ? a.segs : 1;
     float* bufA = smem;
@@ -113,6 +113,8 @@
     float* pval = x2 + 4 * ER;
     unsigned long long* pkey = (unsigned long long*)(pval + 4 * ER);
     int* code_s = (int*)(pkey + ENC_MAX_TILES * ER);
+    int* dirty_s = code_s + 4 * ER;
+    bool dirty = false;
 
     const int tid = threadIdx.x, lane = tid & 63, wave = tid >> 6;
 #ifdef QV2X_ENC_TRACE
@@ -152,6 +154,7 @@
         }
     }
     GemmHead head = gemm_head((const float2*)a.lvl[0], a.lvl[0] + D * D, wave, lane);
+    if (LIST && threadIdx.x == 0) dirty_s[0] = 0;
     lds_barrier();
 
     v16f acc[ERT];
@@ -305,12 +308,20 @@
                 const int bi = (int)(unsigned)bk;
                 code_s[sg * ER + tid] = bi;
                 if (LIST) {
-                    if (m0 + tid < n_listed) a.codes[((size_t)l * segs + sg) * a.M + lst[m0 + tid]] = (uint8_t)(bi - sg * a.kc);
+                    if (m0 + tid < n_listed) {
+                        uint8_t* at = a.codes + ((size_t)l * segs + sg) * a.M + lst[m0 + tid];
+                        if ((int)*at != bi - sg * a.kc) dirty_s[0] = 1;
+                        *at = (uint8_t)(bi - sg * a.kc);
+                    }
                 } else if (m0 + tid < a.m_hi) a.codes[((size_t)l * segs + sg) * a.M + m0 + tid] = (uint8_t)(bi - sg * a.kc);
             }
         }
         lds_barrier();
         EFINE(9);
+        if (LIST) {
+            dirty |= dirty_s[0] != 0;
+            if (l == stop && !dirty) break;
+        }
         }
 
         if (l + 1 < a.levels) {
@@ -350,12 +361,14 @@
 __global__ __launch_bounds__(512, 2) void codebook_encode_list_tail_kernel(const EncArgs a) {
     __shared__ __attribute__((aligned(16))) float smem[enc_smem_floats<32>()];
     const ListPlan plan = list_plan(a);
-    for (int t = plan.full + (int)blockIdx.x; t < plan.total; t += (int)gridDim.x) {
-        int cls, i0;
-        list_tile(plan, t, cls, i0);
-        encode_rows<32, EXT, true>(a, i0, smem, a.list + (size_t)cls * a.M, plan.n[cls], cls);
+    const int nd = a.defer ? __builtin_amdgcn_readfirstlane((int)a.defer_count[0]) : 0, items = nd + plan.total - plan.full;
+    for (int i = (int)blockIdx.x; i < items; i += (int)gridDim.x) {
+        const int t = i < nd ? (int)a.defer[i] : plan.full + i - nd;
+        const ListTile lt = list_tile(a, plan, t);
+        encode_rows<32, EXT, true>(a, lt.i0, smem, a.list + (size_t)lt.cls * a.M, lt.n, lt.start, i < nd ? a.levels - 1 : lt.stop);
         __syncthreads();
     }
+    if (a.defer && threadIdx.x == 0 && atomicAdd(a.defer_count + 1, 1u) == gridDim.x - 1) { a.defer_count[0] = 0; a.defer_count[1] = 0; }
 }
 
 template <bool EXT>
@@ -408,9 +421,11 @@
     return encode_launch(d, (const int8_t*)in, in, level_weights, codes, stream);
 }
 
-extern "C" int qv2x_codebook_encode_listed_f32(const qv2x_encode_desc* d, const int8_t* in, const float* const* level_weights,
-                                               const uint32_t* list, const uint32_t* list_count, uint8_t* codes, void* stream) {
+static int encode_listed(const int span, const qv2x_encode_desc* d, const int8_t* in, const float* const* level_weights,
+                         const uint32_t* list, const uint32_t* list_count, uint8_t* codes, void* stream, uint32_t* defer = nullptr,
+                         uint32_t* defer_count = nullptr) {
     using namespace qv2x;
+    if (span && d && d->levels > 3) return fail(QV2X_EINVAL, "qv2x_codebook_encode_listed_span_f32: up to three levels (got %d)", d->levels);
     if (!d || !in || !level_weights || !codes || !list || !list_count) return fail(QV2X_EINVAL, "qv2x_codebook_encode_listed_f32: null pointer");
     if (d->n <= 0 || d->h <= 0 || d->w <= 0 || d->levels < 1 || d->levels > 4) return fail(QV2X_EINVAL, "qv2x_codebook_encode_listed_f32: bad shape");
     const int segs = d->segs ? d->segs : 1;
@@ -423,7 +438,7 @@
     a.segs = segs; a.ke = segs * d->kc;
     const bool ext = segs > 1 || a.ke > 128;
     a.ax = 128 - d->in_zx; a.dx = d->in_delta; a.M = d->n * d->h * d->w; a.m_lo = 0; a.m_hi = a.M;
-    a.list = list; a.list_count = list_count;
+    a.list = list; a.list_count = list_count; a.span = span; a.defer = defer; a.defer_count = defer_count;
     for (int l = 0; l < 4; ++l) {
         a.lvl[l] = l < d->levels ? level_weights[l] : nullptr;
         if (l < d->levels && (!a.lvl[l] || ((uintptr_t)a.lvl[l] & 15))) return fail(QV2X_EALIGN, "qv2x_codebook_encode_listed_f32: level %d weights null or unaligned", l);
@@ -446,6 +461,17 @@
     if (ext) codebook_encode_list_tail_kernel<true><<<tiles < grid_tail ? tiles : grid_tail, 512, 0, (hipStream_t)stream>>>(a);
     else codebook_encode_list_tail_kernel<false><<<tiles < grid_tail ? tiles : grid_tail, 512, 0, (hipStream_t)stream>>>(a);
     return hip_check(hipGetLastError(), "qv2x_codebook_encode_listed_f32 launch");
+}
+
+extern "C" int qv2x_codebook_encode_listed_f32(const qv2x_encode_desc* d, const int8_t* in, const float* const* level_weights,
+                                               const uint32_t* list, const uint32_t* list_count, uint8_t* codes, void* stream) {
+    return encode_listed(0, d, in, level_weights, list, list_count, codes, stream);
+}
+
+extern "C" int qv2x_codebook_encode_listed_span_f32(const qv2x_encode_desc* d, const int8_t* in, const float* const* level_weights,
+                                                    uint32_t* list, uint32_t* counters, uint8_t* codes, void* stream) {
+    if (!d || !list || !counters) return qv2x::fail(QV2X_EINVAL, "qv2x_codebook_encode_listed_span_f32: null pointer");
+    return encode_listed(1, d, in, level_weights, list, counters, codes, stream, list + 6 * (size_t)d->n * d->h * d->w, counters + 7);
 }
 
 static int encode_launch(const qv2x_encode_desc* d, const int8_t* in, const float* in_f32, const float* const* level_weights, uint8_t* codes, void* stream,
diff --git a/quantv2x_amd/csrc/codebook_encode_cand.hip b/quantv2x_amd/csrc/codebook_encode_cand.hip
--- a/quantv2x_amd/csrc/codebook_encode_cand.hip
+++ b/quantv2x_amd/csrc/codebook_encode_cand.hip
@@ -8,6 +8,7 @@
     uint8_t* codes; unsigned* list; unsigned* counters;
     float tau[3][3];
     int n, h, w, hw, M, levels, kc, ke, zx, gbytes, tbytes;
+    int span;
     float delta;
 };
 
@@ -65,9 +66,9 @@
     const __amdgpu_buffer_rsrc_t brs = __builtin_amdgcn_make_buffer_rsrc((void*)a.bias, 0, a.levels * a.ke * 8, 0x00020000);
     const __amdgpu_buffer_rsrc_t trs = __builtin_amdgcn_make_buffer_rsrc((void*)a.tables, 0, a.tbytes, 0x00020000);
     int o[2][SEGS][CT] = {};
-    int first[CT];
-#pragma unroll
-    for (int ct = 0; ct < CT; ++ct) first[ct] = 3;
+    int fl[CT];
+#pragma unroll
+    for (int ct = 0; ct < CT; ++ct) fl[ct] = 3;
     const int ntile = a.kc >> 5;
     const int tsz = a.ke * a.ke;
     auto level = [&](auto lc) __attribute__((always_inline)) {
@@ -156,48 +157,54 @@
         if constexpr (SEGS > 1) segment(IC<1>{});
 #pragma unroll
         for (int ct = 0; ct < CT; ++ct)
-            if (weak_l[ct] && first[ct] == 3) first[ct] = l;
+            if (weak_l[ct]) fl[ct] = (fl[ct] & 3) == 3 ? (l | l << 2) : ((fl[ct] & 3) | l << 2);
     };
     level(IC<0>{});
     if (a.levels > 1) level(IC<1>{});
     if (a.levels > 2) level(IC<2>{});
-    unsigned long long mask[3][CT];
-    unsigned cnt[3] = {0, 0, 0};
-#pragma unroll
-    for (int c = 0; c < 3; ++c)
-#pragma unroll
-        for (int ct = 0; ct < CT; ++ct) {
-            mask[c][ct] = __builtin_amdgcn_ballot_w64(first[ct] == c && hf == 0 && m[ct] < a.M);
-            cnt[c] += (unsigned)__builtin_popcountll(mask[c][ct]);
-        }
-    __shared__ unsigned wcnt[4][3], wbase[3];
-    if (lane == 0) { wcnt[wave][0] = cnt[0]; wcnt[wave][1] = cnt[1]; wcnt[wave][2] = cnt[2]; }
+    constexpr int NCLS = 6;
+    const int ncls = a.span ? a.levels * (a.levels + 1) / 2 : 3;
+    int cls[CT];
+#pragma unroll
+    for (int ct = 0; ct < CT; ++ct) {
+        const int f = fl[ct] & 3, la = fl[ct] >> 2;
+        cls[ct] = (f == 3 || hf != 0 || m[ct] >= a.M) ? -1 : (a.span ? ncls - (la + 1) * (la + 2) / 2 + f : f);
+    }
+    unsigned cnt[NCLS];
+#pragma unroll
+    for (int c = 0; c < NCLS; ++c) {
+        cnt[c] = 0;
+#pragma unroll
+        for (int ct = 0; ct < CT; ++ct) cnt[c] += (unsigned)__builtin_popcountll(__builtin_amdgcn_ballot_w64(cls[ct] == c));
+    }
+    __shared__ unsigned wcnt[4][NCLS], wbase[NCLS];
+    if (lane == 0) {
+#pragma unroll
+        for (int c = 0; c < NCLS; ++c) wcnt[wave][c] = cnt[c];
+    }
     __syncthreads();
-    if (threadIdx.x < 3) {
+    if (threadIdx.x < NCLS) {
         const unsigned tot = wcnt[0][threadIdx.x] + wcnt[1][threadIdx.x] + wcnt[2][threadIdx.x] + wcnt[3][threadIdx.x];
         wbase[threadIdx.x] = tot ? atomicAdd(a.counters + 1 + threadIdx.x, tot) : 0u;
         if (tot) atomicAdd(a.counters, tot);
     }
     __syncthreads();
-    unsigned base[3];
-#pragma unroll
-    for (int c = 0; c < 3; ++c) {
-        base[c] = wbase[c];
-        for (int w2 = 0; w2 < wave; ++w2) base[c] += wcnt[w2][c];
-    }
-#pragma unroll
-    for (int c = 0; c < 3; ++c) {
-        unsigned at = __builtin_amdgcn_readfirstlane(base[c]);
+#pragma unroll
+    for (int c = 0; c < NCLS; ++c) {
+        unsigned at = wbase[c];
+        for (int w2 = 0; w2 < wave; ++w2) at += wcnt[w2][c];
+        at = __builtin_amdgcn_readfirstlane(at);
 #pragma unroll
         for (int ct = 0; ct < CT; ++ct) {
-            if (first[ct] == c && hf == 0 && m[ct] < a.M)
-                a.list[(size_t)c * a.M + at + (unsigned)__builtin_popcountll(mask[c][ct] & ((1ull << lane) - 1ull))] = (unsigned)m[ct];
-            at += (unsigned)__builtin_popcountll(mask[c][ct]);
+            const unsigned long long mask = __builtin_amdgcn_ballot_w64(cls[ct] == c);
+            if (cls[ct] == c)
+                a.list[(size_t)c * a.M + at + (unsigned)__builtin_popcountll(mask & ((1ull << lane) - 1ull))] = (unsigned)m[ct];
+            at += (unsigned)__builtin_popcountll(mask);
         }
     }
 }
 
-__global__ void zero_counters_kernel(unsigned* c) { if (threadIdx.x < 4) c[threadIdx.x] = 0; }
+__global__ void zero_counters_kernel(unsigned* c, int n) { if ((int)threadIdx.x < n) c[threadIdx.x] = 0; }
 
 template <int CT, int SEGS, int PACK>
 void launch(const CandArgs& a, hipStream_t st) {
@@ -205,7 +212,7 @@
 }
 
 template <int PACK, int MAX_SEGS>
-int candidates(const char* me, const qv2x_encode_desc* d, const int8_t* in, const int8_t* g_limbs, const double* bias_packed, const int32_t* tables,
+int candidates(const char* me, const int span, const qv2x_encode_desc* d, const int8_t* in, const int8_t* g_limbs, const double* bias_packed, const int32_t* tables,
                const float* tau, uint8_t* codes, uint32_t* list, uint32_t* counters, void* stream) {
     if (!d || !in || !g_limbs || !bias_packed || !tau || !codes || !list || !counters) return fail(QV2X_EINVAL, "%s: null pointer", me);
     if (d->n <= 0 || d->h <= 0 || d->w <= 0 || d->levels < 1 || d->levels > 3) return fail(QV2X_EINVAL, "%s: 1..3 levels", me);
@@ -224,9 +231,9 @@
     a.n = d->n; a.h = d->h; a.w = d->w; a.hw = d->h * d->w; a.M = d->n * a.hw; a.levels = d->levels; a.kc = d->kc; a.ke = segs * d->kc; a.zx = d->in_zx;
     a.gbytes = d->levels * (a.ke / 32) * LIMBS * 8 * 1024;
     a.tbytes = (d->levels > 1 ? d->levels * (d->levels - 1) / 2 : 1) * a.ke * a.ke * 4;
-    a.delta = d->in_delta;
+    a.delta = d->in_delta; a.span = span;
     hipStream_t st = (hipStream_t)stream;
-    zero_counters_kernel<<<1, 64, 0, st>>>(counters);
+    zero_counters_kernel<<<1, 64, 0, st>>>(counters, span ? 9 : 4);
     int dev = 0, cus = 256, v = 0;
     if (hipGetDevice(&dev) == hipSuccess && hipDeviceGetAttribute(&v, hipDeviceAttributeMultiprocessorCount, dev) == hipSuccess && v > 0) cus = v;
     const bool large = a.M >= 4 * cus * 32 * (segs == 2 ? 3 : 4) * 2;
@@ -241,11 +248,23 @@
 extern "C" int qv2x_codebook_encode_candidates_i8(const qv2x_encode_desc* d, const int8_t* in, const int8_t* g_limbs, const double* bias_packed,
                                                   const int32_t* tables, const float* tau, uint8_t* codes, uint32_t* list, uint32_t* counters,
                                                   void* stream) {
-    return qv2x::candidates<128, 1>("qv2x_codebook_encode_candidates_i8", d, in, g_limbs, bias_packed, tables, tau, codes, list, counters, stream);
+    return qv2x::candidates<128, 1>("qv2x_codebook_encode_candidates_i8", 0, d, in, g_limbs, bias_packed, tables, tau, codes, list, counters, stream);
 }
 
 extern "C" int qv2x_codebook_encode_candidates_seg_i8(const qv2x_encode_desc* d, const int8_t* in, const int8_t* g_limbs, const double* bias_packed,
                                                       const int32_t* tables, const float* tau, uint8_t* codes, uint32_t* list, uint32_t* counters,
                                                       void* stream) {
-    return qv2x::candidates<256, 2>("qv2x_codebook_encode_candidates_seg_i8", d, in, g_limbs, bias_packed, tables, tau, codes, list, counters, stream);
-}
+    return qv2x::candidates<256, 2>("qv2x_codebook_encode_candidates_seg_i8", 0, d, in, g_limbs, bias_packed, tables, tau, codes, list, counters, stream);
+}
+
+extern "C" int qv2x_codebook_encode_candidates_span_i8(const qv2x_encode_desc* d, const int8_t* in, const int8_t* g_limbs, const double* bias_packed,
+                                                       const int32_t* tables, const float* tau, uint8_t* codes, uint32_t* list, uint32_t* counters,
+                                                       void* stream) {
+    return qv2x::candidates<128, 1>("qv2x_codebook_encode_candidates_span_i8", 1, d, in, g_limbs, bias_packed, tables, tau, codes, list, counters, stream);
+}
+
+extern "C" int qv2x_codebook_encode_candidates_seg_span_i8(const qv2x_encode_desc* d, const int8_t* in, const int8_t* g_limbs, const double* bias_packed,
+                                                           const int32_t* tables, const float* tau, uint8_t* codes, uint32_t* list, uint32_t* counters,
+                                                           void* stream) {
+    return qv2x::candidates<256, 2>("qv2x_codebook_encode_candidates_seg_span_i8", 1, d, in, g_limbs, bias_packed, tables, tau, codes, list, counters, stream);
+}
diff --git a/quantv2x_amd/csrc/codebook_encode_wave.hip b/quantv2x_amd/csrc/codebook_encode_wave.hip
--- a/quantv2x_amd/csrc/codebook_encode_wave.hip
+++ b/quantv2x_amd/csrc/codebook_encode_wave.hip
@@ -61,13 +61,13 @@
     if (LIST && tile >= plan.full) continue;
     int mrow;
     bool owned;
-    int start = 0;
+    int start = 0, stop = 0;
+    bool dirty = false;
     if (LIST) {
-        int cls, i0;
-        list_tile(plan, tile, cls, i0);
-        owned = i0 + j < plan.n[cls];
-        mrow = (int)a.list[(size_t)cls * a.M + (owned ? i0 + j : plan.n[cls] - 1)];
-        start = cls;
+        const ListTile lt = list_tile(a, plan, tile);
+        owned = lt.i0 + j < lt.n;
+        mrow = (int)a.list[(size_t)lt.cls * a.M + (owned ? lt.i0 + j : lt.n - 1)];
+        start = lt.start; stop = lt.stop;
     } else {
         mrow = a.m_lo + tile * 32 + j;
         owned = mrow < a.m_hi;
@@ -274,6 +274,7 @@
                 const float od = __shfl_xor(best, 32);
                 const int oc = __shfl_xor(bc, 32);
                 if (od < best || (od == best && oc < bc)) bc = oc;
+                if (LIST) dirty |= __builtin_amdgcn_ballot_w64(owned && (int)a.codes[((size_t)l * a.segs + seg) * a.M + mrow] != bc) != 0;
                 if (h == 0 && owned) a.codes[((size_t)l * a.segs + seg) * a.M + mrow] = (uint8_t)bc;
                 bcs |= (unsigned)bc << (8 * seg);
                 best = INFINITY; bc = 0;
@@ -317,6 +318,7 @@
                     const float od = __shfl_xor(best[t], 32);
                     const int oc = __shfl_xor(bc[t], 32);
                     if (od < best[t] || (od == best[t] && oc < bc[t])) bc[t] = oc;
+                    if (LIST) dirty |= __builtin_amdgcn_ballot_w64(owned && (int)a.codes[((size_t)l * SEGS + seg) * a.M + mrow] != bc[t]) != 0;
                     if (h == 0 && owned) a.codes[((size_t)l * SEGS + seg) * a.M + mrow] = (uint8_t)bc[t];
                     bcs |= (unsigned)bc[t] << (8 * seg);
                 }
@@ -327,6 +329,13 @@
         }
         WFINE(5);
         if (last) break;
+        if (LIST && l >= start && l <= stop) {
+            if (dirty && a.defer) {
+                if (lane == 0) a.defer[atomicAdd(a.defer_count, 1u)] = (unsigned)tile;
+                break;
+            }
+            if (l == stop && !dirty) break;
+        }
 #pragma unroll 1
         for (int P = 0; P < 4; ++P) {
             const int seg = (P * a.segs) >> 2;
diff --git a/quantv2x_amd/encode_two_stage.py b/quantv2x_amd/encode_two_stage.py
--- a/quantv2x_amd/encode_two_stage.py
+++ b/quantv2x_amd/encode_two_stage.py
@@ -172,3 +172,17 @@
             flags[p] = (P * second + k2) - (P * best + out[p]) <= P * np.ceil(t) + (P - 1.0)
             gaps[p] = (second - best) * h
     return out, flags.any(0), flags, gaps
+
+
+def span_class(first, last, levels: int):
+    first, last = np.asarray(first), np.asarray(last)
+    return levels * (levels + 1) // 2 - (last + 1) * (last + 2) // 2 + first
+
+
+def span_classes(flags: np.ndarray, levels: int, segs: int = 1):
+    und = np.asarray(flags, bool).reshape(levels, segs, -1).any(1)
+    listed = und.any(0)
+    first = np.where(listed, und.argmax(0), -1).astype(np.int32)
+    last = np.where(listed, levels - 1 - und[::-1].argmax(0), -1).astype(np.int32)
+    cls = np.where(listed, span_class(np.maximum(first, 0), np.maximum(last, 0), levels), -1).astype(np.int32)
+    return first, last, cls
diff --git a/quantv2x_amd/engine.py b/quantv2x_amd/engine.py
--- a/quantv2x_amd/engine.py
+++ b/quantv2x_amd/engine.py
@@ -824,8 +824,9 @@
         if self.two_stage_supported():
             if self._two_stage is None and self.encode_mode == "two_stage":
                 self._build_two_stage()
-            b["enc_list"] = torch.zeros(3 * n * hw, dtype=torch.int32, device=self.dev)
-            b["enc_counters"] = torch.zeros(4, dtype=torch.int32, device=self.dev)
+            b["enc_list"] = torch.zeros(7 * n * hw, dtype=torch.int32, device=self.dev)
+            counters = torch.zeros(16, dtype=torch.int32, device=self.dev)
+            b["enc_counters"], b["enc_span_counters"] = counters[:4], counters[4:]
         if not self.has_codebook or self.heads_single is not None:
             b["feats"] = torch.empty((n, hw, 256), dtype=torch.float32, device=self.dev)
         self._bufs[n] = b
@@ -1048,20 +1049,25 @@
 
     def _encode_two_stage(self, d, b, codes):
         gp, bias, tab, tau, _ = self._two_stage
-        name = self.candidate_entry()
+        name = self.candidate_entry().replace("_i8", "_span_i8")
         L.check(getattr(self.lib, name)(C.byref(d), L.ptr(b["s1"]), L.ptr(gp), L.ptr(bias), L.ptr(tab), tau, L.ptr(codes),
-                                        L.ptr(b["enc_list"]), L.ptr(b["enc_counters"]), L.current_stream()), name)
-        L.check(self.lib.qv2x_codebook_encode_listed_f32(C.byref(d), L.ptr(b["s1"]), self.level_ptrs, L.ptr(b["enc_list"]), L.ptr(b["enc_counters"]),
-                                                         L.ptr(codes), L.current_stream()), "qv2x_codebook_encode_listed_f32")
+                                        L.ptr(b["enc_list"]), L.ptr(b["enc_span_counters"]), L.current_stream()), name)
+        L.check(self.lib.qv2x_codebook_encode_listed_span_f32(C.byref(d), L.ptr(b["s1"]), self.level_ptrs, L.ptr(b["enc_list"]), L.ptr(b["enc_span_counters"]),
+                                                              L.ptr(codes), L.current_stream()), "qv2x_codebook_encode_listed_span_f32")
         return codes
 
     def encode_refine_stats(self, n_agents: int) -> dict:
         if not (self.encode_mode == "two_stage" and self.encode_form == "auto") or "enc_counters" not in self._bufs.get(n_agents, {}):
             raise L.Qv2xError(f"encode_refine_stats({n_agents}): no two-stage encode of {n_agents} frames here (encode_mode "
                               f"{self.encode_mode!r}, encode_form {self.encode_form!r}, workspaces {sorted(self._bufs)})")
-        c = self._bufs[n_agents]["enc_counters"].cpu().numpy().astype(np.int64)
+        c = self._bufs[n_agents]["enc_span_counters"].cpu().numpy().astype(np.int64)
         cells = n_agents * self.fh * self.fw
-        return {"cells": cells, "refined": int(c[0]), "refined_fraction": float(c[0]) / cells, "first_flagged_at_level": [int(v) for v in c[1:1 + self.enc_levels]]}
+        from .encode_two_stage import span_class
+        lv = self.enc_levels
+        span = {(f, la): int(c[1 + int(span_class(f, la, lv))]) for la in range(lv) for f in range(la + 1)}
+        return {"cells": cells, "refined": int(c[0]), "refined_fraction": float(c[0]) / cells,
+                "first_flagged_at_level": [sum(v for (f, _), v in span.items() if f == k) for k in range(lv)],
+                "flagged_by_span": {f"{f}-{la}": v for (f, la), v in sorted(span.items())}}
 
     def encode_into(self, inputs: dict, frames: int, codes_out: torch.Tensor):
         self.pillars_to_canvas(inputs, frames, resident=True)
diff --git a/quantv2x_amd/lib.py b/quantv2x_amd/lib.py
--- a/quantv2x_amd/lib.py
+++ b/quantv2x_amd/lib.py
@@ -20,7 +20,7 @@
     "qv2x_codebook64_level_floats", "qv2x_codebook64_c2_f32", "qv2x_codebook_encode64_f32", "qv2x_codebook_encode64_f32in",
     "qv2x_add_relu_f32", "qv2x_occ_sigmoid_f32", "qv2x_pyramid_weighted_fuse_f32p", "qv2x_bottleneck_i8",
     "qv2x_comm_unique_id", "qv2x_comm_init", "qv2x_comm_destroy", "qv2x_allgather_codes", "qv2x_pairwise_from_poses_f64", "qv2x_pairwise_from_poses_batch_f64",
-    "qv2x_codebook_encode_collapsed_f32", "qv2x_codebook_encode_candidates_i8", "qv2x_codebook_encode_candidates_seg_i8", "qv2x_codebook_encode_listed_f32", "qv2x_mean_vfe_f32", "qv2x_sp_index_scatter", "qv2x_sp_out_sites_workspace_bytes", "qv2x_sp_out_sites", "qv2x_sp_rulebook", "qv2x_sp_conv_f32in", "qv2x_sp_conv_i8", "qv2x_sp_to_bev_i8",
+    "qv2x_codebook_encode_collapsed_f32", "qv2x_codebook_encode_candidates_i8", "qv2x_codebook_encode_candidates_seg_i8", "qv2x_codebook_encode_listed_f32", "qv2x_codebook_encode_candidates_span_i8", "qv2x_codebook_encode_candidates_seg_span_i8", "qv2x_codebook_encode_listed_span_f32", "qv2x_mean_vfe_f32", "qv2x_sp_index_scatter", "qv2x_sp_out_sites_workspace_bytes", "qv2x_sp_out_sites", "qv2x_sp_rulebook", "qv2x_sp_conv_f32in", "qv2x_sp_conv_i8", "qv2x_sp_to_bev_i8",
     "qv2x_fuse_att_band_f32", "qv2x_heads_band", "qv2x_fuse_heads_band", "qv2x_assemble_bands",
     "qv2x_voxelize_batch_workspace_bytes", "qv2x_voxelize_batch_f32", "qv2x_postprocess_batch_workspace_bytes", "qv2x_postprocess_batch_f32",
     "qv2x_eval_workspace_bytes", "qv2x_eval_tp_fp_f32", "qv2x_gt_boxes_f32",
@@ -185,6 +185,9 @@
     lib.qv2x_codebook_encode_candidates_i8.argtypes = [C.POINTER(EncodeDesc), vp, vp, vp, vp, C.POINTER(C.c_float), vp, vp, vp, vp]
     lib.qv2x_codebook_encode_candidates_seg_i8.argtypes = [C.POINTER(EncodeDesc), vp, vp, vp, vp, C.POINTER(C.c_float), vp, vp, vp, vp]
     lib.qv2x_codebook_encode_listed_f32.argtypes = [C.POINTER(EncodeDesc), vp, C.POINTER(vp), vp, vp, vp, vp]
+    lib.qv2x_codebook_encode_candidates_span_i8.argtypes = lib.qv2x_codebook_encode_candidates_i8.argtypes
+    lib.qv2x_codebook_encode_candidates_seg_span_i8.argtypes = lib.qv2x_codebook_encode_candidates_i8.argtypes
+    lib.qv2x_codebook_encode_listed_span_f32.argtypes = lib.qv2x_codebook_encode_listed_f32.argtypes
     lib.qv2x_mean_vfe_f32.argtypes = [vp, vp, vp, C.c_int, C.c_int, vp, vp]
     lib.qv2x_sp_index_scatter.argtypes = [vp, vp, C.c_int, C.c_int, C.c_int, C.c_int, C.c_int, vp, C.c_int, vp]
     lib.qv2x_sp_out_sites_workspace_bytes.argtypes = [C.POINTER(SpconvDesc)]
```

Measured after the change: 6907 (median of 6 runs). +1.5%, better.
